# zhoubin-me/supertonic

Hardware: AMD Instinct MI355X
Metric: audio-sec/sec (RTF^-1), 66M model, batch=128 per GPU (higher is better)
Workload: dtype bf16

## Files before the change

### include/stn.h

```cpp
#ifndef STN_H
#define STN_H
#include <stddef.h>
#include <stdint.h>

#include "stn_arch.h"

#ifdef __cplusplus
extern "C" {
#endif

#define STN_OK 0
#define STN_ERR_INVALID (-1)
#define STN_ERR_DEVICE (-2)
#define STN_ERR_STATE (-3)
#define STN_ERR_UNSUPPORTED (-4)
#define STN_ERR_IO (-5)

#define STN_DTYPE_F32 0
#define STN_DTYPE_BF16 1
#define STN_DTYPE_F16 2

typedef struct stn_handle stn_handle;

typedef struct stn_config {
// ... 216 lines not shown
int stn_op_deesser(stn_handle* h, int hz, int rows, int W, const float* x, const stn_deesser* c, float* y);
int stn_op_deesser_ex(stn_handle* h, int hz, int rows, int W, const float* x, const stn_deesser* c, int x_misalign, int in_place, float* y,
                      float* band, float* gr_db, float* st_end, float* st_start, float* s1_end, float* s1_start, float* s2_end,
                      float* s2_start, int* guard_ok, char* form, size_t form_cap);
int stn_deesser_band(const stn_deesser* c, int rate_hz, double c10[10], float c32[10]);
int stn_deesser_coefs(const stn_deesser* c, int rate_hz, double k[2], float k32[2]);
const char* stn_deesser_error(const stn_deesser* c, int rate_hz);

typedef struct stn_expander { float threshold_db, ratio, knee_db, range_db, attack_ms, hold_ms, release_ms; } stn_expander;
int stn_set_expander(stn_handle* h, int on, const stn_expander* c);
int stn_get_expander(const stn_handle* h, int* on, stn_expander* out);
int stn_batch_expander(stn_handle* h, float* min_attenuation_db, int64_t* closed_samples);
int stn_op_expander(stn_handle* h, int hz, int rows, int W, const float* x, const stn_expander* c, float* y);
int stn_op_expander_ex(stn_handle* h, int hz, int rows, int W, const float* x, const stn_expander* c, int x_misalign, int in_place, float* y,
                       float* open_db, float* s1_end, float* s1_start, float* s2_end, float* s2_start, int* guard_ok, char* form,
                       size_t form_cap);
int stn_expander_coefs(const stn_expander* c, int rate_hz, double k[3], float k32[3], int64_t* hold_samples);
int stn_expander_curve(const stn_expander* c, int n, const double* in_db, double* out_db);
const char* stn_expander_error(const stn_expander* c, int rate_hz);

int stn_profile_enable(stn_handle* h, int on);
int stn_profile_reset(stn_handle* h);
int stn_profile_filter(stn_handle* h, const char* family_or_null);
int stn_profile_sample(stn_handle* h, int every);
int stn_launch_log_enable(stn_handle* h, int on);
int64_t stn_launch_log(stn_handle* h, char* out, size_t cap);
int stn_profile_count(stn_handle* h);
int stn_profile_get(stn_handle* h, int idx, char* name, size_t name_cap, double* total_ms, int64_t* launches,
                    double* flops, double* bytes);

int stn_dbg_xattn_hs_enable(stn_handle* h, int on);
int64_t stn_dbg_xattn_hs_stamps(stn_handle* h, unsigned long long* out, size_t cap);
int stn_dbg_fold_run_frames(const int32_t* latent_lengths, int B, int n_cu);

int stn_op_gemm(stn_handle* h, int dtype, int M, int N, int K, const float* A , const float* W ,
                const float* bias_or_null, int act , float* out );
int stn_op_gemm_ex(stn_handle* h, int dtype, int M, int N, int K, const float* A , const float* W , int mode, int act,
                   int out_dtype, int ldo, const float* bias_or_null, const float* gamma_or_null, const int32_t* len_or_null, int L,
                   const int32_t* row_b_or_null, const float* rowvec_or_null, int nseq, int nt, int tr, float* out, int64_t out_elems,
                   char* form, size_t form_cap);
int stn_dbg_gemm_form(int dtype, int M, int N, int K, int mode, int out_dtype, int ldo, int masked, int tr, char* out, size_t cap);
int stn_dbg_ffn_form(int dtype, int stage, int C, int I, int64_t M, int64_t gate_rows, int packed, int k, int max_dil, int mask,
                     int64_t min_rows, int64_t split_min_rows, int nt_hints, char* out, size_t cap);
int stn_op_gemm_bench(stn_handle* h, int dtype, int M, int N, int K, int mode, int iters, double* avg_ms);
int stn_op_gemm_phases(stn_handle* h, int dtype, int M, int N, int K, int mode, double* out6);
int stn_op_dwconv_ln(stn_handle* h, int dtype, int B, int L, int C, int k, int dil, const float* x,
                     const float* w , const float* bias, const float* ln_g, const float* ln_b, float* y);
int stn_op_dwconv_ln_ragged(stn_handle* h, int dtype, int B, int L, int C, int k, int dil, const float* x,
                            const float* w , const float* bias, const float* ln_g, const float* ln_b,
                            const int32_t* seqlen , float* y);
int stn_op_dwconv_ln_ex(stn_handle* h, int dtype, int B, int L, int C, int k, int dil, const float* x, int64_t x_rows,
                        const float* w_or_null , const float* bias_or_null, const float* ln_g, const float* ln_b,
                        const int32_t* seqlen_or_null, int packed, int ln_only, float* y, int64_t y_rows, char* form, size_t form_cap);
int stn_dbg_dwconv_ln_form(int dtype, int B, int L, int C, int k, int packed, char* out, size_t cap);
int stn_op_fold_ln(stn_handle* h, int dtype, int M, int C, int S, const float* part, const float* b2, const float* gamma,
                   const float* rowvec_or_null, const int32_t* row_b_or_null, int nseq, const float* ln_g, const float* ln_b, float* x,
                   float* y);
int stn_op_layout(stn_handle* h, int which, int dtype, const int32_t* p, int n_p, const float* a, int64_t a_n, const float* b, int64_t b_n,
                  const float* c, int64_t c_n, const int64_t* ids, int64_t ids_n, const int32_t* len, int packed, float* out, int64_t out_n,
                  float* out2, int64_t out2_n, int32_t* iout, int64_t iout_n);
int stn_op_attention(stn_handle* h, int dtype, int B, int Lq, int Lk, int H, int dh, const float* q, const float* k,
                     const float* v, const int32_t* qlen_or_null, const int32_t* klen_or_null, int rope_mode, float* o);
int stn_op_attention_ex(stn_handle* h, int dtype, int B, int Lq, int Lk, int H, int dh, const float* q, int64_t q_elems, int ldq,
                        int q_col, float* kv, int64_t kv_elems, int ldk, int k_col, int v_col, float* o, int64_t o_elems, int ldo,
                        const int32_t* qlen_or_null, const int32_t* klen_or_null, const int32_t* q_off_or_null,
                        const int32_t* k_off_or_null, int rope_mode, int k_rotated, int rot_groups, int rot_stride, int rot_col,
                        char* form, size_t form_cap);
int stn_op_xattn_hs(stn_handle* h, int dtype, int M, const float* xn, const float* Wq, const float* bq_or_null, const float* Wo,
                    const float* kv, int64_t kv_elems, int ldk, int k_col, int B, int L, int Lk, const int32_t* qlen,
                    const int32_t* klen_or_null, const int32_t* k_off_or_null, int rope_mode, int pairs_mode, int64_t part_stride,
                    float* part, int64_t part_elems, int32_t* pairs_out_or_null, char* form, size_t form_cap);
int stn_dbg_attn_form(int kind, int dtype, int B, int Lq, int Lk, int H, int dh, int ldq, int ldk, int misaligned, char* out, size_t cap);
int stn_op_ffn(stn_handle* h, int M, int C, int I, const float* xn , const float* W1, const float* b1, const float* W2,
               const float* b2_or_null, const float* gamma_or_null, const float* rowvec_or_null ,
               const int32_t* row_b_or_null , int nseq, float* x, int fused);
int stn_op_ffn_ex(stn_handle* h, int dtype, int M, int C, int I, const float* xn, int ldx, int64_t xn_elems, const float* W1, const float* b1,
                  const float* W2, const float* b2_or_null, const float* gamma_or_null, const int32_t* len_or_null, int L,
                  const int32_t* row_b_or_null, const float* rowvec_or_null, int rv_ld, int nseq, int mode, int split, float* x, int ldo,
                  int64_t x_elems, float* part_or_null, int64_t part_stride, int64_t part_elems, char* form, size_t form_cap);
int stn_op_ffn_bench(stn_handle* h, int M, int C, int I, int fused, int iters, double* out5);
int stn_op_fold_dwconv_ln(stn_handle* h, int B, int C, int k, int dil, int S, const int32_t* seqlen, const float* x, const float* part,
                          const float* b2_or_null, const float* gamma_or_null, const float* rowvec_or_null , const float* w ,
                          const float* bias, const float* ln_g, const float* ln_b, float* x_out, float* y);
int stn_op_fold_dwconv_ln_ex(stn_handle* h, int dtype, int B, int L, int C, int k, int dil, int S, int run_frames, const int32_t* seqlen,
                             const float* x_in, int64_t x_rows, const float* part, int64_t part_stride, int64_t part_elems,
                             const float* b2_or_null, const float* gamma_or_null, const float* rowvec_or_null, int rv_ld,
                             const float* w , const float* bias, const float* ln_g, const float* ln_b, float* x_out, int64_t x_out_rows,
                             float* y, int64_t y_rows, char* form, size_t form_cap);
int stn_dbg_fold_dwconv_ln_form(int dtype, int B, int L, int C, int k, int dil, int S, int has_rowvec, int run_frames, char* out, size_t cap);
int stn_op_block_bench(stn_handle* h, int B, int L, int C, int I, int k, int dil, int mode, int iters, double* out6);
int stn_op_randn(stn_handle* h, uint64_t seed, int B, int D, int L, const int64_t* utt_ids_or_null,
                 const int32_t* len_or_null, float* out);

const char* stn_version(void);
int stn_hip_versions(int* built, int* runtime);
int stn_device_count(void);
int stn_device_sync(int device);
int stn_ffn_fused_forms(int dtype, int C, int I);

#ifdef __cplusplus
}
#endif
#endif
```

### supertonic_amd/binding.py

```python
import ctypes
import os

import numpy as np

from .arch import StnArch

_HERE = os.path.dirname(os.path.abspath(__file__))
LIB_PATH = os.environ.get("STN_LIB") or os.path.join(_HERE, "libstn.so")
_LIB = None

F32, BF16, F16 = 0, 1, 2
_DTYPES = {"f32": F32, "fp32": F32, "float32": F32, "bf16": BF16, "f16": F16, "fp16": F16, "float16": F16, "half": F16,
           F32: F32, BF16: BF16, F16: F16}
ACT_NONE, ACT_GELU, ACT_SILU, ACT_GELU_TANH = 0, 1, 2, 3
EPI_STORE, EPI_RESID, EPI_STORE_T = 0, 1, 2
FFN_VOCODER, FFN_ESTIMATOR, FFN_TEXT = 1, 2, 4
LAYOUT_ROW_MAP, LAYOUT_NCL_TO_ROWS, LAYOUT_EULER_NCL, LAYOUT_UNPACK_ROWS, LAYOUT_EMBED, LAYOUT_MASKED_MEAN, LAYOUT_IM2COL, LAYOUT_VOCODER_IN = range(8)
ENC_F32, ENC_PCM16, ENC_PCM24, ENC_MULAW, ENC_ALAW = 0, 1, 2, 3, 4
ENCODINGS = {"f32": ENC_F32, "pcm16": ENC_PCM16, "pcm24": ENC_PCM24, "mulaw": ENC_MULAW, "alaw": ENC_ALAW}
ENCODING_NAMES = {v: k for k, v in ENCODINGS.items()}
ENCODING_BYTES = {ENC_F32: 4, ENC_PCM16: 2, ENC_PCM24: 3, ENC_MULAW: 1, ENC_ALAW: 1}
ZERO_CODEWORD = {ENC_F32: 0, ENC_PCM16: 0, ENC_PCM24: 0, ENC_MULAW: 0xFF, ENC_ALAW: 0xD5}


# ... 497 lines not shown
    L.stn_batch_vo_rows.restype = ctypes.c_int64
    L.stn_graph_replays.restype = ctypes.c_int64
    L.stn_graph_replays.argtypes = [vp]
    L.stn_graphs_cached.restype = ctypes.c_int64
    L.stn_graphs_cached.argtypes = [vp]
    L.stn_batch_dims.argtypes = [vp, ctypes.POINTER(ci), ctypes.POINTER(ci), ctypes.POINTER(ctypes.c_int64)]
    L.stn_batch_fetch.argtypes = [vp, vp, ctypes.c_size_t, vp]
    L.stn_batch_fetch_latent.argtypes = [vp, _f32p]
    L.stn_batch_fetch_pcm16.argtypes = [vp, vp, ctypes.c_size_t, vp]
    L.stn_batch_fetch_pcm16_begin.argtypes = [vp, ci]
    L.stn_batch_fetch_slot_dims.argtypes = [vp, ci, ctypes.POINTER(ci), ctypes.POINTER(ctypes.c_int64)]
    L.stn_batch_fetch_pcm16_end.argtypes = [vp, ci, ctypes.POINTER(vp), ctypes.POINTER(ctypes.c_size_t), vp]
    L.stn_host_alloc_pinned.restype = vp
    L.stn_host_alloc_pinned.argtypes = [ctypes.c_size_t]
    L.stn_host_free_pinned.argtypes = [vp]
    L.stn_batch_wav_device_ptr.argtypes = [vp, ctypes.POINTER(vp)]
    L.stn_sync.argtypes = [vp]
    L.stn_set_stream.argtypes = [vp, vp]
    L.stn_batch_copy_wav_device.argtypes = [vp, vp, ctypes.c_int64]
    L.stn_batch_copy_pcm16_device.argtypes = [vp, vp, ctypes.c_int64]
    L.stn_profile_filter.argtypes = [vp, ctypes.c_char_p]
    L.stn_profile_sample.argtypes = [vp, ci]
    L.stn_launch_log_enable.argtypes = [vp, ci]
    L.stn_dbg_xattn_hs_enable.argtypes = [vp, ci]
    L.stn_dbg_xattn_hs_stamps.argtypes = [vp, vp, ctypes.c_size_t]
    L.stn_dbg_xattn_hs_stamps.restype = ctypes.c_int64
    L.stn_dbg_fold_run_frames.argtypes = [vp, ctypes.c_int, ctypes.c_int]
    L.stn_dbg_fold_run_frames.restype = ctypes.c_int
    L.stn_dbg_gemm_form.argtypes = [ci, ci, ci, ci, ci, ci, ci, ci, ci, ctypes.c_char_p, ctypes.c_size_t]
    L.stn_dbg_gemm_form.restype = ctypes.c_int
    L.stn_dbg_attn_form.argtypes = [ci, ci, ci, ci, ci, ci, ci, ci, ci, ci, ctypes.c_char_p, ctypes.c_size_t]
    L.stn_dbg_attn_form.restype = ctypes.c_int
    L.stn_dbg_ffn_form.argtypes = [ci, ci, ci, ci, ctypes.c_int64, ctypes.c_int64, ci, ci, ci, ci, ctypes.c_int64, ctypes.c_int64, ci,
                                   ctypes.c_char_p, ctypes.c_size_t]
    L.stn_dbg_ffn_form.restype = ctypes.c_int
    L.stn_launch_log.argtypes = [vp, ctypes.c_char_p, ctypes.c_size_t]
    L.stn_launch_log.restype = ctypes.c_int64
    L.stn_profile_enable.argtypes = [vp, ci]
    L.stn_profile_reset.argtypes = [vp]
    L.stn_profile_count.argtypes = [vp]
    L.stn_profile_get.argtypes = [vp, ci, ctypes.c_char_p, ctypes.c_size_t, ctypes.POINTER(ctypes.c_double),
                                  ctypes.POINTER(ctypes.c_int64), ctypes.POINTER(ctypes.c_double),
                                  ctypes.POINTER(ctypes.c_double)]
    L.stn_op_gemm.argtypes = [vp, ci, ci, ci, ci, _f32p, _f32p, vp, ci, _f32p]
    L.stn_op_gemm_ex.argtypes = [vp, ci, ci, ci, ci, _f32p, _f32p, ci, ci, ci, ci, vp, vp, vp, ci, vp, vp, ci, ci, ci, _f32p,
                                 ctypes.c_int64, ctypes.c_char_p, ctypes.c_size_t]
    L.stn_op_gemm_bench.argtypes = [vp, ci, ci, ci, ci, ci, ci, ctypes.POINTER(ctypes.c_double)]
    L.stn_op_gemm_phases.argtypes = [vp, ci, ci, ci, ci, ci, ctypes.POINTER(ctypes.c_double)]
    L.stn_op_dwconv_ln.argtypes = [vp, ci, ci, ci, ci, ci, ci, _f32p, _f32p, _f32p, _f32p, _f32p, _f32p]
    L.stn_op_dwconv_ln_ragged.argtypes = [vp, ci, ci, ci, ci, ci, ci, _f32p, _f32p, _f32p, _f32p, _f32p, _i32p, _f32p]
    L.stn_op_attention.argtypes = [vp, ci, ci, ci, ci, ci, ci, _f32p, _f32p, _f32p, vp, vp, ci, _f32p]
    L.stn_op_dwconv_ln_ex.argtypes = [vp, ci, ci, ci, ci, ci, ci, _f32p, ctypes.c_int64, vp, vp, _f32p, _f32p, vp, ci, ci, _f32p, ctypes.c_int64,
                                      ctypes.c_char_p, ctypes.c_size_t]
    L.stn_dbg_resample_form.argtypes = [ci, ci, ctypes.c_int64, ctypes.c_char_p, ctypes.c_size_t]
    L.stn_dbg_resample_form.restype = ctypes.c_int
    L.stn_dbg_dwconv_ln_form.argtypes = [ci, ci, ci, ci, ci, ci, ctypes.c_char_p, ctypes.c_size_t]
    L.stn_dbg_dwconv_ln_form.restype = ctypes.c_int
    L.stn_op_fold_ln.argtypes = [vp, ci, ci, ci, ci, _f32p, _f32p, _f32p, vp, vp, ci, _f32p, _f32p, _f32p, _f32p]
    L.stn_op_layout.argtypes = [vp, ci, ci, _i32p, ci, vp, ctypes.c_int64, vp, ctypes.c_int64, vp, ctypes.c_int64, vp, ctypes.c_int64, vp, ci,
                                vp, ctypes.c_int64, vp, ctypes.c_int64, vp, ctypes.c_int64]
    L.stn_op_attention_ex.argtypes = [vp, ci, ci, ci, ci, ci, ci, _f32p, ctypes.c_int64, ci, ci, _f32p, ctypes.c_int64, ci, ci, ci,
                                      _f32p, ctypes.c_int64, ci, vp, vp, vp, vp, ci, ci, ci, ci, ci, ctypes.c_char_p, ctypes.c_size_t]
    L.stn_op_xattn_hs.argtypes = [vp, ci, ci, _f32p, _f32p, vp, _f32p, _f32p, ctypes.c_int64, ci, ci, ci, ci, ci, _i32p, vp, vp, ci, ci,
                                  ctypes.c_int64, _f32p, ctypes.c_int64, vp, ctypes.c_char_p, ctypes.c_size_t]
    L.stn_op_randn.argtypes = [vp, cu64, ci, ci, ci, vp, vp, _f32p]
    L.stn_op_ffn.argtypes = [vp, ci, ci, ci, _f32p, _f32p, _f32p, _f32p, vp, vp, vp, vp, ci, _f32p, ci]
    L.stn_op_ffn_ex.argtypes = [vp, ci, ci, ci, ci, _f32p, ci, ctypes.c_int64, _f32p, _f32p, _f32p, vp, vp, vp, ci, vp, vp, ci, ci, ci, ci, _f32p, ci,
                                ctypes.c_int64, vp, ctypes.c_int64, ctypes.c_int64, ctypes.c_char_p, ctypes.c_size_t]
    L.stn_op_ffn_bench.argtypes = [vp, ci, ci, ci, ci, ci, ctypes.POINTER(ctypes.c_double)]
    L.stn_set_fused_ffn.argtypes = [vp, ci]
    L.stn_set_fused_ffn_min_rows.argtypes = [vp, ctypes.c_int64, ctypes.c_int64]
    L.stn_op_fold_dwconv_ln.argtypes = [vp, ci, ci, ci, ci, ci, _i32p, _f32p, _f32p, vp, vp, vp, _f32p, _f32p, _f32p, _f32p, _f32p, _f32p]
    L.stn_op_fold_dwconv_ln_ex.argtypes = [vp, ci, ci, ci, ci, ci, ci, ci, ci, _i32p, _f32p, ctypes.c_int64, _f32p, ctypes.c_int64, ctypes.c_int64, vp, vp,
                                           vp, ci, _f32p, _f32p, _f32p, _f32p, _f32p, ctypes.c_int64, _f32p, ctypes.c_int64, ctypes.c_char_p,
                                           ctypes.c_size_t]
    L.stn_dbg_fold_dwconv_ln_form.argtypes = [ci, ci, ci, ci, ci, ci, ci, ci, ci, ctypes.c_char_p, ctypes.c_size_t]
    L.stn_dbg_fold_dwconv_ln_form.restype = ctypes.c_int
    L.stn_op_block_bench.argtypes = [vp, ci, ci, ci, ci, ci, ci, ci, ci, ctypes.POINTER(ctypes.c_double)]
    L.stn_group_create.argtypes = [ci, vp, ci, ctypes.POINTER(vp)]
    L.stn_group_destroy.argtypes = [vp]
    L.stn_group_last_error.restype = ctypes.c_char_p
    L.stn_group_last_error.argtypes = [vp]
    L.stn_group_size.argtypes = [vp]
    L.stn_group_uses_rccl.argtypes = [vp]
    L.stn_group_handle.restype = vp
    L.stn_group_handle.argtypes = [vp, ci]
    L.stn_group_load_synthetic.argtypes = [vp, ctypes.POINTER(StnArch), cu64]
    L.stn_group_load_dir.argtypes = [vp, ctypes.c_char_p]
    L.stn_group_deal.argtypes = [ci, _i32p, ci, _i32p, _i32p]
    L.stn_group_synthesize.argtypes = [vp, ci, ci, _i64p, _f32p, _f32p, _f32p, ci, cf, vp, cu64, ctypes.POINTER(ctypes.c_int64)]
    L.stn_group_fetch_pcm16.argtypes = [vp, vp, ctypes.c_size_t, vp]
    L.stn_set_output_rate.argtypes = [vp, ci]
    L.stn_get_output_rate.argtypes = [vp]
    L.stn_resample_filter.argtypes = [ci, ci, vp, ctypes.c_size_t, ctypes.POINTER(ci), ctypes.POINTER(ci)]
    L.stn_resample_error.argtypes = [ci, ci]
    L.stn_resample_error.restype = ctypes.c_char_p
    L.stn_op_resample.argtypes = [vp, ci, ci, ci, ci, _f32p, vp, vp]
    L.stn_group_set_output_rate.argtypes = [vp, ci]
    _f64p = np.ctypeslib.ndpointer(np.float64, flags="C_CONTIGUOUS")
    L.stn_set_loudness.argtypes = [vp, ci, cf, cf]
    L.stn_get_loudness.argtypes = [vp, ctypes.POINTER(ci), ctypes.POINTER(cf), ctypes.POINTER(cf)]
    L.stn_batch_loudness.argtypes = [vp, vp, vp, vp]
    L.stn_op_loudness.argtypes = [vp, ci, ci, ci, _f32p, vp, vp, vp]
    L.stn_kweighting_filter.argtypes = [ci, _f64p, _f64p, _f64p, _f64p]
    L.stn_op_loudness_ex.argtypes = [vp, ci, ci, ci, _f32p, vp, ci, cf, cf, ci, vp, vp, vp, vp, vp, vp, vp, vp, ctypes.c_char_p, ctypes.c_size_t]
    L.stn_loudness_table.argtypes = [ci, vp, vp, ctypes.c_size_t, ctypes.POINTER(ci)]
# ... 1474 lines not shown
        C = x_in.shape[1]
        w = _c(w, np.float32)
        _b2, b2p = _opt(b2, np.float32)
        _g, gp = _opt(gamma, np.float32)
        _v, vp_ = _opt(rowvec, np.float32)
        form = ctypes.create_string_buffer(96)
        self._ck(self._lib.stn_op_fold_dwconv_ln_ex(self._h, self.dtype if dtype is None else _DTYPES[dtype], len(seqlen), int(L), C, w.shape[1], int(dil),
                                                    int(S), int(run_frames), seqlen, x_in.reshape(-1), x_in.shape[0], part, int(part_stride), part.size,
                                                    b2p, gp, vp_, C if _v is None else _v.shape[1], w, _c(bias, np.float32), _c(g, np.float32),
                                                    _c(b, np.float32), xo.reshape(-1), xo.shape[0], yo.reshape(-1), yo.shape[0], form, ctypes.sizeof(form)))
        return xo, yo, form.value.decode()

    def op_block_bench(self, B, L, C, I, k, dil, mode, iters=20):
        out = (ctypes.c_double * 6)()
        self._ck(self._lib.stn_op_block_bench(self._h, B, L, C, I, k, dil, mode, iters, out))
        return dict(ms=out[0], conv_ms=out[1], fold_phase1=out[2], fold_barrier=out[3], fold_phase2=out[4], fold_span=out[5])

    def set_fused_ffn_min_rows(self, k4_rows=-1, split_rows=-1):
        self._ck(self._lib.stn_set_fused_ffn_min_rows(self._h, int(k4_rows), int(split_rows)))

    def op_gemm_phases(self, M, N, K, mode=0, dtype=None):
        out = (ctypes.c_double * 6)()
        self._ck(self._lib.stn_op_gemm_phases(self._h, self.dtype if dtype is None else _DTYPES[dtype], M, N, K, mode, out))
        return dict(first_stage=out[0], k_loop=out[1], epilogue=out[2], grid_span=out[3], entry_spread=out[4], workgroups=int(out[5]))

    def op_dwconv_ln(self, x, w, bias, g, b, dil, dtype=None, seqlen=None):
        B, L, C = x.shape
        k = w.shape[1]
        y = np.empty((B, L, C), np.float32)
        if seqlen is not None:
            self._ck(self._lib.stn_op_dwconv_ln_ragged(self._h, self.dtype if dtype is None else _DTYPES[dtype], B, L, C, k,
                                                       dil, _c(x, np.float32), _c(w, np.float32), _c(bias, np.float32),
                                                       _c(g, np.float32), _c(b, np.float32), _c(seqlen, np.int32), y))
            return y
        self._ck(self._lib.stn_op_dwconv_ln(self._h, self.dtype if dtype is None else _DTYPES[dtype], B, L, C, k, dil,
                                            _c(x, np.float32), _c(w, np.float32), _c(bias, np.float32),
                                            _c(g, np.float32), _c(b, np.float32), y))
        return y

    def op_dwconv_ln_ex(self, x, w, bias, g, b, dil, out, B, L, seqlen=None, packed=False, ln_only=False, dtype=None):
        x = _c(x, np.float32)
        o_r = np.array(out, dtype=np.float32, order="C", copy=True)
        C = x.shape[1]
        _w, wp = _opt(w, np.float32)
        _b, bp = _opt(bias, np.float32)
        _l, lp = _opt(seqlen, np.int32)
        form = ctypes.create_string_buffer(32)
        self._ck(self._lib.stn_op_dwconv_ln_ex(self._h, self.dtype if dtype is None else _DTYPES[dtype], int(B), int(L), C,
                                               1 if _w is None else _w.shape[1], int(dil), x.reshape(-1), x.shape[0], wp, bp, _c(g, np.float32),
                                               _c(b, np.float32), lp, int(bool(packed)), int(bool(ln_only)), o_r.reshape(-1), o_r.shape[0], form,
                                               ctypes.sizeof(form)))
        return o_r, form.value.decode()

    def op_fold_ln(self, x, part, b2, gamma, g, b, rowvec=None, row_b=None, dtype=None):
        x_r = np.array(x, dtype=np.float32, order="C", copy=True)
        M, C = x_r.shape
        part = _c(part, np.float32)
        y = np.empty((M, C), np.float32)
        _v, vp_ = _opt(rowvec, np.float32)
        _r, rp = _opt(row_b, np.int32)
        self._ck(self._lib.stn_op_fold_ln(self._h, self.dtype if dtype is None else _DTYPES[dtype], M, C, part.shape[0], part.reshape(-1),
                                          _c(b2, np.float32), _c(gamma, np.float32), vp_, rp, 0 if _v is None else _v.shape[0],
                                          _c(g, np.float32), _c(b, np.float32), x_r, y))
        return x_r, y

    def op_layout(self, which, p, a=None, b=None, c=None, ids=None, length=None, packed=False, out=None, out2=None, iout=None, dtype="f32"):
        def f32(v):
            return (None, None, 0) if v is None else (lambda arr: (arr, arr.ctypes.data, arr.size))(_c(v, np.float32))
        pa = _c(p, np.int32)
        _a, ap, an = f32(a)
        _b, bp, bn = f32(b)
        _cc, cp, cn = f32(c)
        _i, ip = _opt(ids, np.int64)
        _l, lp = _opt(length, np.int32)
        o1 = None if out is None else np.array(out, dtype=np.float32, order="C", copy=True)
        o2 = None if out2 is None else np.array(out2, dtype=np.float32, order="C", copy=True)
        io = None if iout is None else np.array(iout, dtype=np.int32, order="C", copy=True)
        ptr = lambda v: (None, 0) if v is None else (v.ctypes.data, v.size)
        self._ck(self._lib.stn_op_layout(self._h, int(which), _DTYPES[dtype], pa, len(pa), ap, an, bp, bn, cp, cn, ip, 0 if _i is None else _i.size,
                                         lp, int(bool(packed)), *ptr(o1), *ptr(o2), *ptr(io)))
        return o1, o2, io

    def op_attention(self, q, k, v, H, qlen=None, klen=None, rope_mode=-1, dtype=None):
        B, Lq, C = q.shape
        Lk = k.shape[1]
        o = np.empty((B, Lq, C), np.float32)
        _q, qp = _opt(qlen, np.int32)
        _k, kp = _opt(klen, np.int32)
        self._ck(self._lib.stn_op_attention(self._h, self.dtype if dtype is None else _DTYPES[dtype], B, Lq, Lk, H,
                                            C // H, _c(q, np.float32), _c(k, np.float32), _c(v, np.float32), qp, kp,
                                            rope_mode, o))
        return o

    def op_attention_ex(self, q, kv, out, B, Lq, Lk, H, dh, q_col=0, k_col=0, v_col=None, qlen=None, klen=None, q_off=None, k_off=None,
                        rope_mode=-1, k_rotated=False, rot_groups=1, rot_stride=0, rot_col=None, dtype=None):
        q = _c(q, np.float32)
        kv_r = np.array(kv, dtype=np.float32, order="C", copy=True)
        o_r = np.array(out, dtype=np.float32, order="C", copy=True)
        _a, qlp = _opt(qlen, np.int32)
        _b, klp = _opt(klen, np.int32)
        _d, qop = _opt(q_off, np.int32)
        _e, kop = _opt(k_off, np.int32)
        form = ctypes.create_string_buffer(64)
        self._ck(self._lib.stn_op_attention_ex(self._h, self.dtype if dtype is None else _DTYPES[dtype], int(B), int(Lq), int(Lk), int(H), int(dh),
                                               q.reshape(-1), q.size, q.shape[1], int(q_col), kv_r.reshape(-1), kv_r.size, kv_r.shape[1],
                                               int(k_col), int(k_col + H * dh if v_col is None else v_col), o_r.reshape(-1), o_r.size,
# ... 42 lines not shown
```

### supertonic_amd/csrc/api.cpp

```cpp
#include "../../include/stn.h"

#include <algorithm>
#include <complex>
#include <cstdio>
#include <cstring>
#include <fstream>
#include <string>

#include "engine.hpp"
#include "host/json_min.hpp"
#include "host/graph_bind.hpp"
#include "host/onnx_reader.hpp"

#include <map>
#include <sstream>

struct stn_handle {
    stn::Engine* eng = nullptr;
    std::string err;
    std::vector<std::pair<std::string, stn::KernelStat>> prof;
};

static thread_local std::string g_create_err;

// ... 883 lines not shown
        (dtype != STN_DTYPE_F32 && dtype != STN_DTYPE_BF16 && dtype != STN_DTYPE_F16))
        return STN_ERR_INVALID;
    const std::string f = stn::ffn_form(dtype, stage, C, I, M, gate_rows, packed != 0, k, max_dil, mask, min_rows, split_min_rows, nt_hints != 0).str();
    if (out && cap > f.size()) std::memcpy(out, f.c_str(), f.size() + 1);
    return (int)f.size();
}
int stn_op_gemm_bench(stn_handle* h, int dtype, int M, int N, int K, int mode, int iters, double* avg_ms) {
    STN_TRY(h, { need(M > 0 && N > 0 && K > 0 && iters > 0 && avg_ms, "stn_op_gemm_bench: bad argument");
                 need(K % (dtype != STN_DTYPE_F32 ? 8 : 4) == 0, "K must be a multiple of 8 (bf16) / 4 (f32)");
                 *avg_ms = h->eng->op_gemm_bench(dtype, M, N, K, mode, iters); })
}
int stn_op_gemm_phases(stn_handle* h, int dtype, int M, int N, int K, int mode, double* out6) {
    STN_TRY(h, { need(M > 0 && N > 0 && K > 0 && out6, "stn_op_gemm_phases: bad argument");
                 need(K % (dtype != STN_DTYPE_F32 ? 8 : 4) == 0, "K must be a multiple of 8 (bf16) / 4 (f32)");
                 h->eng->op_gemm_phases(dtype, M, N, K, mode, out6); })
}
int stn_op_dwconv_ln(stn_handle* h, int dtype, int B, int L, int C, int k, int dil, const float* x, const float* w,
                     const float* bias, const float* g, const float* b, float* y) {
    STN_TRY(h, { need(B > 0 && L > 0 && C > 0 && C % 4 == 0 && C <= 1024 && k > 0 && (k & 1) && dil > 0 && x && w && bias && g && b && y,
                      "stn_op_dwconv_ln: bad argument");
                 h->eng->op_dwconv_ln(dtype, B, L, C, k, dil, x, w, bias, g, b, y); })
}
int stn_op_dwconv_ln_ragged(stn_handle* h, int dtype, int B, int L, int C, int k, int dil, const float* x, const float* w,
                            const float* bias, const float* g, const float* b, const int32_t* seqlen, float* y) {
    STN_TRY(h, { need(B > 0 && L > 0 && C > 0 && C % 4 == 0 && C <= 1024 && k > 0 && (k & 1) && dil > 0 && x && w && bias && g && b && y && seqlen,
                      "stn_op_dwconv_ln_ragged: bad argument");
                 for (int i = 0; i < B; ++i) need(seqlen[i] >= 0 && seqlen[i] <= L, "stn_op_dwconv_ln_ragged: seqlen out of [0, L]");
                 h->eng->op_dwconv_ln(dtype, B, L, C, k, dil, x, w, bias, g, b, y, seqlen); })
}
static void dwconv_ln_ex_checked(stn_handle* h, int dtype, int B, int L, int C, int k, int dil, const float* x, int64_t x_rows, const float* w,
                                 const float* bias, const float* g, const float* b, const int32_t* seqlen, int packed, int ln_only, float* y,
                                 int64_t y_rows, char* form, size_t form_cap) {
    need(B > 0 && L > 0 && C > 0 && C % 4 == 0 && C <= 1024 && k > 0 && (k & 1) && dil > 0 && x && g && b && y && x_rows > 0 && y_rows > 0,
         "stn_op_dwconv_ln_ex: bad argument");
    need(dtype == STN_DTYPE_F32 || dtype == STN_DTYPE_BF16 || dtype == STN_DTYPE_F16, "stn_op_dwconv_ln_ex: unknown dtype");
    need(ln_only || (w && bias), "stn_op_dwconv_ln_ex: the conv needs w and bias");
    need(!(packed && ln_only), "stn_op_dwconv_ln_ex: ln_only takes no packed layout");
    need(!packed || (seqlen && B <= 1024), "stn_op_dwconv_ln_ex: packed rows need seqlen and B <= 1024");
    int64_t rows = (int64_t)B * L;
    if (seqlen && !ln_only) {
        int64_t tot = 0;
        for (int i = 0; i < B; ++i) { need(seqlen[i] >= 0 && seqlen[i] <= L, "stn_op_dwconv_ln_ex: seqlen out of [0, L]"); tot += seqlen[i]; }
        if (packed) rows = tot;
    }
    need(x_rows >= rows && y_rows >= rows, "stn_op_dwconv_ln_ex: x / y hold fewer rows than the launch addresses");
    const std::string f = h->eng->op_dwconv_ln_ex(dtype, B, L, C, k, dil, x, x_rows, w, bias, g, b, ln_only ? nullptr : seqlen, packed, ln_only, y, y_rows);
    if (form && form_cap) std::snprintf(form, form_cap, "%s", f.c_str());
}
int stn_op_dwconv_ln_ex(stn_handle* h, int dtype, int B, int L, int C, int k, int dil, const float* x, int64_t x_rows, const float* w,
                        const float* bias, const float* g, const float* b, const int32_t* seqlen, int packed, int ln_only, float* y,
                        int64_t y_rows, char* form, size_t form_cap) {
    STN_TRY(h, dwconv_ln_ex_checked(h, dtype, B, L, C, k, dil, x, x_rows, w, bias, g, b, seqlen, packed, ln_only, y, y_rows, form, form_cap))
}
int stn_dbg_dwconv_ln_form(int dtype, int B, int L, int C, int k, int packed, char* out, size_t cap) {
    if (B < 1 || L < 1 || C < 1 || k < 1 || !(k & 1) || (dtype != STN_DTYPE_F32 && dtype != STN_DTYPE_BF16 && dtype != STN_DTYPE_F16)) return STN_ERR_INVALID;
    std::string f;
    try { f = stn::dwconv_ln_form(dtype, B, L, C, k, packed != 0).str(); } catch (const std::exception&) { return STN_ERR_INVALID; }
    if (out && cap > f.size()) std::memcpy(out, f.c_str(), f.size() + 1);
    return (int)f.size();
}
int stn_op_fold_ln(stn_handle* h, int dtype, int M, int C, int S, const float* part, const float* b2, const float* gamma, const float* rowvec,
                   const int32_t* row_b, int nseq, const float* g, const float* b, float* x, float* y) {
    STN_TRY(h, { need(M > 0 && C > 0 && C % 4 == 0 && C <= 1024 && (S == 4 || S == 8 || S == 12 || S == 24) && part && b2 && gamma && g && b && x && y,
                      "stn_op_fold_ln: bad argument");
                 need(dtype == STN_DTYPE_BF16 || dtype == STN_DTYPE_F16, "stn_op_fold_ln: a 16-bit format needed");
                 need(!rowvec || nseq > 0, "stn_op_fold_ln: rowvec needs nseq > 0");
                 if (rowvec && row_b) for (int m = 0; m < M; ++m) need(row_b[m] >= 0 && row_b[m] < nseq, "stn_op_fold_ln: row_b out of range");
                 h->eng->op_fold_ln(dtype, M, C, S, part, b2, gamma, rowvec, row_b, nseq, g, b, x, y); })
}
int stn_op_layout(stn_handle* h, int which, int dtype, const int32_t* p, int n_p, const float* a, int64_t a_n, const float* b, int64_t b_n,
                  const float* c, int64_t c_n, const int64_t* ids, int64_t ids_n, const int32_t* len, int packed, float* out, int64_t out_n,
                  float* out2, int64_t out2_n, int32_t* iout, int64_t iout_n) {
    static const int n_params[8] = {3, 4, 5, 3, 4, 3, 6, 6};
    STN_TRY(h, { need(which >= 0 && which < 8 && p && n_p == n_params[which], "stn_op_layout: unknown kernel or parameter count");
                 need(dtype == STN_DTYPE_F32 || dtype == STN_DTYPE_BF16 || dtype == STN_DTYPE_F16, "stn_op_layout: unknown dtype");
                 need(a_n >= 0 && b_n >= 0 && c_n >= 0 && ids_n >= 0 && out_n >= 0 && out2_n >= 0 && iout_n >= 0 && (a || !a_n) && (b || !b_n) && (c || !c_n) &&
                          (ids || !ids_n) && (out || !out_n) && (out2 || !out2_n) && (iout || !iout_n),
                      "stn_op_layout: a buffer without a pointer");
                 h->eng->op_layout(which, dtype, p, a, a_n, b, b_n, c, c_n, ids, ids_n, len, packed, out, out_n, out2, out2_n, iout, iout_n); })
}
int stn_op_attention(stn_handle* h, int dtype, int B, int Lq, int Lk, int H, int dh, const float* q, const float* k,
                     const float* v, const int32_t* qlen, const int32_t* klen, int rope_mode, float* o) {
    STN_TRY(h, { need(B > 0 && Lq > 0 && Lk > 0 && H > 0 && dh >= 8 && dh % 8 == 0 && dh <= 96 && q && k && v && o,
                      "stn_op_attention: bad argument");
                 h->eng->op_attention(dtype, B, Lq, Lk, H, dh, q, k, v, qlen, klen, rope_mode, o); })
}
static void attention_ex_checked(stn_handle* h, int dtype, int B, int Lq, int Lk, int H, int dh, const float* q, int64_t q_elems, int ldq,
                                 int q_col, float* kv, int64_t kv_elems, int ldk, int k_col, int v_col, float* o, int64_t o_elems, int ldo,
                                 const int32_t* qlen, const int32_t* klen, const int32_t* q_off, const int32_t* k_off, int rope_mode,
                                 int k_rotated, int rot_groups, int rot_stride, int rot_col, char* form, size_t form_cap) {
    need(B > 0 && Lq > 0 && Lk > 0 && H > 0 && dh >= 8 && dh % 8 == 0 && dh <= 96 && q && kv && o, "stn_op_attention_ex: bad argument");
    need(dtype == STN_DTYPE_F32 || dtype == STN_DTYPE_BF16 || dtype == STN_DTYPE_F16, "stn_op_attention_ex: unknown dtype");
    need(rope_mode >= -1 && rope_mode <= 1, "stn_op_attention_ex: rope_mode must be -1, 0 or 1");
    const int64_t C = (int64_t)H * dh;
    need(ldq > 0 && ldk > 0 && ldo >= C && q_col >= 0 && k_col >= 0 && v_col >= 0 && q_col + C <= ldq && k_col + C <= ldk && v_col + C <= ldk,
         "stn_op_attention_ex: the heads must lie inside the rows (col + H*dh <= ld, ldo >= H*dh)");
    need((q_off == nullptr || qlen) && (k_off == nullptr || klen), "stn_op_attention_ex: packed rows need their lengths");
    const int64_t qrows = q_elems / ldq, krows = kv_elems / ldk, orows = o_elems / ldo;
    for (int b = 0; b < B; ++b) {
        need(!qlen || qlen[b] >= 0, "stn_op_attention_ex: qlen < 0");
        need(!klen || klen[b] >= 0, "stn_op_attention_ex: klen < 0");
        if (q_off)
            need(qlen[b] <= Lq && q_off[b] >= 0 && (int64_t)q_off[b] + qlen[b] <= std::min(qrows, orows),
                 "stn_op_attention_ex: packed query rows outside q / o (or qlen > Lq)");
        if (k_off) need(k_off[b] >= 0 && (int64_t)k_off[b] + std::min(klen[b], Lk) <= krows, "stn_op_attention_ex: packed key rows outside kv");
    }
// ... 169 lines not shown
```

### supertonic_amd/csrc/engine.cpp

```cpp
#include "engine.hpp"
#include "dev_env.hpp"
#include "engine_internal.hpp"

#include <algorithm>
#include <cmath>
#include <cstdio>
#include <cstring>

namespace stn {
using detail::up;

Arena::~Arena() {
    for (auto& c : chunks_) (void)hipFree(c.p);
}
size_t Arena::capacity() const {
    size_t t = 0;
    for (auto& c : chunks_) t += c.cap;
    return t;
}
void* Arena::alloc(size_t bytes) {
    bytes = (bytes + 255) & ~size_t(255);
    if (bytes == 0) bytes = 256;
    for (;;) {
        if (cur_ < chunks_.size()) {
// ... 80 lines not shown
    STN_HIP(hipEventCreateWithFlags(&ev_te_, hipEventDisableTiming));
    STN_HIP(hipEventCreateWithFlags(&ev_copied_, hipEventDisableTiming));
    STN_HIP(hipEventCreateWithFlags(&ev_dp_, hipEventDisableTiming));
    STN_HIP(hipStreamCreateWithPriority(&te_s_, hipStreamNonBlocking, prio_side));
    if (const char* p = stn::dev_env("STN_DP_STREAM")) if (atoi(p) == 0) {
        (void)hipStreamDestroy(dp_s_); dp_s_ = nullptr;
        (void)hipStreamDestroy(te_s_); te_s_ = nullptr;
    }
    if (const char* p = stn::dev_env("STN_NT")) nt_hints_ = atoi(p) != 0;
    if (const char* p = stn::dev_env("STN_FFN")) fused_ffn_ = atoi(p);
    if (const char* p = stn::dev_env("STN_FFN_MIN_ROWS")) ffn_min_rows_ = atoll(p);
    if (const char* p = stn::dev_env("STN_XATTN")) set_fused_xattn(atoi(p));
    if (const char* p = stn::dev_env("STN_FFN_SPLIT_MIN_ROWS")) ffn_split_min_rows_ = atoll(p);
    if (const char* p = stn::dev_env("STN_PACKED")) packed_ve_ = atoi(p) != 0;
}

void Engine::set_stream(hipStream_t s) {
    sync();
    s_ = s ? s : own_s_;
}

void Engine::drop_graphs() {
    for (auto& g : graphs_) {
        if (g.exec) (void)hipGraphExecDestroy(g.exec);
        if (g.graph) (void)hipGraphDestroy(g.graph);
        if (g.exec2) (void)hipGraphExecDestroy(g.exec2);
        if (g.graph2) (void)hipGraphDestroy(g.graph2);
    }
    graphs_.clear();
    warm_keys_.clear();
}

void Engine::free_weights() {
    if (s_) (void)hipStreamSynchronize(s_);
    drop_graphs();
    ++wgen_;
    for (void* p : owned_) (void)hipFree(p);
    owned_.clear();
    w_.clear();
    frag_w_.clear();
    ffn_w_.clear();
    loaded_ = false;
    params_ = 0;
}

Engine::~Engine() {
    (void)hipSetDevice(device_);
    if (s_) (void)hipStreamSynchronize(s_);
    if (dp_s_) (void)hipStreamSynchronize(dp_s_);
    if (te_s_) (void)hipStreamSynchronize(te_s_);
    free_weights();
    for (void* p : batch_owned_) (void)hipFree(p);
    for (void* p : batch_retired_) (void)hipFree(p);
    if (vo_quiet_) (void)hipFree(vo_quiet_);
    if (vo_edge_) (void)hipFree(vo_edge_);
    if (tcond_.buf) (void)hipFree(tcond_.buf);
    for (auto& sp : spans_) { (void)hipEventDestroy(sp.a); (void)hipEventDestroy(sp.b); }
    for (auto ev : ev_pool_) (void)hipEventDestroy(ev);
    drop_graphs();
    if (pin_llen_) (void)hipHostFree(pin_llen_);
    if (pin_seed_) (void)hipHostFree(pin_seed_);
    if (seed_dev_) (void)hipFree(seed_dev_);
    rs_release();
    fl_release();
    xp_release();
    ds_release();
    cp_release();
    lo_release();
    for (auto& f : fetch_) {
        if (f.busy && f.done) (void)hipEventSynchronize(f.done);
        if (f.dev) (void)hipFree(f.dev);
        if (f.pin) (void)hipHostFree(f.pin);
        if (f.ready) (void)hipEventDestroy(f.ready);
        if (f.done) (void)hipEventDestroy(f.done);
    }
    if (copy_s_) (void)hipStreamDestroy(copy_s_);
    if (own_s_) (void)hipStreamDestroy(own_s_);
    if (dp_s_) (void)hipStreamDestroy(dp_s_);
    if (te_s_) (void)hipStreamDestroy(te_s_);
    if (ev_te_) (void)hipEventDestroy(ev_te_);
    if (ev_copied_) (void)hipEventDestroy(ev_copied_);
    if (ev_dp_) (void)hipEventDestroy(ev_dp_);
}

DevTensor& Engine::tensor(const std::string& name) {
    auto it = w_.find(name);
    if (it == w_.end()) throw std::runtime_error("unknown weight tensor: " + name);
    return it->second;
}
Linear Engine::linear(const std::string& p) {
    Linear l;
    l.w = tensor(p + ".w");
    l.b = tensor(p + ".b").f32;
    l.N = l.w.rows;
    l.K = l.w.cols;
    return l;
}
LNorm Engine::lnorm(const std::string& p) { return LNorm{tensor(p + ".g").f32, tensor(p + ".b").f32}; }
ConvNeXt Engine::convnext_w(const std::string& p) {
    ConvNeXt c;
    c.dw_t = tensor(p + ".dw.wt").f32;
    c.dw_b = tensor(p + ".dw.b").f32;
    c.ln = lnorm(p + ".ln");
    c.pw1 = linear(p + ".pw1");
    c.pw2 = linear(p + ".pw2");
    c.gamma = tensor(p + ".gamma").f32;
    return c;
}
// ... 257 lines not shown
        while (b < k.size() && (k[b] == '(' || k[b] == ' ' || k[b] == '&')) ++b;
        size_t en = b;
        while (en < k.size() && (isalnum((unsigned char)k[en]) || k[en] == '_' || k[en] == ':')) ++en;
        out += e.first + "\t" + k.substr(b, en - b) + "\n";
    }
    return out;
}
std::vector<std::pair<std::string, KernelStat>> Engine::profile_collect() {
    sync();
    std::unordered_map<std::string, KernelStat> acc;
    std::vector<std::string> order;
    for (auto& sp : spans_) {
        float ms = 0.f;
        if (hipEventElapsedTime(&ms, sp.a, sp.b) != hipSuccess) { (void)hipGetLastError(); continue; }
        auto it = acc.find(sp.tag);
        if (it == acc.end()) { order.push_back(sp.tag); it = acc.emplace(sp.tag, KernelStat{}).first; }
        it->second.ms += ms;
        it->second.launches += 1;
        it->second.flops += sp.flops;
        it->second.bytes += sp.bytes;
    }
    std::vector<std::pair<std::string, KernelStat>> out;
    for (auto& t : order) out.emplace_back(t, acc[t]);
    return out;
}

void Engine::gemm(const char* tag, int dt, const void* A, int lda, const Linear& w, int M, Epilogue e) {
    if (!e.bias) e.bias = w.b;
    const double esz = is_half(dt) ? 2.0 : 4.0;
    if (prof_on_) {
        double out_b = (double)M * w.N * (e.mode == EPI_STORE ? (is_half(e.out_dtype) ? 2.0 : 4.0) : (e.mode == EPI_RESID ? 8.0 : 4.0));
        prof_begin(tag, 2.0 * M * (double)w.N * w.K, ((double)M * w.K + (double)w.N * w.K) * esz + out_b);
    }
    const GemmForm f = gemm_form(dt, M, w.N, w.K, lda, w.K, e, A, w.w.as(dt));
    if (f.split > 1) {
        const Arena::Mark mk = ar_.mark();
        float* ws = f32_alloc((int64_t)f.split * M * w.N);
        launch_gemm_form(s_, f, A, lda, w.w.as(dt), w.K, M, w.N, w.K, e, ws);
        ar_.release(mk);
    } else {
        launch_gemm_form(s_, f, A, lda, w.w.as(dt), w.K, M, w.N, w.K, e, nullptr);
    }
    if (prof_on_) prof_end();
}

void* Engine::to_act(const float* src, int64_t n) {
    if (dt_ == F32) return const_cast<float*>(src);
    void* d = act_alloc(n);
    launch_cast(s_, dt_, src, n, d);
    return d;
}

void Engine::convnext(const ConvNeXt& p, const FfnForm& f, float* x, int B, int L, int C, int hid, int k, int dil, const int* len,
                      const int* conv_len, const float* rowvec, int rv_ld, const Ragged* rg, FoldState* fs) {
    const int64_t M = rg ? (int64_t)rg->rows : (int64_t)B * L;
    if (f.kind == FFN_K4_SPLIT && !(fs && rg)) throw std::logic_error("convnext: K4-split needs the stage's fold state and packed rows");
    const Arena::Mark mk = ar_.mark();
    void* xn = act_alloc(M * C);
    if (fs) x = fs->x;
    if (fs && fs->pending) {
        if (prof_on_) prof_begin("fold_dwconv_ln", (double)M * C * (2.0 * k + 8 + 2.0 * fs->fold.S), (double)M * C * (8.0 + 2.0 + 2.0 * fs->fold.S));
        fs->fold.run_frames = rg->fold_run;
        launch_fold_dwconv_ln(s_, dt_, fs->x, fs->x_alt, B, L, C, fs->fold, p.dw_t, p.dw_b, k, dil, p.ln.g, p.ln.b, a_.ln_eps, xn, len, rg->off);
        if (prof_on_) prof_end();
        std::swap(fs->x, fs->x_alt);
        fs->pending = false;
        x = fs->x;
    } else {
        if (prof_on_) prof_begin("dwconv_ln", (double)M * C * (2.0 * k + 8), (double)M * C * (4.0 + (is_half(dt_) ? 2.0 : 4.0)));
        launch_dwconv_ln(s_, dt_, x, B, L, C, p.dw_t, p.dw_b, k, dil, p.ln.g, p.ln.b, a_.ln_eps, xn, rg ? len : conv_len, rg ? rg->off : nullptr);
        if (prof_on_) prof_end();
    }
    FfnArgs fa;
    fa.xn = xn; fa.ldx = C; fa.b1 = p.pw1.b; fa.b2 = p.pw2.b; fa.gamma = p.gamma; fa.x = x; fa.ldo = C; fa.M = (int)M; fa.I = hid;
    fa.rowvec = rowvec; fa.rv_ld = rv_ld; fa.row_b = (rg && rowvec) ? rg->row_b : nullptr;
    fa.len = rg ? nullptr : len; fa.L = L;
    if (f.kind != FFN_GEMMS) {
        const auto fw = ffn_w_.find(p.pw1.w.as(dt_));
        const int* s = std::find(std::begin(FFN_SPLITS), std::end(FFN_SPLITS), f.split);
        fa.wseq = fw == ffn_w_.end() ? nullptr : f.kind == FFN_K4 ? fw->second.wseq : s != std::end(FFN_SPLITS) ? fw->second.wsplit[s - FFN_SPLITS] : nullptr;
        if (!fa.wseq) throw std::logic_error("convnext: no packed weight stream for " + f.str());
    }
    if (f.kind == FFN_K4_SPLIT) { fa.part = fs->part; fa.part_stride = fs->part_stride; }
    const FoldArgs pending = ffn_launch(f, C, fa, p.pw1, p.pw2);
    if (f.kind == FFN_K4_SPLIT) { fs->fold = pending; fs->pending = true; }
    ar_.release(mk);
}

FoldArgs Engine::ffn_launch(const FfnForm& f, int C, const FfnArgs& a, const Linear& w1, const Linear& w2) {
    const int64_t M = a.M;
    const int hid = a.I;
    FoldArgs pending;
    if (f.kind == FFN_K4_SPLIT) {
        FfnArgs sa;
        sa.xn = a.xn; sa.ldx = a.ldx; sa.wseq = a.wseq; sa.b1 = a.b1; sa.M = a.M; sa.I = hid; sa.ts = a.ts;
        sa.split = f.split; sa.part = a.part; sa.part_stride = a.part_stride;
        if (prof_on_) prof_begin("ffn_split", 4.0 * M * (double)C * hid, (double)M * C * (2.0 + 2.0 * sa.split) + 4.0 * C * hid);
        launch_ffn_fused(s_, dt_, C, sa);
        if (prof_on_) prof_end();
        pending = ffn_pending(f, a);
    } else if (f.kind == FFN_K4) {
        if (prof_on_) prof_begin("ffn_fused", 4.0 * M * (double)C * hid, (double)M * C * (2.0 + 8.0) + 4.0 * C * hid);
        launch_ffn_fused(s_, dt_, C, a);
        if (prof_on_) prof_end();
    } else {
        const Arena::Mark mk = ar_.mark();
        void* u = act_alloc(M * hid);
        Epilogue e1;
        e1.mode = EPI_STORE; e1.act = gelu_act_; e1.out_dtype = dt_; e1.out = u; e1.ldo = hid; e1.bias = a.b1; e1.nt = f.nt ? 1 : 0;
        gemm("gemm_pw1_gelu", dt_, a.xn, a.ldx, w1, (int)M, e1);
        Epilogue e2;
        e2.mode = EPI_RESID; e2.resid = a.x; e2.ldo = a.ldo; e2.bias = a.b2; e2.gamma = a.gamma; e2.len = a.len; e2.L = a.L;
        e2.rowvec = a.rowvec; e2.rv_ld = a.rv_ld; e2.row_b = a.row_b;
        gemm("gemm_pw2_resid", dt_, u, hid, w2, (int)M, e2);
        ar_.release(mk);
    }
    return pending;
}

void Engine::fold_layernorm(FoldState& fs, int64_t M, int C, const LNorm& ln, void* xn, const char* tag) {
    const size_t esz = is_half(dt_) ? 2 : 4;
    if (fs.pending) {
        if (prof_on_) prof_begin("fold_ln", (double)M * C * (8 + 2.0 * fs.fold.S), (double)M * C * (8.0 + esz + 2.0 * fs.fold.S));
// ... 334 lines not shown
                owned_.push_back(dst);
                launch_repack_frag_acc(s_, src, w.o.N, w.o.K, dst);
                frag_acc_w_[src] = dst;
            }
        }
    sync();
}

void Engine::prepare_ffn_weights() {
    ffn_w_.clear();
    const stn_arch& a = a_;
    void* tmp = nullptr;
    size_t tmp_bytes = 0;
    auto add = [&](const std::string& p, int C, int hid) {
        if (!ffn_fused_supported(dt_, C, hid)) return;
        const ConvNeXt c = convnext_w(p);
        void* wseq = nullptr;
        STN_HIP(hipMalloc(&wseq, (size_t)2 * hid * C * 2));
        owned_.push_back(wseq);
        if ((size_t)2 * hid * C * 2 > tmp_bytes) {
            if (tmp) (void)hipFree(tmp);
            tmp_bytes = (size_t)2 * hid * C * 2;
            STN_HIP(hipMalloc(&tmp, tmp_bytes));
        }
        launch_ffn_pack(s_, c.pw1.w.as(dt_), c.pw2.w.as(dt_), C, hid, tmp, wseq);
        sync();
        FfnW fw; fw.wseq = wseq;
        if (p.compare(0, 3, "ve.") == 0)
            for (size_t i = 0; i < std::size(FFN_SPLITS); ++i) {
                if (!ffn_split_valid(dt_, C, hid, FFN_SPLITS[i])) continue;
                void* ws = nullptr;
                STN_HIP(hipMalloc(&ws, (size_t)2 * hid * C * 2));
                owned_.push_back(ws);
                launch_ffn_pack(s_, c.pw1.w.as(dt_), c.pw2.w.as(dt_), C, hid, tmp, ws, FFN_SPLITS[i]);
                sync();
                fw.wsplit[i] = ws;
            }
        ffn_w_[c.pw1.w.as(dt_)] = fw;
    };
    auto S = [](const char* fmt, int i, int j = 0) { char b[64]; snprintf(b, sizeof b, fmt, i, j); return std::string(b); };
    for (int i = 0; i < a.dp_conv_blocks; ++i) add(S("dp.conv%d", i), a.dp_dim, a.dp_hidden);
    for (int i = 0; i < a.te_conv_blocks; ++i) add(S("te.conv%d", i), a.te_dim, a.te_hidden);
    for (int b = 0; b < a.ve_main_blocks; ++b) {
        for (int j = 0; j < a.ve_dilated; ++j) add(S("ve.m%d.dil%d", b, j), a.ve_dim, a.ve_hidden);
        add(S("ve.m%d.cn_a", b), a.ve_dim, a.ve_hidden);
        add(S("ve.m%d.cn_b", b), a.ve_dim, a.ve_hidden);
    }
    for (int j = 0; j < a.ve_tail_blocks; ++j) add(S("ve.tail%d", j), a.ve_dim, a.ve_hidden);
    for (int i = 0; i < a.vo_blocks; ++i) add(S("vo.blk%d", i), a.vo_dim, a.vo_hidden);
    sync();
    if (tmp) (void)hipFree(tmp);
}

void Engine::prepare_vocoder_constants() {
    if (vo_quiet_) { (void)hipFree(vo_quiet_); vo_quiet_ = nullptr; }
    if (vo_edge_) { (void)hipFree(vo_edge_); vo_edge_ = nullptr; }
    vo_rf_ = 0;
    const stn_arch& a = a_;
    if (!is_half(dt_) || !dwconv_ln_supports_packed(a.vo_dim, a.vo_kernel) || a.base_chunk_size % 4) return;
    const int rf = vocoder_receptive_field(), ccf = a.chunk_compress_factor, W = a.base_chunk_size;
    const int Lz = (4 * rf + ccf) / ccf + 1, Tz = Lz * ccf, D = a.latent_dim * ccf;
    ar_.reset();
    float* lat = f32_alloc((int64_t)D * Lz);
    float* wz = f32_alloc((int64_t)Tz * W);
    STN_HIP(hipMemsetAsync(lat, 0, sizeof(float) * (size_t)D * Lz, s_));
    vocoder_dev(1, Lz, lat, wz);
    STN_HIP(hipMalloc(reinterpret_cast<void**>(&vo_quiet_), sizeof(float) * (size_t)W));
    STN_HIP(hipMalloc(reinterpret_cast<void**>(&vo_edge_), sizeof(float) * (size_t)rf * W));
    STN_HIP(hipMemcpyAsync(vo_quiet_, wz + (size_t)2 * rf * W, sizeof(float) * (size_t)W, hipMemcpyDeviceToDevice, s_));
    STN_HIP(hipMemcpyAsync(vo_edge_, wz + (size_t)(Tz - rf) * W, sizeof(float) * (size_t)rf * W, hipMemcpyDeviceToDevice, s_));
    sync();
    vo_rf_ = rf;
}

int Engine::trimmed_rows(int B, int L, std::vector<int>* n_host) const {
    if (!packed_ve_ || vo_ragged_ || !vo_quiet_ || vo_rf_ <= 0 || B > 1024) return 0;
    const int ccf = a_.chunk_compress_factor, T = L * ccf, rf = vo_rf_;
    long tot = 0;
    bool any = false;
    for (int i = 0; i < B; ++i) {
        const int l6 = bt_.h_llen[i] * ccf;
        const bool trim = l6 + 2 * rf <= T;
        any = any || trim;
        const int n = trim ? l6 + 2 * rf : T;
        if (n_host) n_host->push_back(n);
        tot += n;
    }
    return (any && tot * 10 <= (long)B * T * 9) ? (int)tot : 0;
}

void Engine::vocoder_dev(int B, int L, const float* latent, float* wav, const int* vlen, int vrows, const int* valid) {
    stage_ = "vo";
    const stn_arch& a = a_;
    const int C = a.vo_dim, T = L * a.chunk_compress_factor;
    const bool packed = vlen && vrows > 0 && is_half(dt_) && B <= 1024 && dwconv_ln_supports_packed(C, a.vo_kernel);
    if (valid && !packed) throw std::runtime_error("trimmed vocoder needs the packed bf16 path");
    const int64_t M = packed ? (int64_t)vrows : (int64_t)B * T;
    const Arena::Mark mk = ar_.mark();
    Ragged rg;
    if (packed) {
        int* off = static_cast<int*>(ar_.alloc(sizeof(int) * (size_t)(B + 1)));
        launch_row_map(s_, vlen, B, off, nullptr);
        rg.off = off; rg.rows = vrows;
    }
    const Ragged* rgp = packed ? &rg : nullptr;
    float* x = f32_alloc(M * C);
    if (is_half(dt_)) {
        const int kp = (a.latent_dim * a.vo_in_kernel + 63) / 64 * 64;
        void* cols = act_alloc(M * kp);
        launch_vocoder_im2col(s_, dt_, latent, B, L, a.latent_dim, a.chunk_compress_factor, a.vo_in_kernel, kp, cols, vlen,
                              packed ? rg.off : nullptr);
        Linear lin;
        lin.w = tensor("vo.in_gemm.w"); lin.b = vecf("vo.in.b"); lin.N = C; lin.K = kp;
        Epilogue ei; ei.mode = EPI_STORE; ei.out_dtype = F32; ei.out = x; ei.ldo = C;
        gemm("gemm_in", dt_, cols, kp, lin, (int)M, ei);
    } else {
        if (prof_on_) prof_begin("vocoder_in", 2.0 * M * C * a.latent_dim * a.vo_in_kernel, (double)M * (a.latent_dim + C) * 4.0);
        launch_vocoder_in(s_, latent, B, L, a.latent_dim, a.chunk_compress_factor, vecf("vo.in.wt"), vecf("vo.in.b"), C,
                          a.vo_in_kernel, x, vlen);
        if (prof_on_) prof_end();
    }
    const FfnForm ff = ffn_plan(FFN_VOCODER, C, a.vo_hidden, M, valid ? (int64_t)B * T : 0, packed, a.vo_kernel,
                                a.vo_blocks ? *std::max_element(a.vo_dilations, a.vo_dilations + a.vo_blocks) : 1);
    for (int i = 0; i < a.vo_blocks; ++i)
        convnext(convnext_w("vo.blk" + std::to_string(i)), ff, x, B, T, C, a.vo_hidden, a.vo_kernel, a.vo_dilations[i],
                 packed ? vlen : nullptr, packed ? nullptr : vlen, nullptr, 0, rgp);
    void* xn = act_alloc(M * C);
    const LNorm ln = lnorm("vo.out_ln");
    launch_layernorm(s_, dt_, x, M, C, ln.g, ln.b, a.ln_eps, xn);
    if (packed) {
        float* wp = f32_alloc(M * a.base_chunk_size);
        Epilogue e; e.mode = EPI_STORE; e.out_dtype = F32; e.out = wp; e.ldo = a.base_chunk_size;
        gemm("gemm_head", dt_, xn, C, linear("vo.head"), (int)M, e);
        if (valid) launch_unpack_rows_quiet(s_, wp, valid, rg.off, B, T, a.base_chunk_size, vo_rf_, vo_quiet_, vo_edge_, wav);
        else launch_unpack_rows(s_, wp, vlen, rg.off, B, T, a.base_chunk_size, wav);
    } else {
        Epilogue e; e.mode = EPI_STORE; e.out_dtype = F32; e.out = wav; e.ldo = a.base_chunk_size; e.len = vlen; e.L = T;
        gemm("gemm_head", dt_, xn, C, linear("vo.head"), (int)M, e);
    }
    ar_.release(mk);
}


void Engine::duration(int B, int Lt, const int64_t* ids, const float* style_dp, const float* text_mask, float* dur) {
    STN_HIP(hipSetDevice(device_));
    ar_.reset();
    int64_t* d_ids = up(ar_, s_, ids, (size_t)B * Lt);
    float* d_mask = up(ar_, s_, text_mask, (size_t)B * Lt);
    float* d_st = up(ar_, s_, style_dp, (size_t)B * a_.n_style_dp * a_.d_style_dp);
    int* tlen = static_cast<int*>(ar_.alloc(sizeof(int) * B));
    float* d_dur = f32_alloc(B);
    launch_mask_to_len(s_, d_mask, B, Lt, tlen);
    duration_dev(B, Lt, d_ids, d_st, tlen, d_dur);
    STN_HIP(hipMemcpyAsync(dur, d_dur, sizeof(float) * B, hipMemcpyDeviceToHost, s_));
    sync();
}

void Engine::text_enc(int B, int Lt, const int64_t* ids, const float* style_ttl, const float* text_mask, float* text_emb) {
    STN_HIP(hipSetDevice(device_));
    ar_.reset();
    int64_t* d_ids = up(ar_, s_, ids, (size_t)B * Lt);
    float* d_mask = up(ar_, s_, text_mask, (size_t)B * Lt);
    float* d_st = up(ar_, s_, style_ttl, (size_t)B * a_.n_style_ttl * a_.d_style_ttl);
    int* tlen = static_cast<int*>(ar_.alloc(sizeof(int) * B));
    const size_t n = (size_t)B * a_.te_out_dim * Lt;
    float* d_out = f32_alloc(n);
    launch_mask_to_len(s_, d_mask, B, Lt, tlen);
    text_enc_dev(B, Lt, d_ids, d_st, tlen, d_out, nullptr);
    STN_HIP(hipMemcpyAsync(text_emb, d_out, n * 4, hipMemcpyDeviceToHost, s_));
    sync();
}

void Engine::vector_est(int B, int L, int Lt, const float* noisy, const float* text_emb, const float* style_ttl,
                        const float* text_mask, const float* latent_mask, const float* total_step,
                        const float* current_step, float* denoised) {
    STN_HIP(hipSetDevice(device_));
    ar_.reset();
    const int D = a_.latent_dim * a_.chunk_compress_factor, Ce = a_.te_out_dim;
    float* d_x = up(ar_, s_, noisy, (size_t)B * D * L);
    float* d_emb = up(ar_, s_, text_emb, (size_t)B * Ce * Lt);
    float* d_st = up(ar_, s_, style_ttl, (size_t)B * a_.n_style_ttl * a_.d_style_ttl);
    float* d_tm = up(ar_, s_, text_mask, (size_t)B * Lt);
    float* d_lm = up(ar_, s_, latent_mask, (size_t)B * L);
    float* d_tot = up(ar_, s_, total_step, (size_t)B);
    float* d_cur = up(ar_, s_, current_step, (size_t)B);
    int* tlen = static_cast<int*>(ar_.alloc(sizeof(int) * B));
    int* llen = static_cast<int*>(ar_.alloc(sizeof(int) * B));
    float* d_out = f32_alloc((size_t)B * D * L);
// ... 24 lines not shown
```

### supertonic_amd/csrc/engine.hpp

```cpp
#pragma once
#include <cmath>
#include <hip/hip_runtime.h>

#include <cstdint>
#include <functional>
#include <iterator>
#include <stdexcept>
#include <string>
#include <unordered_map>
#include <vector>

#include "../../include/stn_arch.h"
#include "host/join_plan.hpp"
#include "host/pause_plan.hpp"
#include "host/pitch.hpp"
#include "kernels.hpp"

namespace stn {

#define STN_HIP(expr)                                                                                          \
    do {                                                                                                       \
        hipError_t e_ = (expr);                                                                                \
        if (e_ != hipSuccess)                                                                                  \
            throw std::runtime_error(std::string("HIP error: ") + hipGetErrorString(e_) + " at " #expr);       \
// ... 77 lines not shown
};

struct Carve {
    char* base = nullptr;
    size_t off = 0;
    template <typename T> T* take(size_t count) {
        const size_t o = off;
        off += (count * sizeof(T) + 255) / 256 * 256;
        return base ? reinterpret_cast<T*>(base + o) : nullptr;
    }
};

struct KernelStat { double ms = 0; long launches = 0; double flops = 0; double bytes = 0; };

class Engine {
   public:
    Engine(int device, int dtype);
    ~Engine();
    Engine(const Engine&) = delete;

    void load_synthetic(const stn_arch& a, uint64_t seed);
    using TensorSource = std::function<std::vector<float>(const std::string& name, int rows, int cols)>;
    void load_tensors(const stn_arch& a, const TensorSource& src);
    std::vector<std::string> tensor_names(const stn_arch& a);
    bool loaded() const { return loaded_; }
    const stn_arch& arch() const { return a_; }
    int64_t param_count() const { return params_; }
    int dtype() const { return dt_; }
    hipStream_t stream() const { return s_; }
    void sync() { STN_HIP(hipStreamSynchronize(s_)); if (dp_s_) STN_HIP(hipStreamSynchronize(dp_s_)); if (te_s_) STN_HIP(hipStreamSynchronize(te_s_)); }
    void set_stream(hipStream_t s);

    struct Ragged;
    void duration_dev(int B, int Lt, const int64_t* ids, const float* style_dp, const int* tlen, float* dur, const Ragged* trg = nullptr);
    void text_enc_dev(int B, int Lt, const int64_t* ids, const float* style_ttl, const int* tlen, float* ncl, void* rows,
                      const Ragged* trg = nullptr);
    struct VeCtx { void* text_kv = nullptr; void* style_kv = nullptr; int Lt = 0; const int* text_off = nullptr; };
    VeCtx ve_prepare_dev(int B, int Lt, const void* text_rows, const float* style_ttl, const int* tlen, const Ragged* trg = nullptr, bool defer_text = false);
    void ve_text_kv_dev(const VeCtx& c, int B, int Lt, const void* text_rows, const int* tlen, const Ragged* trg);
    float* ve_time_cond_dev(int rows, const float* total_step, const float* current_step, float* tb_out = nullptr );
    struct TimeCond { int steps = 0, B = 0; uint64_t wgen = ~0ull; float* buf = nullptr; size_t cap = 0; float *tot = nullptr, *cur = nullptr, *dt = nullptr, *tb = nullptr; };
    TimeCond tcond_;
    void ensure_time_cond(int total_step, int B);
    struct Ragged { const int* off = nullptr; const int* row_b = nullptr; int rows = 0;
                    const int* hs_pairs = nullptr;
                    int fold_run = 0; };
    void ve_step_dev(int B, int L, const VeCtx& c, const float* noisy, const int* tlen, const int* llen,
                     const float* total_step, const float* current_step, float* denoised, const float* tb = nullptr,
                     const Ragged* rg = nullptr, const float* dt = nullptr ,
                     void* z_rows = nullptr ,
                     bool z_ready = false ,
                     bool z_next = false );
    void vocoder_dev(int B, int L, const float* latent, float* wav, const int* vlen = nullptr, int vrows = 0,
                     const int* valid = nullptr);
    int vocoder_receptive_field() const;
    void prepare_xattn_weights();
    std::unordered_map<const void*, const void*> frag_w_;
    void hs_stamps_enable(bool on);
    int64_t hs_stamps_fetch(unsigned long long* out, size_t cap);
    unsigned long long* hs_ts_ = nullptr;
    int hs_ts_wgs_ = 0;
    static constexpr int HS_TS_WG = 8192;
    const float* unit_vec_ = nullptr;
    std::unordered_map<const void*, const void*> frag_acc_w_;
    void prepare_vocoder_constants();
    void prepare_ffn_weights();
    struct FfnW { const void *wseq = nullptr, *wsplit[std::size(FFN_SPLITS)] = {}; };
    std::unordered_map<const void*, FfnW> ffn_w_;

    void duration(int B, int Lt, const int64_t* ids, const float* style_dp, const float* text_mask, float* dur);
    void text_enc(int B, int Lt, const int64_t* ids, const float* style_ttl, const float* text_mask, float* text_emb);
    void vector_est(int B, int L, int Lt, const float* noisy, const float* text_emb, const float* style_ttl,
                    const float* text_mask, const float* latent_mask, const float* total_step,
                    const float* current_step, float* denoised);
    void vocoder(int B, int L, const float* latent, float* wav);

    struct Batch {
        int B = 0, Lt = 0, L = 0, noise_L = 0, total_step = 0;
        float speed = 1.f;
        bool have_override = false, have_noise = false;
        uint64_t noise_seed = 0;
        int64_t* ids = nullptr; size_t ids_cap = 0;
        int* tlen = nullptr; size_t tlen_cap = 0;
        float* style_ttl = nullptr; size_t ttl_cap = 0;
        float* style_dp = nullptr; size_t dp_cap = 0;
        float* dur = nullptr; size_t dur_cap = 0;
        int* llen = nullptr; size_t llen_cap = 0;
        int64_t* utt_ids = nullptr; size_t utt_cap = 0;
        float* noise = nullptr; size_t noise_cap = 0;
        float* xt[2] = {nullptr, nullptr}; size_t xt_cap[2] = {0, 0};
        float* wav = nullptr; size_t wav_cap = 0;
        unsigned char* text_side = nullptr; size_t text_side_cap = 0;
        unsigned char* text_rows = nullptr; size_t text_cap = 0;
        int* toff = nullptr; size_t toff_cap = 0;
        int trows = 0;
        uint64_t gen = 0;
        std::vector<float> h_dur; std::vector<int> h_llen;
    };
    void batch_upload(int B, int Lt, const int64_t* ids, const float* text_mask, const float* style_ttl,
                      const float* style_dp, const float* duration_override, const int64_t* utt_ids);
    void batch_set_noise(const float* noise, int L);
    void batch_run(int total_step, float speed, uint64_t noise_seed);
    void set_graph_mode(bool on) { graph_on_ = on; }
    void set_vocoder_mode(bool length_aware) { vo_ragged_ = length_aware; }
    void set_packed_rows(bool on) { packed_ve_ = on; }
    void set_gelu_form(int tanh_form) { if ((tanh_form != 0) != (gelu_act_ == ACT_GELU_TANH)) { sync(); drop_graphs(); } gelu_act_ = tanh_form ? ACT_GELU_TANH : ACT_GELU; }
    int gelu_form() const { return gelu_act_ == ACT_GELU_TANH ? 1 : 0; }
// ... 142 lines not shown
        const char* form = "";
    };
    void op_compressor(int hz, int rows, int W, const float* x, const stn_compressor& c, float* y, CpProbe* probe);

    void set_deesser(bool on, const stn_deesser* c);
    bool deesser_on() const { return ds_on_; }
    const stn_deesser& deesser() const { return ds_set_; }
    void batch_deesser(float* max_reduction_db);
    struct DsProbe {
        int x_misalign = 0, in_place = 0;
        float *band = nullptr, *gr = nullptr, *st_end = nullptr, *st_start = nullptr;
        float *s1_end = nullptr, *s1_start = nullptr, *s2_end = nullptr, *s2_start = nullptr;
        bool guard_ok = false;
        const char* form = "";
    };
    void op_deesser(int hz, int rows, int W, const float* x, const stn_deesser& c, float* y, DsProbe* probe);

    void set_expander(bool on, const stn_expander* c);
    bool expander_on() const { return xp_on_; }
    const stn_expander& expander() const { return xp_set_; }
    void batch_expander(float* min_attenuation_db, int64_t* closed_samples);
    struct XpProbe {
        int x_misalign = 0, in_place = 0;
        float *open = nullptr, *s1_end = nullptr, *s1_start = nullptr, *s2_end = nullptr, *s2_start = nullptr;
        bool guard_ok = false;
        const char* form = "";
    };
    void op_expander(int hz, int rows, int W, const float* x, const stn_expander& c, float* y, XpProbe* probe);

    void profile_enable(bool on) { if (on != prof_on_) profile_reset(); prof_on_ = on; }
    void launch_log_enable(bool on);
    std::string launch_log() const;
    void profile_sample(int every) { prof_every_ = every < 1 ? 1 : every; prof_seen_ = 0; }
    void profile_filter(const std::string& family) { if (family != prof_filter_) profile_reset(); prof_filter_ = family; }
    void profile_reset();
    std::vector<std::pair<std::string, KernelStat>> profile_collect();

    void op_gemm(int dtype, int M, int N, int K, const float* A, const float* W, const float* bias, int act, float* out);
    std::string op_gemm_ex(int dtype, int M, int N, int K, const float* A, const float* W, int mode, int act, int out_dtype, int ldo,
                           const float* bias, const float* gamma, const int* len, int L, const int* row_b, const float* rowvec, int nseq,
                           int nt, int tr, float* out, int64_t out_elems);
    std::string op_attention_ex(int dtype, int B, int Lq, int Lk, int H, int dh, const float* q, int64_t q_elems, int ldq, int q_col,
                                float* kv, int64_t kv_elems, int ldk, int k_col, int v_col, float* o, int64_t o_elems, int ldo,
                                const int* qlen, const int* klen, const int* q_off, const int* k_off, int rope_mode, int k_rotated,
                                int rot_groups, int rot_stride, int rot_col);
    std::string op_xattn_hs(int dtype, int M, const float* xn, const float* Wq, const float* bq, const float* Wo, const float* kv,
                            int64_t kv_elems, int ldk, int k_col, int B, int L, int Lk, const int* qlen, const int* klen, const int* k_off,
                            int rope_mode, int pairs_mode, int64_t part_stride, float* part, int64_t part_elems, int* pairs_out);
    void op_attention(int dtype, int B, int Lq, int Lk, int H, int dh, const float* q, const float* k, const float* v,
                      const int* qlen, const int* klen, int rope_mode, float* o);
    void op_dwconv_ln(int dtype, int B, int L, int C, int k, int dil, const float* x, const float* w, const float* bias,
                      const float* g, const float* b, float* y, const int* seqlen = nullptr );
    std::string op_dwconv_ln_ex(int dtype, int B, int L, int C, int k, int dil, const float* x, int64_t x_rows, const float* w, const float* bias,
                                const float* g, const float* b, const int* seqlen, int packed, int ln_only, float* y, int64_t y_rows);
    void op_fold_ln(int dtype, int M, int C, int S, const float* part, const float* b2, const float* gamma, const float* rowvec, const int* row_b,
                    int nseq, const float* g, const float* b, float* x, float* y);
    void op_layout(int which, int dtype, const int* p, const float* a, int64_t a_n, const float* b, int64_t b_n, const float* c, int64_t c_n,
                   const int64_t* ids, int64_t ids_n, const int* len, int packed, float* out, int64_t out_n, float* out2, int64_t out2_n, int* iout,
                   int64_t iout_n);
    double op_gemm_bench(int dtype, int M, int N, int K, int mode, int iters);
    void op_gemm_phases(int dtype, int M, int N, int K, int mode, double* out6);
    void op_randn(uint64_t seed, int B, int D, int L, const int64_t* utt_ids, const int* len, float* out);
    void op_ffn(int M, int C, int I, const float* xn, const float* W1, const float* b1, const float* W2, const float* b2, const float* gamma,
                const float* rowvec , const int* row_b , int nseq, float* x, int mode);
    std::string op_ffn_ex(int M, int C, int I, const float* xn, int ldx, int64_t xn_elems, const float* W1, const float* b1, const float* W2,
                          const float* b2, const float* gamma, const int* len, int L, const int* row_b, const float* rowvec, int rv_ld, int nseq,
                          int mode, int split, float* x, int ldo, int64_t x_elems, float* part, int64_t part_stride, int64_t part_elems);
    void op_fold_dwconv_ln(int B, int C, int k, int dil, int S, const int* seqlen, const float* x, const float* part, const float* b2,
                           const float* gamma, const float* rowvec , const float* w , const float* bias,
                           const float* g, const float* b, float* x_out, float* y);
    std::string op_fold_dwconv_ln_ex(int dtype, int B, int L, int C, int k, int dil, int S, int run_frames, const int* seqlen, const float* x_in,
                                     int64_t x_rows, const float* part, int64_t part_stride, int64_t part_elems, const float* b2, const float* gamma,
                                     const float* rowvec, int rv_ld, const float* w, const float* bias, const float* g, const float* b, float* x_out,
                                     int64_t x_out_rows, float* y, int64_t y_rows);
    void op_ffn_bench(int M, int C, int I, int mode, int iters, double* out5);
    void op_block_bench(int B, int L, int C, int I, int k, int dil, int mode, int iters, double* out6);

    Arena& arena() { return ar_; }

   private:
    DevTensor& tensor(const std::string& name);
    const float* vecf(const std::string& name) { return tensor(name).f32; }
    Linear linear(const std::string& prefix);
    LNorm lnorm(const std::string& prefix);
    ConvNeXt convnext_w(const std::string& prefix);
    Attn attn_w(const std::string& prefix, bool self);
    void free_weights();
    using RawSource = std::function<std::vector<float>(const std::string& name, int kind, int rows, int cols, float gain)>;
    void load_weights(const stn_arch& a, const RawSource& src, std::vector<std::string>* names_only);

    size_t act_bytes(int64_t n) const { return (size_t)n * (is_half(dt_) ? 2 : 4); }
    void* act_alloc(int64_t n) { return ar_.alloc(act_bytes(n)); }
    float* f32_alloc(int64_t n) { return static_cast<float*>(ar_.alloc((size_t)n * 4)); }
    void gemm(const char* tag, int dt, const void* A, int lda, const Linear& w, int M, Epilogue e);
    struct FoldState {
        float* x = nullptr;
        float* x_alt = nullptr;
        void* part = nullptr;
        int64_t part_stride = 0;
        bool pending = false;
        FoldArgs fold;
    };
    FfnForm ffn_plan(int stage, int C, int I, int64_t M, int64_t gate_rows, bool packed, int k, int max_dil) const {
        return ffn_form(dt_, stage, C, I, M, gate_rows, packed, k, max_dil, fused_ffn_, ffn_min_rows_, ffn_split_min_rows_, nt_hints_);
    }
    FoldArgs ffn_launch(const FfnForm& f, int C, const FfnArgs& a, const Linear& w1, const Linear& w2);
    static FoldArgs ffn_pending(const FfnForm& f, const FfnArgs& a) {
        return FoldArgs{a.part, f.split, a.part_stride, a.b2, a.gamma, a.rowvec, a.rv_ld, a.row_b};
    }
    struct FfnOp { FfnForm f; Linear w1, w2; FfnArgs a; };
    FfnOp op_ffn_setup(const char* op, int mode, int M, int C, int I, const float* W1, const float* W2, int split = 0);
    void convnext(const ConvNeXt& p, const FfnForm& f, float* x, int B, int L, int C, int hid, int k, int dil, const int* len,
                  const int* conv_len = nullptr, const float* rowvec = nullptr, int rv_ld = 0, const Ragged* rg = nullptr, FoldState* fs = nullptr);
    void fold_layernorm(FoldState& fs, int64_t M, int C, const LNorm& ln, void* xn, const char* tag);
    void attn_block(const Attn& p, float* x, int B, int Lq, int C, int H, const void* ctx, int Lk, const int* qlen,
                    const int* klen, int rope_mode, bool self, const Ragged* qrg = nullptr);
    void* to_act(const float* src, int64_t n);

    struct ProfSpan { std::string tag; hipEvent_t a, b; double flops, bytes; };
    void prof_begin(const char* tag, double flops, double bytes);
    void prof_end();
    class StageSpan {
       public:
        StageSpan(Engine& e, const char* stage, const char* tag, double flops, double bytes) : e_(e), prev_(e.stage_) {
            e_.stage_ = stage;
            begin(tag, flops, bytes);
        }
        ~StageSpan() { end(); e_.stage_ = prev_; }
        StageSpan(const StageSpan&) = delete;
        StageSpan& operator=(const StageSpan&) = delete;
        void next(const char* tag, double flops, double bytes) { end(); begin(tag, flops, bytes); }

       private:
        void begin(const char* tag, double flops, double bytes) { if ((begun_ = e_.prof_on_)) e_.prof_begin(tag, flops, bytes); }
        void end() { if (begun_) e_.prof_end(); begun_ = false; }
        Engine& e_;
        const char* prev_;
        bool begun_ = false;
    };

    int device_, dt_;
    int n_cu_ = 256;
    hipStream_t s_ = nullptr, own_s_ = nullptr;
    const char* stage_ = "";
    std::string prof_filter_;
    std::string log_family_;
    int prof_every_ = 1;
    uint64_t prof_seen_ = 0;
    bool prof_active_ = false;
    stn_arch a_{};
    bool loaded_ = false;
    int64_t params_ = 0;
    std::unordered_map<std::string, DevTensor> w_;
    std::vector<void*> owned_;
    Arena ar_;
    Batch bt_;
    std::vector<void*> batch_owned_;
    std::vector<void*> batch_retired_;
    template <typename T> void ensure(T*& p, size_t& cap, size_t need);
    std::vector<float> reported_dur_;
    std::vector<int64_t> out_spans(int64_t Wo, int hz) const;
    void enqueue_after_duration(int total_step, const std::function<void()>& take_text_rows);
    struct GraphKey {
        int B = 0, Lt = 0, L = 0, steps = 0; bool noise = false, ragged = false; int xattn = 0; int ffn = 0; int rows = 0, vrows = 0, trows = 0;
        uint64_t gen = 0, wgen = 0; const void* p0 = nullptr; const void* p1 = nullptr; const void* pin = nullptr; hipStream_t s = nullptr;
        bool operator==(const GraphKey& o) const {
            return B == o.B && Lt == o.Lt && L == o.L && steps == o.steps && noise == o.noise && ragged == o.ragged && xattn == o.xattn && ffn == o.ffn &&
                   rows == o.rows && vrows == o.vrows && trows == o.trows && gen == o.gen && wgen == o.wgen && p0 == o.p0 && p1 == o.p1 && pin == o.pin && s == o.s;
        }
    };
    struct GraphEntry { GraphKey key; hipGraph_t graph = nullptr, graph2 = nullptr; hipGraphExec_t exec = nullptr, exec2 = nullptr; uint64_t last_use = 0; };
    static constexpr size_t kGraphCache = 8, kWarmKeys = 16;
    std::vector<GraphEntry> graphs_;
    std::vector<GraphKey> warm_keys_;
    uint64_t graph_clock_ = 0, wgen_ = 0;
    void drop_graphs();
    bool graph_on_ = true;
    bool vo_ragged_ = false;
    bool packed_ve_ = true;
    bool nt_hints_ = true;
    hipStream_t dp_s_ = nullptr, te_s_ = nullptr;
    Arena dp_ar_, te_ar_;
    hipEvent_t ev_te_ = nullptr, ev_copied_ = nullptr, ev_dp_ = nullptr;
    std::function<void()> text_gate_;
    bool copied_valid_ = false;
    int64_t ffn_min_rows_ = 18432;
    int64_t ffn_split_min_rows_ = 1;
    int fused_ffn_ = 9;
    bool shape_buckets_ = false;
    bool dur_read_always_ = false;
    int gelu_act_ = ACT_GELU;
    int fused_xattn_ = 1;
    int64_t last_ve_rows_ = 0, last_vo_rows_ = 0;
    float* vo_quiet_ = nullptr;
    float* vo_edge_ = nullptr;
    int vo_rf_ = 0;
    int trimmed_rows(int B, int L, std::vector<int>* n_host) const;
    long graph_replays_ = 0;
    int* pin_llen_ = nullptr; size_t pin_llen_cap_ = 0;
    unsigned long long* pin_seed_ = nullptr;
    bool pin_valid_ = false;
    unsigned long long* seed_dev_ = nullptr;
    int final_xt_ = 0;
    struct FetchSlot { unsigned char* dev = nullptr; unsigned char* pin = nullptr; size_t cap = 0, n = 0; int enc = ENC_PCM16; hipEvent_t ready = nullptr, done = nullptr; bool busy = false; std::vector<float> dur; };
    FetchSlot fetch_[2];
    int out_hz_ = 0;
    ResampleTable rs_, op_rs_;
    void rs_prepare(ResampleTable& t, int in_hz, int out_hz);
    const ResampleTable& rs_table();
    void rs_release();
    void resample_enqueue(const ResampleTable& t, const float* x, int64_t rows, int64_t W, int enc, void* y, int64_t dst_stride);
    float ps_semi_ = 0.0f;
    int ps_a_ = 1, ps_b_ = 1;
    uint64_t ps_gen_ = 0;
    ResampleTable ps_rs_, op_ps_rs_;
    void ps_table(ResampleTable& t, int a, int b);
    DevBuf ps_buf_;
    struct PsScratch { int64_t* n; float* win; int* delta; float* score; float* ys; float* y; size_t bytes; };
    static PsScratch ps_layout(char* base, int64_t rows, int64_t W, const PitchPlan& p);
    std::vector<int64_t> ps_n_; std::vector<float> ps_win_;
    struct PsKey {
        uint64_t seq = 0, gen = 0; int64_t W = 0; int B = 0; const void* buf = nullptr;
        bool operator==(const PsKey& o) const { return seq == o.seq && gen == o.gen && W == o.W && B == o.B && buf == o.buf; }
    };
    PsKey ps_key_; bool ps_valid_ = false;
    void ps_enqueue(const float* x, int64_t rows, int64_t W, const int64_t* n, int a, int b, const PitchPlan& p, const float* win, int* delta, float* score,
                    float* ys);
    void ps_resample(const ResampleTable& t, const float* ys, int64_t rows, int64_t Ws, int64_t W, float* y);
    void ps_op(int hz, int rows, int W, const float* x, const int64_t* n, int a, int b, float* ys_out, int* delta_out, float* score_out, float* y_out);
    const float* ps_batch();
    const float* wav_rows() { return pitch_on() ? ps_batch() : bt_.wav; }
    bool lo_on_ = false;
    float lo_target_ = -23.0f, lo_ceiling_ = -1.0f;
    LoudTable lo_, op_lo_;
    DevBuf lo_buf_;
    std::vector<int64_t> lo_n_;
    int64_t* lo_n_ptr_ = nullptr;
    struct LoRes { const float *lufs = nullptr, *peak = nullptr, *gain = nullptr; const int64_t* n = nullptr; };
    struct LoScratch { float *st, *pk, *pa, *pb, *res; int64_t* n; LoRes out; size_t bytes; };
    static LoScratch lo_layout(char* base, int64_t rows, int64_t W);
    LoScratch lo_scratch(int64_t rows, int64_t W);
    void lo_prepare(LoudTable& t, int hz);
    void lo_release();
    void lo_measure(const LoudTable& t, const float* x, int64_t rows, int64_t W, const LoScratch& sc, int64_t max_seg, bool on, float target, float ceiling,
                    float* st_end = nullptr, bool true_peak = false);
    void lo_op(int hz, int rows, int W, const float* x, const int64_t* n, bool on, float target, float ceiling, LoProbe* probe, float* lufs,
               float* peak, float* gain);
    LoRes lo_rows(const LoudTable& t, const float* x, int64_t rows, int64_t W, std::vector<int64_t> n, bool on, float target, float ceiling,
                  bool true_peak = false);
    bool lo_true_peak() const { return true_peak_on() && !limiter_active(); }
// ... 161 lines not shown
```

### supertonic_amd/csrc/engine_batch.cpp

```cpp
#include "engine.hpp"
#include "engine_internal.hpp"

#include <algorithm>
#include <cmath>
#include <cstdio>
#include <cstring>

namespace stn {
using detail::up;


template <typename T>
void Engine::ensure(T*& p, size_t& cap, size_t need) {
    if (p && need <= cap) return;
    const size_t n = std::max<size_t>(need + need / 4, 64);
    T* q = nullptr;
    STN_HIP(hipMalloc(reinterpret_cast<void**>(&q), n * sizeof(T)));
    if (p) {
        batch_owned_.erase(std::find(batch_owned_.begin(), batch_owned_.end(), static_cast<void*>(p)));
        batch_retired_.push_back(p);
    }
    batch_owned_.push_back(q);
    p = q;
    cap = n;
// ... 114 lines not shown
                STN_HIP(hipEventRecord(ev_dp_, s_));
            }
        }
        if (!b.have_override || dur_read_always_) STN_HIP(hipEventSynchronize(ev_dp_));
        if (b.have_override) dur = b.h_dur;
    }
    auto take_text_rows = [this, &b, text_bytes]() {
        if (te_s_) STN_HIP(hipStreamWaitEvent(s_, ev_te_, 0));
        STN_HIP(hipMemcpyAsync(b.text_rows, b.text_side, text_bytes, hipMemcpyDeviceToDevice, s_));
        STN_HIP(hipEventRecord(ev_copied_, s_));
        copied_valid_ = true;
    };
    for (float& d : dur) d /= speed;
    int L = 0;
    latent_geometry(a, dur, L, b.h_llen);
    if (L < 1) throw std::runtime_error("predicted duration too short: zero latent frames");
    if (shape_buckets_ && !b.have_noise) L = (int)bucket_up(L, 16);
    if (b.have_noise && b.noise_L != L)
        throw std::runtime_error("injected noise has L=" + std::to_string(b.noise_L) + " but the durations imply L=" + std::to_string(L));
    b.L = L;
    reported_dur_ = dur;
    ++ed_seq_;
    const size_t nx = (size_t)B * D * L, nw = (size_t)B * L * a.base_chunk_size * a.chunk_compress_factor;
    ensure(b.xt[0], b.xt_cap[0], nx);
    ensure(b.xt[1], b.xt_cap[1], nx);
    ensure(b.wav, b.wav_cap, nw);
    if ((size_t)B > pin_llen_cap_) {
        if (pin_llen_) { sync(); drop_graphs(); (void)hipHostFree(pin_llen_); pin_llen_ = nullptr; }
        const size_t cap = std::max<size_t>((size_t)B, 1024);
        STN_HIP(hipHostMalloc(reinterpret_cast<void**>(&pin_llen_), sizeof(int) * cap, hipHostMallocDefault));
        pin_llen_cap_ = cap;
        pin_valid_ = false;
    }
    if (!pin_seed_) {
        STN_HIP(hipHostMalloc(reinterpret_cast<void**>(&pin_seed_), sizeof(unsigned long long), hipHostMallocDefault));
        STN_HIP(hipMalloc(reinterpret_cast<void**>(&seed_dev_), sizeof(unsigned long long)));
        pin_valid_ = false;
    }
    if (!pin_valid_ || !std::equal(b.h_llen.begin(), b.h_llen.end(), pin_llen_) || *pin_seed_ != (unsigned long long)noise_seed) {
        sync();
        std::copy(b.h_llen.begin(), b.h_llen.end(), pin_llen_);
        *pin_seed_ = (unsigned long long)noise_seed;
        pin_valid_ = true;
    }

    ensure_time_cond(total_step, B);
    GraphKey key;
    key.B = B; key.Lt = Lt; key.L = L; key.steps = total_step; key.noise = b.have_noise; key.ragged = vo_ragged_; key.xattn = fused_xattn_;
    key.ffn = fused_ffn_; key.gen = b.gen; key.wgen = wgen_; key.pin = pin_llen_;
    key.rows = 0;
    if (packed_rows_ok(B)) for (int v : b.h_llen) key.rows += v;
    if (shape_buckets_) key.rows = (int)bucket_up(key.rows, 64);
    last_ve_rows_ = key.rows ? key.rows : (int64_t)B * L;
    key.vrows = trimmed_rows(B, L, nullptr);
    if (shape_buckets_) key.vrows = (int)bucket_up(key.vrows, 64 * a.chunk_compress_factor);
    key.trows = tpk ? b.trows : 0;
    last_vo_rows_ = (int64_t)B * L * a.chunk_compress_factor;
    if (vo_ragged_ && packed_ve_ && is_half(dt_)) {
        last_vo_rows_ = 0;
        for (int v : b.h_llen) last_vo_rows_ += (int64_t)v * a.chunk_compress_factor;
        if (shape_buckets_) last_vo_rows_ = bucket_up(last_vo_rows_, 64 * a.chunk_compress_factor);
        key.vrows = (int)last_vo_rows_;
    }
    else if (key.vrows) last_vo_rows_ = key.vrows;
    key.p0 = b.xt[0]; key.p1 = b.wav; key.s = s_;
    const bool graphable = graph_on_ && !prof_on_;
    if (graphable) {
        for (auto& g : graphs_)
            if (g.key == key) {
                g.last_use = ++graph_clock_;
                STN_HIP(hipGraphLaunch(g.exec, s_));
                take_text_rows();
                STN_HIP(hipGraphLaunch(g.exec2, s_));
                ++graph_replays_;
                return;
            }
    }
    const auto warm = std::find(warm_keys_.begin(), warm_keys_.end(), key);
    if (graphable && warm != warm_keys_.end()) {
        const Arena::Mark cap0 = ar_.mark();
        const size_t cap_before = ar_.capacity();
        STN_HIP(hipStreamBeginCapture(s_, hipStreamCaptureModeThreadLocal));
        bool ok = true;
        std::string why;
        hipGraph_t g = nullptr, g2 = nullptr;
        hipError_t ec1 = hipErrorUnknown;
        bool split = false;
        auto split_capture = [&]() {
            ec1 = hipStreamEndCapture(s_, &g);
            split = true;
            STN_HIP(hipStreamBeginCapture(s_, hipStreamCaptureModeThreadLocal));
        };
        try { enqueue_after_duration(total_step, split_capture); } catch (const std::exception& e) { ok = false; why = e.what(); }
        const hipError_t ec = hipStreamEndCapture(s_, &g2);
        text_gate_ = nullptr;
        ar_.release(cap0);
        hipGraphExec_t ex = nullptr, ex2 = nullptr;
        if (ok && split && ec1 == hipSuccess && ec == hipSuccess && g && g2 && ar_.capacity() == cap_before &&
            hipGraphInstantiate(&ex, g, nullptr, nullptr, 0) == hipSuccess && hipGraphInstantiate(&ex2, g2, nullptr, nullptr, 0) == hipSuccess) {
            if (graphs_.size() >= kGraphCache) {
                auto lru = std::min_element(graphs_.begin(), graphs_.end(), [](const GraphEntry& x, const GraphEntry& y) { return x.last_use < y.last_use; });
                sync();
                (void)hipGraphExecDestroy(lru->exec);
                (void)hipGraphDestroy(lru->graph);
                if (lru->exec2) (void)hipGraphExecDestroy(lru->exec2);
                if (lru->graph2) (void)hipGraphDestroy(lru->graph2);
                graphs_.erase(lru);
// ... 62 lines not shown
        launch_mask_ncl(s_, b.xt[0], B, D, L, b.llen);
    } else {
        launch_randn_masked(s_, 0, b.utt_ids, B, D, L, b.llen, b.xt[0], seed_dev_);
    }
    VeCtx c = ve_prepare_dev(B, Lt, text_rows, b.style_ttl, b.tlen, trgp, true);
    text_gate_ = [this, &c, &b, &take_text_rows, B, Lt, text_rows, trgp]() {
        take_text_rows();
        ve_text_kv_dev(c, B, Lt, text_rows, b.tlen, trgp);
    };
    struct Disarm { std::function<void()>& g; ~Disarm() { g = nullptr; } } disarm{text_gate_};
    if (a.ve_main_blocks == 0) { auto fire = std::move(text_gate_); text_gate_ = nullptr; fire(); }
    if (tcond_.steps != total_step || tcond_.B != B || tcond_.wgen != wgen_) throw std::runtime_error("time conditioning not prepared for this run");
    const float* tot_all = tcond_.tot;
    const float* cur_all = tcond_.cur;
    const float* dt_all = tcond_.dt;
    const float* tb_all = tcond_.tb;
    const size_t tb_stride = (size_t)B * a.ve_main_blocks * a.ve_dim;
    Ragged rg;
    const Ragged* rgp = nullptr;
    if (packed_rows_ok(B)) {
        rg.rows = 0;
        for (int v : b.h_llen) rg.rows += v;
        if (shape_buckets_) rg.rows = (int)bucket_up(rg.rows, 64);
        int* off = static_cast<int*>(ar_.alloc(sizeof(int) * (size_t)(B + 1)));
        int* row_b = static_cast<int*>(ar_.alloc(sizeof(int) * (size_t)std::max(rg.rows, 1)));
        launch_row_map(s_, b.llen, B, off, row_b, rg.rows);
        rg.off = off; rg.row_b = row_b;
        rg.fold_run = fold_run_frames(b.h_llen.data(), B, n_cu_);
        if (fused_xattn_ && is_half(dt_) && B >= 2) {
            int* pairs = static_cast<int*>(ar_.alloc(sizeof(int) * (size_t)(B + 2)));
            launch_xattn_hs_pairs(s_, b.llen, B, pairs);
            rg.hs_pairs = pairs;
        }
        rgp = &rg;
    }
    int cur = 0;
    const int Dz = (a.latent_dim * a.chunk_compress_factor + 63) / 64 * 64;
    const int64_t Mz = rgp ? (int64_t)rg.rows : (int64_t)B * L;
    void* z_rows = act_alloc(Mz * Dz);
    for (int st = 0; st < total_step; ++st) {
        ve_step_dev(B, L, c, b.xt[cur], b.tlen, b.llen, tot_all + (size_t)st * B, cur_all + (size_t)st * B, b.xt[cur ^ 1],
                    tb_all + (size_t)st * tb_stride, rgp, dt_all, z_rows, st > 0, st + 1 < total_step);
        cur ^= 1;
    }
    final_xt_ = cur;
    const int* vlen = nullptr;
    if (vo_ragged_) {
        int* v = static_cast<int*>(ar_.alloc(sizeof(int) * B));
        launch_scale_len(s_, b.llen, B, a.chunk_compress_factor, v);
        vlen = v;
    }
    int vrows = 0;
    const int* valid = nullptr;
    if (vo_ragged_ && packed_ve_) {
        for (int v : b.h_llen) vrows += v * a.chunk_compress_factor;
        if (shape_buckets_) vrows = (int)bucket_up(vrows, 64 * a.chunk_compress_factor);
    } else if (int tr = trimmed_rows(B, L, nullptr)) {
        if (shape_buckets_) tr = (int)bucket_up(tr, 64 * a.chunk_compress_factor);
        int* n_dev = static_cast<int*>(ar_.alloc(sizeof(int) * B));
        int* v_dev = static_cast<int*>(ar_.alloc(sizeof(int) * B));
        launch_trim_len(s_, b.llen, B, a.chunk_compress_factor, L * a.chunk_compress_factor, vo_rf_, n_dev, v_dev);
        vlen = n_dev; valid = v_dev; vrows = tr;
    }
    vocoder_dev(B, L, b.xt[cur], b.wav, vlen, vrows, valid);
    STN_HIP(hipGetLastError());
}


char* DevBuf::reserve(Engine& e, size_t bytes, bool* moved) {
    const bool grow = !p_ || bytes > cap_;
    if (moved) *moved = grow;
    if (!grow) return p_;
    e.sync();
    if (p_) (void)hipFree(p_);
    p_ = nullptr; cap_ = 0;
    STN_HIP(hipMalloc(reinterpret_cast<void**>(&p_), bytes + bytes / 4));
    cap_ = bytes + bytes / 4;
    return p_;
}

int64_t Engine::out_row_len() {
    STN_HIP(hipSetDevice(device_));
    const Batch& b = bt_;
    if (!b.wav || b.L == 0) throw std::runtime_error("no finished batch");
    return out_len(native_row_len());
}

bool Engine::out_native() const { return !pitch_on() && !loudness_on() && !out_in_scratch(); }

const float* Engine::out_source(int64_t Wo) {
    const Batch& b = bt_;
    const float* wav = wav_rows();
    if (!out_in_scratch()) return wav;
    float* d = out_f32_buf((size_t)b.B * Wo);
    if (resample_on()) resample_enqueue(rs_table(), wav, b.B, native_row_len(), ENC_F32, d, Wo);
    if (filter_on()) fl_batch(resample_on() ? d : wav, Wo, d);
    if (expander_on()) xp_batch(resample_on() || filter_on() ? d : wav, Wo, d);
    if (deesser_on()) ds_batch(resample_on() || filter_on() || expander_on() ? d : wav, Wo, d);
    if (compressor_on()) cp_batch(resample_on() || filter_on() || expander_on() || deesser_on() ? d : wav, Wo, d);
    return d;
}

Engine::GainedRows Engine::gain_step(const float* src, int64_t rows, int64_t W, int64_t stride, const LoRes& m) {
    if (!limiter_active()) return {src, m.gain, stride};
    const LmScratch lm = lm_rows(src, rows, W, m.n, m.gain);
    return {lm.y, lm.trim, W};
}

static int64_t join_stride(const JoinPlan& p);
static size_t join_f32_offset(size_t n_rows);
static int need_enc(int enc) {
    const int eb = enc_bytes(enc);
    if (eb == 0) throw std::invalid_argument("unknown sample encoding " + std::to_string(enc));
    return eb;
}

void Engine::enqueue_output(const OutRows& o) {
// ... 422 lines not shown
```

### supertonic_amd/csrc/engine_ops.cpp

```cpp
#include "engine.hpp"
#include "engine_internal.hpp"

#include <algorithm>
#include <cmath>
#include <cstdio>
#include <cstring>

namespace stn {
using detail::up;

void Engine::op_gemm(int dtype, int M, int N, int K, const float* A, const float* W, const float* bias, int act, float* out) {
    STN_HIP(hipSetDevice(device_));
    ar_.reset();
    float* dA = up(ar_, s_, A, (size_t)M * K);
    float* dW = up(ar_, s_, W, (size_t)N * K);
    float* dB = bias ? up(ar_, s_, bias, (size_t)N) : nullptr;
    float* dO = f32_alloc((size_t)M * N);
    const void* pa = dA;
    const void* pw = dW;
    if (is_half(dtype)) {
        void* a16 = ar_.alloc((size_t)M * K * 2);
        void* w16 = ar_.alloc((size_t)N * K * 2);
        launch_cast(s_, dtype, dA, (int64_t)M * K, a16);
        launch_cast(s_, dtype, dW, (int64_t)N * K, w16);
// ... 451 lines not shown
            ++live;
            p1 += (double)(h[4 * w + 1] - h[4 * w]); p2 += (double)(h[4 * w + 2] - h[4 * w + 1]); p3 += (double)(h[4 * w + 3] - h[4 * w + 2]);
            tmin = std::min(tmin, h[4 * w]); tmax = std::max(tmax, h[4 * w + 3]);
        }
        if (live) { out2[2] = p1 / live; out2[3] = p2 / live; out2[4] = p3 / live; out2[5] = (double)(tmax - tmin); }
    }
    STN_HIP(hipGetLastError());
    sync();
}

static void down_as(Arena& ar, hipStream_t s, int dtype, const void* d, float* h, size_t n) {
    const float* src = static_cast<const float*>(d);
    if (is_half(dtype)) {
        float* w = static_cast<float*>(ar.alloc(n * 4));
        launch_half_to_f32(s, dtype, d, (int64_t)n, w);
        src = w;
    }
    STN_HIP(hipMemcpyAsync(h, src, n * 4, hipMemcpyDeviceToHost, s));
}

std::string Engine::op_ffn_ex(int M, int C, int I, const float* xn, int ldx, int64_t xn_elems, const float* W1, const float* b1, const float* W2,
                              const float* b2, const float* gamma, const int* len, int L, const int* row_b, const float* rowvec, int rv_ld, int nseq,
                              int mode, int split, float* x, int ldo, int64_t x_elems, float* part, int64_t part_stride, int64_t part_elems) {
    STN_HIP(hipSetDevice(device_));
    ar_.reset();
    float* d_w1 = up(ar_, s_, W1, (size_t)I * C);
    float* d_w2 = up(ar_, s_, W2, (size_t)C * I);
    FfnOp op = op_ffn_setup("op_ffn_ex", mode, M, C, I, d_w1, d_w2, split);
    FfnArgs& fa = op.a;
    fa.xn = up_as(ar_, s_, dt_, xn, (size_t)xn_elems); fa.ldx = ldx;
    float* d_x = up(ar_, s_, x, (size_t)x_elems);
    fa.x = d_x; fa.ldo = ldo;
    fa.b1 = up(ar_, s_, b1, (size_t)I);
    fa.b2 = b2 ? up(ar_, s_, b2, (size_t)C) : nullptr;
    fa.gamma = gamma ? up(ar_, s_, gamma, (size_t)C) : nullptr;
    fa.rowvec = rowvec ? up(ar_, s_, rowvec, (size_t)nseq * rv_ld) : nullptr; fa.rv_ld = rv_ld;
    fa.row_b = row_b ? up(ar_, s_, row_b, (size_t)M) : nullptr;
    fa.len = len ? up(ar_, s_, len, (size_t)nseq) : nullptr; fa.L = L;
    void* d_part = nullptr;
    if (op.f.kind == FFN_K4_SPLIT) {
        d_part = up_as(ar_, s_, dt_, part, (size_t)part_elems);
        fa.part = d_part; fa.part_stride = part_stride;
    }
    ffn_launch(op.f, C, fa, op.w1, op.w2);
    STN_HIP(hipGetLastError());
    STN_HIP(hipMemcpyAsync(x, d_x, sizeof(float) * (size_t)x_elems, hipMemcpyDeviceToHost, s_));
    if (d_part) down_as(ar_, s_, dt_, d_part, part, (size_t)part_elems);
    sync();
    return op.f.str();
}

std::string Engine::op_dwconv_ln_ex(int dtype, int B, int L, int C, int k, int dil, const float* x, int64_t x_rows, const float* w,
                                    const float* bias, const float* g, const float* b, const int* seqlen, int packed, int ln_only, float* y,
                                    int64_t y_rows) {
    STN_HIP(hipSetDevice(device_));
    ar_.reset();
    const int* dlen = seqlen ? up(ar_, s_, seqlen, (size_t)B) : nullptr;
    float* dx = up(ar_, s_, x, (size_t)x_rows * C);
    float* dg = up(ar_, s_, g, (size_t)C);
    float* dbt = up(ar_, s_, b, (size_t)C);
    void* dy = up_as(ar_, s_, dtype, y, (size_t)y_rows * C);
    std::string form = "layernorm";
    if (ln_only) {
        launch_layernorm(s_, dtype, dx, (int64_t)B * L, C, dg, dbt, 1e-6f, dy);
    } else {
        std::vector<float> wt((size_t)C * k);
        for (int c = 0; c < C; ++c) for (int j = 0; j < k; ++j) wt[(size_t)j * C + c] = w[(size_t)c * k + j];
        float* dw = up(ar_, s_, wt.data(), wt.size());
        float* db = up(ar_, s_, bias, (size_t)C);
        int* off = nullptr;
        if (packed) {
            off = static_cast<int*>(ar_.alloc(sizeof(int) * (size_t)(B + 1)));
            launch_row_map(s_, dlen, B, off, nullptr);
        }
        form = dwconv_ln_form(dtype, B, L, C, k, packed != 0).str();
        launch_dwconv_ln(s_, dtype, dx, B, L, C, dw, db, k, dil, dg, dbt, 1e-6f, dy, dlen, off);
    }
    STN_HIP(hipGetLastError());
    down_as(ar_, s_, dtype, dy, y, (size_t)y_rows * C);
    sync();
    return form;
}

void Engine::op_fold_ln(int dtype, int M, int C, int S, const float* part, const float* b2, const float* gamma, const float* rowvec,
                        const int* row_b, int nseq, const float* g, const float* b, float* x, float* y) {
    STN_HIP(hipSetDevice(device_));
    ar_.reset();
    const size_t n = (size_t)M * C;
    FoldArgs fo;
    fo.part = up_as(ar_, s_, dtype, part, n * S); fo.S = S; fo.part_stride = (int64_t)n;
    fo.b2 = up(ar_, s_, b2, (size_t)C); fo.gamma = up(ar_, s_, gamma, (size_t)C);
    fo.rowvec = rowvec ? up(ar_, s_, rowvec, (size_t)nseq * C) : nullptr; fo.rv_ld = C;
    fo.row_b = (rowvec && row_b) ? up(ar_, s_, row_b, (size_t)M) : nullptr;
    float* dx = up(ar_, s_, x, n);
    float* dg = up(ar_, s_, g, (size_t)C);
    float* dbt = up(ar_, s_, b, (size_t)C);
    void* dy = ar_.alloc(n * 2);
    launch_fold_ln(s_, dtype, dx, M, C, fo, dg, dbt, 1e-6f, dy);
    STN_HIP(hipGetLastError());
    STN_HIP(hipMemcpyAsync(x, dx, n * 4, hipMemcpyDeviceToHost, s_));
    down_as(ar_, s_, dtype, dy, y, n);
    sync();
}

std::string Engine::op_fold_dwconv_ln_ex(int dtype, int B, int L, int C, int k, int dil, int S, int run_frames, const int* seqlen, const float* x_in,
                                         int64_t x_rows, const float* part, int64_t part_stride, int64_t part_elems, const float* b2, const float* gamma,
                                         const float* rowvec, int rv_ld, const float* w, const float* bias, const float* g, const float* b, float* x_out,
                                         int64_t x_out_rows, float* y, int64_t y_rows) {
    STN_HIP(hipSetDevice(device_));
    ar_.reset();
    std::vector<float> wt((size_t)C * k);
    for (int c = 0; c < C; ++c) for (int j = 0; j < k; ++j) wt[(size_t)j * C + c] = w[(size_t)c * k + j];
    const int* dlen = up(ar_, s_, seqlen, (size_t)B);
    int* doff = static_cast<int*>(ar_.alloc(sizeof(int) * (size_t)(B + 1)));
    launch_row_map(s_, dlen, B, doff, nullptr);
    float* dx = up(ar_, s_, x_in, (size_t)x_rows * C);
    float* dxo = up(ar_, s_, x_out, (size_t)x_out_rows * C);
    void* dy = up_as(ar_, s_, dtype, y, (size_t)y_rows * C);
    float* dw = up(ar_, s_, wt.data(), wt.size());
    float* db = up(ar_, s_, bias, (size_t)C);
    float* dg = up(ar_, s_, g, (size_t)C);
    float* dbt = up(ar_, s_, b, (size_t)C);
    FoldArgs fo;
    fo.part = up_as(ar_, s_, dtype, part, (size_t)part_elems); fo.S = S; fo.part_stride = part_stride;
    if (b2) fo.b2 = up(ar_, s_, b2, (size_t)C);
    else { float* z = f32_alloc(C); launch_fill(s_, z, C, 0.f); fo.b2 = z; }
    if (gamma) fo.gamma = up(ar_, s_, gamma, (size_t)C);
    else { float* o = f32_alloc(C); launch_fill(s_, o, C, 1.f); fo.gamma = o; }
    fo.rowvec = rowvec ? up(ar_, s_, rowvec, (size_t)B * rv_ld) : nullptr; fo.rv_ld = rowvec ? rv_ld : C;
// ... 160 lines not shown
```

### supertonic_amd/csrc/kernels.hpp

```cpp
#pragma once
#include <hip/hip_runtime.h>
#include <hip/hip_ext.h>
#include <stdint.h>
#include <stdio.h>
#include <stdlib.h>

#include <stdexcept>
#include <type_traits>
#include <utility>
#include <vector>
#include <string>

#include "dither.hpp"

namespace stn {

struct LaunchEvents { hipEvent_t start = nullptr, stop = nullptr; };
inline thread_local LaunchEvents g_launch_ev;
struct LaunchLog {
    bool on = false;
    const char* family = "-";
    std::vector<std::pair<std::string, const char*>> entries;
    void add(const char* kexpr) { if (entries.size() < 200000) entries.emplace_back(family, kexpr); }
};
// ... 95 lines not shown
    int M = 0, I = 0;
    const int* row_b = nullptr;
    const float* rowvec = nullptr; int rv_ld = 0;
    const int* len = nullptr; int L = 1;
    unsigned long long* ts = nullptr;
    int split = 1;
    void* part = nullptr;
    int64_t part_stride = 0;
};
bool ffn_fused_supported(int dtype, int C, int I);
int ffn_split_factor(int dtype, int C, int I);
constexpr int FFN_SPLITS[] = {4, 8, 12};
bool ffn_split_valid(int dtype, int C, int I, int S);
int ffn_split_choose(int dtype, int C, int I, int64_t M);
inline int64_t ffn_split_rows(int64_t M) { return (M + 127) / 128 * 128; }
enum FfnKind : int { FFN_GEMMS = 0, FFN_K4 = 1, FFN_K4_SPLIT = 2 };
enum FfnStage : int { FFN_VOCODER = 1, FFN_ESTIMATOR = 2, FFN_TEXT = 4 };
struct FfnForm {
    int kind = FFN_GEMMS, split = 1;
    bool nt = false;
    std::string str() const;
};
FfnForm ffn_form(int dtype, int stage, int C, int I, int64_t M, int64_t gate_rows, bool packed, int k, int max_dil, int mask, int64_t min_rows,
                 int64_t split_min_rows, bool nt_hints);
__host__ __device__ constexpr inline int ffn_lds_side_offset(int C, int I) { return (4 * C * 64 + (I + 2 * C) * 4 + 1023) & ~1023; }
__host__ __device__ constexpr inline bool ffn_lds_has_side(int C) { return C == 384; }
void launch_ffn_fused(hipStream_t s, int dtype, int C, const FfnArgs& a);
struct FoldArgs {
    const void* part = nullptr; int S = 0; int64_t part_stride = 0;
    const float* b2 = nullptr;
    const float* gamma = nullptr;
    const float* rowvec = nullptr; int rv_ld = 0;
    const int* row_b = nullptr;
    unsigned long long* ts = nullptr;
    int run_frames = 0;
};
int fold_run_frames(const int* lengths, int B, int n_cu);
void launch_fold_ln(hipStream_t s, int act_dtype, float* x, int64_t M, int C, const FoldArgs& f, const float* g, const float* b, float eps, void* y);
bool fold_dwconv_ln_supported(int C, int k, int dil);
struct FoldDwconvLnForm {
    int act_dtype = BF16, K = 5, nslot = 3, S = 4, U = 1, run = 32, cps = 1;
    bool rv = false;
    unsigned grid = 0;
    size_t lds = 0;
    std::string str() const;
};
FoldDwconvLnForm fold_dwconv_ln_form(int act_dtype, int B, int L, int C, int k, int dil, int S, bool has_rowvec, int run_frames);
void launch_fold_dwconv_ln(hipStream_t s, int act_dtype, const float* x_in, float* x_out, int B, int L, int C, const FoldArgs& f, const float* w_t,
                           const float* bias, int k, int dil, const float* ln_g, const float* ln_b, float eps, void* y, const int* seqlen,
                           const int* row_off);
void launch_repack_frag_acc(hipStream_t s, const void* W, int N, int K, void* Wf);
void launch_ffn_pack(hipStream_t s, const void* W1, const void* W2, int C, int I, void* tmp, void* wseq, int S = 1);

void launch_dwconv_ln(hipStream_t s, int out_dtype, const float* x, int B, int L, int C, const float* w_t,
                      const float* bias, int k, int dil, const float* ln_g, const float* ln_b, float eps, void* y,
                      const int* seqlen = nullptr, const int* row_off = nullptr);
enum DwconvLnKernel : int { DW_V3 = 0, DW_V2 = 1, DW_GENERIC = 2 };
struct DwconvLnForm {
    int out_dtype = F32;
    int kernel = DW_GENERIC;
    int K = 0, R = 1;
    bool occ4 = false;
    std::string str() const;
};
DwconvLnForm dwconv_ln_form(int out_dtype, int B, int L, int C, int k, bool packed);
bool dwconv_ln_supports_packed(int C, int k);
void launch_row_map(hipStream_t s, const int* len, int B, int* row_off , int* row_b ,
                    int rows_padded = 0 );
constexpr int LN_NI = 4;
void check_ln_shape(int C);
void launch_layernorm(hipStream_t s, int out_dtype, const float* x, int64_t M, int C, const float* g, const float* b,
                      float eps, void* y);

enum AttnVec : int { ATTN_VEC_Q = 1, ATTN_VEC_K = 2, ATTN_VEC_V = 4 };
struct AttnForm {
    int dtype = F32;
    bool mfma = false;
    int dh = 0;
    int kc = 0, nch = 0;
    int tpr = 8, vec = 0;
    size_t lds = 0;
    std::string str() const;
};
AttnForm attn_form(int dtype, int B, int Lq, int Lk, int H, int dh, int ldq, int ldk, const void* q, const void* k, const void* v);
void launch_attention(hipStream_t s, int dtype, const void* q, int ldq, const void* k, const void* v, int ldk, void* o,
                      int ldo, int B, int Lq, int Lk, int H, int dh, const int* qlen, const int* klen, int rope_mode,
                      float rope_base, float rope_gamma, bool k_rotated = false,
                      const int* q_off = nullptr ,
                      const int* k_off = nullptr );
void launch_repack_frag(hipStream_t s, const void* W, int N, int K, void* Wf);
bool xattn_hs_supported(int dtype, int C, int H, int L, int Lk, int ldk);
void launch_xattn_hs(hipStream_t s, int dtype, const void* xn, int64_t M, const void* WqF, const float* bq, const void* kp, const void* vp, int ldk,
                     const void* WoA, void* part, int64_t part_stride, int B, int L, int Lk, const int* qlen, const int* klen,
                     const int* q_off, const int* k_off, int rope_mode, float rope_base, float rope_gamma, unsigned long long* ts = nullptr,
                     const int* pairs = nullptr );
struct XattnHsForm {
    bool f16 = false;
    int U = 1, kc = 32;
    size_t lds = 0;
    std::string str() const;
};
XattnHsForm xattn_hs_form(int dtype, int C, int H, int B, int L, int Lk, int ldk);
void launch_xattn_hs_pairs(hipStream_t s, const int* qlen, int B, int* pairs);
void launch_rope_rows(hipStream_t s, int dtype, void* x, int ld, int B, int L, const int* len, int groups, int group_stride,
                      int H, int dh, int rope_mode, float rope_base, float rope_gamma, const int* row_off = nullptr );

void launch_embed(hipStream_t s, const int64_t* ids, const float* emb, int vocab, int B, int L, int C, const int* len,
                  float* x, const int* row_off = nullptr );
void launch_mask_to_len(hipStream_t s, const float* mask, int B, int L, int* len);
void launch_ncl_to_rows(hipStream_t s, int out_dtype, const float* in, int B, int C, int L, void* out, int ld_out = 0,
                        const int* len = nullptr, const int* row_off = nullptr );
void launch_euler_ncl(hipStream_t s, const float* prev, const float* v, const float* dt, const int* len, int B, int D, int L, float* out,
                      const int* row_off = nullptr , void* z_rows = nullptr, int z_dtype = 0, int ldz = 0);
void launch_cast(hipStream_t s, int out_dtype, const float* in, int64_t n, void* out);
void launch_add_rowvec(hipStream_t s, float* x, const float* v, int ldv, int B, int L, int C, const int* len);
void launch_time_embed(hipStream_t s, const float* cur, const float* tot, int B, int dim, float scale, float* te);
void launch_scale_len(hipStream_t s, const int* len, int B, int factor, int* out);
void launch_vocoder_in(hipStream_t s, const float* latent, int B, int L, int ld, int ccf, const float* w ,
                       const float* bias, int C, int k, float* x, const int* seqlen = nullptr);
void launch_vocoder_im2col(hipStream_t s, int out_dtype, const float* latent, int B, int L, int ld, int ccf, int k, int kp, void* cols,
                           const int* seqlen = nullptr ,
                           const int* row_off = nullptr );
void launch_unpack_rows(hipStream_t s, const float* src, const int* len, const int* row_off, int B, int T, int W, float* dst);
void launch_trim_len(hipStream_t s, const int* len, int B, int ccf, int T, int rf, int* n_out, int* valid_out);
void launch_unpack_rows_quiet(hipStream_t s, const float* src, const int* valid, const int* row_off, int B, int T, int W, int rf,
                              const float* quiet, const float* edge, float* dst);
void launch_masked_mean(hipStream_t s, int in_dtype, const void* x, int B, int L, int C, const int* len, float* pooled,
                        const int* row_off = nullptr );
void launch_softplus(hipStream_t s, float* x, int n);
void launch_scale(hipStream_t s, float* x, int n, float mul);
void launch_randn_masked(hipStream_t s, uint64_t seed, const int64_t* utt_ids, int B, int D, int L, const int* len,
                         float* xt, const unsigned long long* seed_dev = nullptr );
void launch_mask_ncl(hipStream_t s, float* x, int B, int D, int L, const int* len);
void launch_reciprocal(hipStream_t s, const float* in, int n, float* out);
void launch_bf16_to_f32(hipStream_t s, const uint16_t* in, int64_t n, float* out);
void launch_half_to_f32(hipStream_t s, int in_dtype, const void* in, int64_t n, float* out);
void launch_fill(hipStream_t s, float* x, int n, float v);
void launch_step_counters(hipStream_t s, float* tot , float* cur , float* dt , int B, int steps);
enum OutEnc : int { ENC_F32 = 0, ENC_PCM16 = 1, ENC_PCM24 = 2, ENC_MULAW = 3, ENC_ALAW = 4 };
constexpr int enc_bytes(int enc) {
    return enc == ENC_F32 ? 4 : enc == ENC_PCM16 ? 2 : enc == ENC_PCM24 ? 3 : (enc == ENC_MULAW || enc == ENC_ALAW) ? 1 : 0;
}
template <typename Fn>
inline void with_enc(int enc, const char* who, Fn&& fn) {
    switch (enc) {
        case ENC_F32: fn(std::integral_constant<int, ENC_F32>{}); break;
        case ENC_PCM16: fn(std::integral_constant<int, ENC_PCM16>{}); break;
        case ENC_PCM24: fn(std::integral_constant<int, ENC_PCM24>{}); break;
        case ENC_MULAW: fn(std::integral_constant<int, ENC_MULAW>{}); break;
        case ENC_ALAW: fn(std::integral_constant<int, ENC_ALAW>{}); break;
        default: throw std::invalid_argument(std::string(who) + ": unknown encoding " + std::to_string(enc));
    }
}
struct Dither {
    int mode = DITHER_OFF; uint64_t seed = 0; unsigned kind = DITHER_ROW; const int64_t* ids = nullptr;
    const int64_t* lim = nullptr; int64_t lim_stride = 1;
};
void launch_store_rows(hipStream_t s, const float* x, int64_t rows, int64_t W, const float* g, int enc, void* y, int64_t dst_stride, const Dither& d = {});
struct JoinSeg { int64_t dst, len, row; };
struct JoinProg { int64_t len; int32_t first, count; };
void launch_join_rows(hipStream_t s, const float* x, int64_t src_stride, const JoinSeg* seg, const JoinProg* prog, int G, int64_t Wj, const float* g,
                      int enc, void* y, int64_t dst_stride, const Dither& d = {});
struct JoinSegT { int64_t dst, len, row, src; int32_t fin, fout; };
void launch_join_trim_rows(hipStream_t s, const float* x, int64_t src_stride, const JoinSegT* seg, const JoinProg* prog, int G, int64_t Wj,
                           const float* g, const float* fade, int enc, void* y, int64_t dst_stride, const Dither& d = {});

constexpr int ED_CHUNK = 32;
constexpr int ED_WG = 256;
__host__ __device__ inline int64_t ed_chunks(int64_t W) { return (W + ED_CHUNK - 1) / ED_CHUNK; }
inline int edges_frame(int hz) { return (hz + 50) / 100; }
inline int64_t edges_frames(int64_t W, int hz) { const int F = edges_frame(hz); return (W + F - 1) / F; }
void launch_edges_frames(hipStream_t s, const float* x, int64_t rows, int64_t W, const int64_t* n, int hz, float* pa, float* pb);
void launch_edges_rows(hipStream_t s, int64_t rows, int64_t W, const int64_t* n, int hz, double top_db, int64_t keep, int64_t fd, const float* pa,
                       const float* pb, double* lev, int64_t* edges, JoinSegT* seg, JoinProg* prog);
const char* edges_staging_form(const float* x, int64_t W);
constexpr int PZ_MAX_CUTS = 255;
void launch_pause_rows(hipStream_t s, int64_t rows, int64_t W, const int64_t* n, int hz, double top_db, int64_t fd, int64_t Mp, int S, const double* lev,
// ... 122 lines not shown
```

### supertonic_amd/csrc/kernels_dwconv_ln.hip

```cpp
#include "kernels.hpp"
#include "kernels_dev.hpp"
#include "dev_env.hpp"

#include <type_traits>
#include <stdio.h>
#include <stdlib.h>

namespace stn {

template <typename OutT, bool CONV>
__global__ __launch_bounds__(256) void dwconv_ln_kernel(const float* __restrict__ x, int64_t M, int L, int C,
                                                        const float* __restrict__ w_t, const float* __restrict__ bias,
                                                        int k, int dil, const float* __restrict__ g,
                                                        const float* __restrict__ bt, float eps, OutT* __restrict__ y,
                                                        const int* __restrict__ seqlen) {
    const int lane = threadIdx.x & 63;
    const int64_t row = (int64_t)blockIdx.x * 4 + (threadIdx.x >> 6);
    if (row >= M) return;
    const int Lv = (CONV && seqlen) ? seqlen[row / L] : L;
    const bool live = !(CONV && (int)(row % L) >= Lv);
    const int C4 = C >> 2;
    const float4* x4 = reinterpret_cast<const float4*>(x);
    float4 h[LN_NI];
    if (CONV) {
// ... 90 lines not shown
#pragma unroll
        for (int j = 0; j < K; ++j) wv[j] = w4[(int64_t)j * C4 + cc];
#pragma unroll
        for (int r = 0; r < R; ++r)
#pragma unroll
            for (int j = 0; j < K; ++j) {
                const int tt = tpos[r] + (j - HALF) * dil;
                const int tc = tt < 0 ? 0 : (tt >= L ? L - 1 : tt);
                xv[r][j] = x4[(base[r] + tc) * C4 + cc];
            }
        const float4 bv = b4[cc];
#pragma unroll
        for (int r = 0; r < R; ++r) {
            float4 a = bv;
#pragma unroll
            for (int j = 0; j < K; ++j) {
                const int tt = tpos[r] + (j - HALF) * dil;
                const bool keep = tt >= 0 && tt < lv[r];
                const float4 v = keep ? xv[r][j] : make_float4(0.f, 0.f, 0.f, 0.f);
                a.x = fmaf(wv[j].x, v.x, a.x); a.y = fmaf(wv[j].y, v.y, a.y);
                a.z = fmaf(wv[j].z, v.z, a.z); a.w = fmaf(wv[j].w, v.w, a.w);
            }
            h[r][i] = act ? a : make_float4(0.f, 0.f, 0.f, 0.f);
        }
    }
    const float4* g4 = reinterpret_cast<const float4*>(g);
    const float4* bt4 = reinterpret_cast<const float4*>(bt);
#pragma unroll
    for (int r = 0; r < R; ++r) {
        float s = (h[r][0].x + h[r][0].y) + (h[r][0].z + h[r][0].w) + (h[r][1].x + h[r][1].y) + (h[r][1].z + h[r][1].w);
        const float mean = wave_sum(s) / (float)C;
        float v = 0.f;
#pragma unroll
        for (int i = 0; i < 2; ++i)
            if (lane + 64 * i < C4) {
                const float dx = h[r][i].x - mean, dy = h[r][i].y - mean, dz = h[r][i].z - mean, dw = h[r][i].w - mean;
                v += (dx * dx + dy * dy) + (dz * dz + dw * dw);
            }
        const float rstd = rsqrtf(wave_sum(v) / (float)C + eps);
        if (!rowok[r]) continue;
        const bool live = tpos[r] < lv[r];
#pragma unroll
        for (int i = 0; i < 2; ++i) {
            const int c4 = lane + 64 * i;
            if (c4 < C4) {
                const float4 gg = g4[c4], bb = bt4[c4];
                store4(y + (r0 + r) * C + c4 * 4, live ? (h[r][i].x - mean) * rstd * gg.x + bb.x : 0.f, live ? (h[r][i].y - mean) * rstd * gg.y + bb.y : 0.f,
                       live ? (h[r][i].z - mean) * rstd * gg.z + bb.z : 0.f, live ? (h[r][i].w - mean) * rstd * gg.w + bb.w : 0.f);
            }
        }
    }
}

template <typename OutT, int K, int R>
__device__ __forceinline__ void dwconv_ln_v3_body(const float* __restrict__ x, int nseq, int L, int C,
                                                           const float* __restrict__ w_t, const float* __restrict__ bias,
                                                           int dil, int wps , const float* __restrict__ g,
                                                           const float* __restrict__ bt, float eps, OutT* __restrict__ y,
                                                           const int* __restrict__ seqlen, const int* __restrict__ row_off, int xcd_runs) {
    const int lane = threadIdx.x & 63;
    int bid = blockIdx.x;
    if (xcd_runs) {
        const int nb = gridDim.x, q = nb >> 3, rr = nb & 7, xcd = bid & 7, idx = bid >> 3;
        bid = xcd * q + (xcd < rr ? xcd : rr) + idx;
    }
    const int64_t wid = (int64_t)bid * 4 + (threadIdx.x >> 6);
    if (wid >= (int64_t)nseq * wps) return;
    const int b = (int)(wid / wps), rem = (int)(wid % wps);
    const int t0 = (rem / dil) * (R * dil) + (rem % dil);
    const int Lv = seqlen ? seqlen[b] : L;
    constexpr int HALF = (K - 1) / 2, NWIN = R + K - 1;
    const int C4 = C >> 2;
    const int64_t row0 = row_off ? (int64_t)row_off[b] : (int64_t)b * L;
    if (t0 >= Lv) {
        if (row_off) return;
#pragma unroll
        for (int r = 0; r < R; ++r) {
            const int t = t0 + r * dil;
            if (t >= L) break;
#pragma unroll
            for (int i = 0; i < 2; ++i)
                if (lane + 64 * i < C4) store4(y + (row0 + t) * C + (lane + 64 * i) * 4, 0.f, 0.f, 0.f, 0.f);
        }
        return;
    }
    const float4* x4 = reinterpret_cast<const float4*>(x) + row0 * C4;
    const float4* w4 = reinterpret_cast<const float4*>(w_t);
    const float4* b4 = reinterpret_cast<const float4*>(bias);
    float4 h[R][2];
#pragma unroll
    for (int i = 0; i < 2; ++i) {
        const int c4 = lane + 64 * i;
        const bool act = c4 < C4;
        const int cc = act ? c4 : 0;
        float4 win[NWIN], wv[K];
#pragma unroll
        for (int j = 0; j < K; ++j) wv[j] = w4[(int64_t)j * C4 + cc];
#pragma unroll
        for (int q = 0; q < NWIN; ++q) {
            const int tt = t0 + (q - HALF) * dil;
            const int hi_ = row_off ? Lv : L;
            const int tc = tt < 0 ? 0 : (tt >= hi_ ? hi_ - 1 : tt);
            const float4 v = x4[(int64_t)tc * C4 + cc];
            win[q] = (tt >= 0 && tt < Lv) ? v : make_float4(0.f, 0.f, 0.f, 0.f);
        }
        const float4 bv = b4[cc];
#pragma unroll
        for (int r = 0; r < R; ++r) {
            float4 a = bv;
#pragma unroll
            for (int j = 0; j < K; ++j) {
                a.x = fmaf(wv[j].x, win[r + j].x, a.x); a.y = fmaf(wv[j].y, win[r + j].y, a.y);
                a.z = fmaf(wv[j].z, win[r + j].z, a.z); a.w = fmaf(wv[j].w, win[r + j].w, a.w);
            }
            h[r][i] = act ? a : make_float4(0.f, 0.f, 0.f, 0.f);
        }
    }
    const float4* g4 = reinterpret_cast<const float4*>(g);
    const float4* bt4 = reinterpret_cast<const float4*>(bt);
    float4 gg[2], bb[2];
#pragma unroll
    for (int i = 0; i < 2; ++i) {
        const int c4 = lane + 64 * i;
        gg[i] = g4[c4 < C4 ? c4 : 0];
        bb[i] = bt4[c4 < C4 ? c4 : 0];
    }
#pragma unroll
    for (int r = 0; r < R; ++r) {
        const int t = t0 + r * dil;
        const float s = (h[r][0].x + h[r][0].y) + (h[r][0].z + h[r][0].w) + (h[r][1].x + h[r][1].y) + (h[r][1].z + h[r][1].w);
        const float mean = wave_sum(s) / (float)C;
        float v = 0.f;
#pragma unroll
        for (int i = 0; i < 2; ++i)
            if (lane + 64 * i < C4) {
                const float dx = h[r][i].x - mean, dy = h[r][i].y - mean, dz = h[r][i].z - mean, dw = h[r][i].w - mean;
                v += (dx * dx + dy * dy) + (dz * dz + dw * dw);
            }
        const float rstd = rsqrtf(wave_sum(v) / (float)C + eps);
        if (t >= L) continue;
        if (t >= Lv) {
            if (row_off) continue;
#pragma unroll
            for (int i = 0; i < 2; ++i)
                if (lane + 64 * i < C4) store4(y + (row0 + t) * C + (lane + 64 * i) * 4, 0.f, 0.f, 0.f, 0.f);
            continue;
        }
#pragma unroll
        for (int i = 0; i < 2; ++i) {
            const int c4 = lane + 64 * i;
            if (c4 < C4)
                store4(y + (row0 + t) * C + c4 * 4, (h[r][i].x - mean) * rstd * gg[i].x + bb[i].x,
                       (h[r][i].y - mean) * rstd * gg[i].y + bb[i].y, (h[r][i].z - mean) * rstd * gg[i].z + bb[i].z,
                       (h[r][i].w - mean) * rstd * gg[i].w + bb[i].w);
        }
    }
}

template <typename OutT, int K, int R>
__global__ __launch_bounds__(256) void dwconv_ln_v3_kernel(const float* __restrict__ x, int nseq, int L, int C, const float* __restrict__ w_t,
                                                           const float* __restrict__ bias, int dil, int wps, const float* __restrict__ g, const float* __restrict__ bt,
                                                           float eps, OutT* __restrict__ y, const int* __restrict__ seqlen, const int* __restrict__ row_off, int xcd_runs) {
    dwconv_ln_v3_body<OutT, K, R>(x, nseq, L, C, w_t, bias, dil, wps, g, bt, eps, y, seqlen, row_off, xcd_runs);
}
template <typename OutT, int K, int R>
__global__ __launch_bounds__(256) __attribute__((amdgpu_waves_per_eu(4, 4))) void dwconv_ln_v3_occ4_kernel(
    const float* __restrict__ x, int nseq, int L, int C, const float* __restrict__ w_t, const float* __restrict__ bias, int dil, int wps,
    const float* __restrict__ g, const float* __restrict__ bt, float eps, OutT* __restrict__ y, const int* __restrict__ seqlen,
    const int* __restrict__ row_off, int xcd_runs) {
    dwconv_ln_v3_body<OutT, K, R>(x, nseq, L, C, w_t, bias, dil, wps, g, bt, eps, y, seqlen, row_off, xcd_runs);
}

template <typename OutT, int K, int R>
static void launch_dwconv_ln_v3_kr(hipStream_t s, bool occ4, const float* x, int nseq, int L, int C, const float* w_t, const float* bias,
                                   int dil, const float* g, const float* b, float eps, OutT* y, const int* seqlen, const int* row_off) {
    const int wps = ((L + R * dil - 1) / (R * dil)) * dil;
    const int64_t nw = (int64_t)nseq * wps;
    static const int xcd_runs = [] { const char* e = stn::dev_env("STN_DWCONV_XCD"); return e ? atoi(e) : 1; }();
    if constexpr (K == 7 && R == 4 && !std::is_same<OutT, f16_t>::value) {
        if (occ4) {
            STN_KLAUNCH((dwconv_ln_v3_occ4_kernel<OutT, K, R>), dim3((unsigned)((nw + 3) / 4)), dim3(256), 0, s, x, nseq, L, C, w_t, bias,
                               dil, wps, g, b, eps, y, seqlen, row_off, xcd_runs);
            return;
        }
    }
    if (occ4) throw std::logic_error("dwconv_ln: no occ4 kernel for this form");
    STN_KLAUNCH((dwconv_ln_v3_kernel<OutT, K, R>), dim3((unsigned)((nw + 3) / 4)), dim3(256), 0, s, x, nseq, L, C, w_t, bias,
                       dil, wps, g, b, eps, y, seqlen, row_off, xcd_runs);
}

void check_ln_shape(int C) {
    if (C % 4 || C > 4 * 64 * LN_NI) { char m_[256]; snprintf(m_, sizeof m_, "LayerNorm width %d unsupported (C %% 4 == 0, C <= 1024)", C); throw std::invalid_argument(m_); }
}

bool dwconv_ln_supports_packed(int C, int k) { return C <= 512 && C % 4 == 0 && (k == 5 || k == 7); }

std::string DwconvLnForm::str() const {
    if (kernel == DW_GENERIC) return "generic";
    char m_[32];
    if (kernel == DW_V2) snprintf(m_, sizeof m_, "v2<%d>", K);
    else snprintf(m_, sizeof m_, "%s<%d,%d>", occ4 ? "v3occ4" : "v3", K, R);
    return m_;
}

DwconvLnForm dwconv_ln_form(int out_dtype, int B, int L, int C, int k, bool packed) {
    check_ln_shape(C);
    if (packed && !dwconv_ln_supports_packed(C, k)) throw std::invalid_argument("packed dwconv_ln needs lengths, C <= 512, k in {5,7}");
    DwconvLnForm f;
    f.out_dtype = out_dtype == BF16 || out_dtype == F16 ? out_dtype : F32;
    f.K = k;
    if (C > 512 || (k != 5 && k != 7)) return f;
    const int64_t M = (int64_t)B * L;
    f.kernel = DW_V3;
    if (M >= 32768) {
        f.R = k == 5 ? 8 : 4;
    } else if (M >= 4096) {
        f.R = k == 5 ? (M < 16384 ? 2 : 4) : 4;
    } else if (packed) {
        f.R = k == 5 ? (M < 1024 ? 2 : 4) : 4;
    } else {
        f.kernel = DW_V2;
        f.R = 2;
    }
    f.occ4 = f.kernel == DW_V3 && f.K == 7 && f.R == 4 && f.out_dtype != F16;
    return f;
}

template <typename OutT>
static void launch_dwconv_ln_t(hipStream_t s, const DwconvLnForm& f, const float* x, int B, int L, int C, const float* w_t, const float* bias,
                               int k, int dil, const float* g, const float* b, float eps, OutT* y, const int* seqlen, const int* row_off) {
    const int64_t M = (int64_t)B * L;
    if (f.kernel == DW_V3) {
        if (f.K == 5 && f.R == 2) launch_dwconv_ln_v3_kr<OutT, 5, 2>(s, f.occ4, x, B, L, C, w_t, bias, dil, g, b, eps, y, seqlen, row_off);
        else if (f.K == 5 && f.R == 4) launch_dwconv_ln_v3_kr<OutT, 5, 4>(s, f.occ4, x, B, L, C, w_t, bias, dil, g, b, eps, y, seqlen, row_off);
        else if (f.K == 5 && f.R == 8) launch_dwconv_ln_v3_kr<OutT, 5, 8>(s, f.occ4, x, B, L, C, w_t, bias, dil, g, b, eps, y, seqlen, row_off);
        else if (f.K == 7 && f.R == 4) launch_dwconv_ln_v3_kr<OutT, 7, 4>(s, f.occ4, x, B, L, C, w_t, bias, dil, g, b, eps, y, seqlen, row_off);
        else throw std::logic_error("dwconv_ln: no v3 kernel for form " + f.str());
    } else if (f.kernel == DW_V2) {
        constexpr int R = 2;
        const dim3 grid((unsigned)((M + 4 * R - 1) / (4 * R)));
        if (f.K == 5) STN_KLAUNCH((dwconv_ln_v2_kernel<OutT, 5, R>), grid, dim3(256), 0, s, x, M, L, C, w_t, bias, dil, g, b, eps, y, seqlen);
        else if (f.K == 7) STN_KLAUNCH((dwconv_ln_v2_kernel<OutT, 7, R>), grid, dim3(256), 0, s, x, M, L, C, w_t, bias, dil, g, b, eps, y, seqlen);
        else throw std::logic_error("dwconv_ln: no v2 kernel for form " + f.str());
    } else {
        const dim3 grid((unsigned)((M + 3) / 4));
        STN_KLAUNCH((dwconv_ln_kernel<OutT, true>), grid, dim3(256), 0, s, x, M, L, C, w_t, bias, k, dil, g, b, eps, y, seqlen);
    }
}

void launch_dwconv_ln(hipStream_t s, int out_dtype, const float* x, int B, int L, int C, const float* w_t,
                      const float* bias, int k, int dil, const float* ln_g, const float* ln_b, float eps, void* y,
                      const int* seqlen, const int* row_off) {
    check_ln_shape(C);
    if ((int64_t)B * L == 0) return;
    if (row_off && !seqlen) { throw std::invalid_argument("packed dwconv_ln needs lengths, C <= 512, k in {5,7}"); }
    const DwconvLnForm f = dwconv_ln_form(out_dtype, B, L, C, k, row_off != nullptr);
    with_out_type(f.out_dtype, [&](auto* tag) {
        using T = std::remove_pointer_t<decltype(tag)>;
        launch_dwconv_ln_t(s, f, x, B, L, C, w_t, bias, k, dil, ln_g, ln_b, eps, static_cast<T*>(y), seqlen, row_off);
    });
}

void launch_layernorm(hipStream_t s, int out_dtype, const float* x, int64_t M, int C, const float* g, const float* b,
                      float eps, void* y) {
    check_ln_shape(C);
    if (M == 0) return;
    const dim3 grid((unsigned)((M + 3) / 4));
    with_out_type(out_dtype, [&](auto* tag) {
        using T = std::remove_pointer_t<decltype(tag)>;
        STN_KLAUNCH((dwconv_ln_kernel<T, false>), grid, dim3(256), 0, s, x, M, 1, C, nullptr, nullptr, 1, 1, g, b, eps, static_cast<T*>(y),
                    static_cast<const int*>(nullptr));
    });
}

}
```

### supertonic_amd/csrc/kernels_layout.hip

```cpp
#include "kernels.hpp"
#include "kernels_dev.hpp"

#include <type_traits>

namespace stn {

__global__ void embed_kernel(const int64_t* __restrict__ ids, const float* __restrict__ emb, int vocab, int L, int C,
                             const int* __restrict__ len, float* __restrict__ x, const int* __restrict__ row_off) {
    const int row = blockIdx.x, b = row / L, t = row - b * L;
    if (row_off && t >= len[b]) return;
    const int64_t id = ids[row];
    const bool ok = t < len[b] && id >= 0 && id < vocab;
    const int C4 = C >> 2;
    float4* o = reinterpret_cast<float4*>(x) + (row_off ? (int64_t)row_off[b] + t : (int64_t)row) * C4;
    const float4* e = reinterpret_cast<const float4*>(emb) + (ok ? id : 0) * C4;
    for (int c = threadIdx.x; c < C4; c += blockDim.x) {
        float4 v = make_float4(0.f, 0.f, 0.f, 0.f);
        if (ok) v = e[c];
        o[c] = v;
    }
}
void launch_embed(hipStream_t s, const int64_t* ids, const float* emb, int vocab, int B, int L, int C, const int* len,
                  float* x, const int* row_off) {
    if (B * L == 0) return;
// ... 364 lines not shown
}
void launch_step_counters(hipStream_t s, float* tot, float* cur, float* dt, int B, int steps) {
    const int n = B * steps;
    if (n) STN_KLAUNCH(step_counters_kernel, dim3((n + 255) / 256), dim3(256), 0, s, tot, cur, dt, B, steps);
}

__global__ void randn_masked_kernel(unsigned long long seed, const unsigned long long* __restrict__ seed_dev,
                                    const int64_t* __restrict__ utt_ids, int D, int L, const int* __restrict__ len, int64_t n4,
                                    float* __restrict__ xt) {
    if (seed_dev) seed = *seed_dev;
    const int64_t i = (int64_t)blockIdx.x * blockDim.x + threadIdx.x;
    if (i >= n4) return;
    const int L4 = (L + 3) >> 2;
    const int t4 = (int)(i % L4);
    const int64_t r = i / L4;
    const int d = (int)(r % D);
    const int b = (int)(r / D);
    const unsigned long long u = utt_ids ? (unsigned long long)utt_ids[b] : (unsigned long long)b;
    unsigned c[4] = {(unsigned)t4, (unsigned)d, (unsigned)u, (unsigned)(u >> 32)};
    philox4x32_10(c, (unsigned)seed, (unsigned)(seed >> 32));
    float nrm[4];
#pragma unroll
    for (int h = 0; h < 2; ++h) {
        const float u1 = ((float)(c[2 * h] >> 8) + 0.5f) * (1.0f / 16777216.0f);
        const float u2 = ((float)(c[2 * h + 1] >> 8) + 0.5f) * (1.0f / 16777216.0f);
        const float rr = sqrtf(-2.0f * logf(u1)), th = 6.28318530717958647692f * u2;
        nrm[2 * h] = rr * cosf(th);
        nrm[2 * h + 1] = rr * sinf(th);
    }
    const int nb = len ? len[b] : L;
#pragma unroll
    for (int q = 0; q < 4; ++q) {
        const int t = t4 * 4 + q;
        if (t < L) xt[((int64_t)b * D + d) * L + t] = t < nb ? nrm[q] : 0.f;
    }
}
void launch_randn_masked(hipStream_t s, uint64_t seed, const int64_t* utt_ids, int B, int D, int L, const int* len,
                         float* xt, const unsigned long long* seed_dev) {
    const int64_t n4 = (int64_t)B * D * ((L + 3) / 4);
    if (n4 == 0) return;
    STN_KLAUNCH(randn_masked_kernel, dim3((unsigned)((n4 + 255) / 256)), dim3(256), 0, s, (unsigned long long)seed,
                       seed_dev, utt_ids, D, L, len, n4, xt);
}

__global__ void scale_len_kernel(const int* __restrict__ len, int B, int factor, int* __restrict__ out) {
    const int i = blockIdx.x * blockDim.x + threadIdx.x;
    if (i < B) out[i] = len[i] * factor;
}
void launch_scale_len(hipStream_t s, const int* len, int B, int factor, int* out) {
    if (B == 0) return;
    STN_KLAUNCH(scale_len_kernel, dim3((B + 255) / 256), dim3(256), 0, s, len, B, factor, out);
}

__global__ void trim_len_kernel(const int* __restrict__ len, int B, int ccf, int T, int rf, int* __restrict__ n_out,
                                int* __restrict__ valid_out) {
    const int i = blockIdx.x * blockDim.x + threadIdx.x;
    if (i >= B) return;
    const int l6 = len[i] * ccf;
    const bool trim = l6 + 2 * rf <= T;
    n_out[i] = trim ? l6 + 2 * rf : T;
    valid_out[i] = trim ? l6 + rf : T;
}
void launch_trim_len(hipStream_t s, const int* len, int B, int ccf, int T, int rf, int* n_out, int* valid_out) {
    if (B == 0) return;
    STN_KLAUNCH(trim_len_kernel, dim3((B + 255) / 256), dim3(256), 0, s, len, B, ccf, T, rf, n_out, valid_out);
}

__global__ void unpack_rows_quiet_kernel(const float* __restrict__ src, const int* __restrict__ valid, const int* __restrict__ row_off,
                                         int T, int W4, int rf, const float* __restrict__ quiet, const float* __restrict__ edge,
                                         int64_t n4, float* __restrict__ dst) {
    const int64_t i = (int64_t)blockIdx.x * blockDim.x + threadIdx.x;
    if (i >= n4) return;
    const int c = (int)(i % W4);
    const int64_t r = i / W4;
    const int t = (int)(r % T);
    const int b = (int)(r / T);
    float4 v;
    if (t < valid[b]) v = reinterpret_cast<const float4*>(src)[((int64_t)row_off[b] + t) * W4 + c];
    else if (t >= T - rf) v = reinterpret_cast<const float4*>(edge)[(int64_t)(t - (T - rf)) * W4 + c];
    else v = reinterpret_cast<const float4*>(quiet)[c];
    reinterpret_cast<float4*>(dst)[i] = v;
}
void launch_unpack_rows_quiet(hipStream_t s, const float* src, const int* valid, const int* row_off, int B, int T, int W, int rf,
                              const float* quiet, const float* edge, float* dst) {
    const int64_t n4 = (int64_t)B * T * (W / 4);
    if (n4 == 0) return;
    if (W % 4) { throw std::invalid_argument("unpack_rows needs W % 4 == 0"); }
    STN_KLAUNCH(unpack_rows_quiet_kernel, dim3((unsigned)((n4 + 255) / 256)), dim3(256), 0, s, src, valid, row_off, T, W / 4, rf, quiet, edge,
                n4, dst);
}

__global__ void mask_ncl_kernel(float* __restrict__ x, int D, int L, int64_t n, const int* __restrict__ len) {
    const int64_t i = (int64_t)blockIdx.x * blockDim.x + threadIdx.x;
    if (i >= n) return;
    const int t = (int)(i % L);
    const int b = (int)(i / ((int64_t)D * L));
    if (t >= len[b]) x[i] = 0.f;
}
void launch_mask_ncl(hipStream_t s, float* x, int B, int D, int L, const int* len) {
    const int64_t n = (int64_t)B * D * L;
    if (n == 0) return;
    STN_KLAUNCH(mask_ncl_kernel, dim3((unsigned)((n + 255) / 256)), dim3(256), 0, s, x, D, L, n, len);
}

}
```

Baseline: 47200.

## Add tail-table trimmed vocoder form using precomputed zero-latent boundary rows

Adds a new trimmed vocoder form that computes only valid rows plus one receptive field per sequence, instead of two. Rows past each sequence's end that the dwconv stencil needs come from per-block tail tables captured once from a zero-latent run. The tables are kept separately for the GEMM and fused-K4 FFN forms. The unpack kernel is also restructured so each wave copies whole rows and resolves its source pointers once. The tail substitution assumes boundary activations match the zero-latent run, which adds complexity and some numerical risk.

```diff
diff --git a/include/stn.h b/include/stn.h
--- a/include/stn.h
+++ b/include/stn.h
@@ -292,6 +292,9 @@
 int stn_op_dwconv_ln_ex(stn_handle* h, int dtype, int B, int L, int C, int k, int dil, const float* x, int64_t x_rows,
                         const float* w_or_null , const float* bias_or_null, const float* ln_g, const float* ln_b,
                         const int32_t* seqlen_or_null, int packed, int ln_only, float* y, int64_t y_rows, char* form, size_t form_cap);
+int stn_op_dwconv_ln_tail(stn_handle* h, int dtype, int B, int L, int C, int k, int dil, const float* x, int64_t x_rows,
+                          const float* w , const float* bias, const float* ln_g, const float* ln_b, const int32_t* seqlen,
+                          const float* tail , int T, int rf, float* y, int64_t y_rows, char* form, size_t form_cap);
 int stn_dbg_dwconv_ln_form(int dtype, int B, int L, int C, int k, int packed, char* out, size_t cap);
 int stn_op_fold_ln(stn_handle* h, int dtype, int M, int C, int S, const float* part, const float* b2, const float* gamma,
                    const float* rowvec_or_null, const int32_t* row_b_or_null, int nseq, const float* ln_g, const float* ln_b, float* x,
diff --git a/supertonic_amd/binding.py b/supertonic_amd/binding.py
--- a/supertonic_amd/binding.py
+++ b/supertonic_amd/binding.py
@@ -573,6 +573,8 @@
     L.stn_op_attention.argtypes = [vp, ci, ci, ci, ci, ci, ci, _f32p, _f32p, _f32p, vp, vp, ci, _f32p]
     L.stn_op_dwconv_ln_ex.argtypes = [vp, ci, ci, ci, ci, ci, ci, _f32p, ctypes.c_int64, vp, vp, _f32p, _f32p, vp, ci, ci, _f32p, ctypes.c_int64,
                                       ctypes.c_char_p, ctypes.c_size_t]
+    L.stn_op_dwconv_ln_tail.argtypes = [vp, ci, ci, ci, ci, ci, ci, _f32p, ctypes.c_int64, _f32p, _f32p, _f32p, _f32p, _i32p, _f32p, ci, ci, _f32p,
+                                        ctypes.c_int64, ctypes.c_char_p, ctypes.c_size_t]
     L.stn_dbg_resample_form.argtypes = [ci, ci, ctypes.c_int64, ctypes.c_char_p, ctypes.c_size_t]
     L.stn_dbg_resample_form.restype = ctypes.c_int
     L.stn_dbg_dwconv_ln_form.argtypes = [ci, ci, ci, ci, ci, ci, ctypes.c_char_p, ctypes.c_size_t]
@@ -2153,6 +2155,21 @@
                                                ctypes.sizeof(form)))
         return o_r, form.value.decode()
 
+    def op_dwconv_ln_tail(self, x, w, bias, g, b, dil, out, L, seqlen, tail, T, dtype=None):
+        x = _c(x, np.float32)
+        tail = _c(tail, np.float32)
+        o_r = np.array(out, dtype=np.float32, order="C", copy=True)
+        C = x.shape[1]
+        w = _c(w, np.float32)
+        seqlen = _c(seqlen, np.int32)
+        assert tail.ndim == 2 and tail.shape[1] == C and tail.shape[0] >= 1
+        form = ctypes.create_string_buffer(32)
+        self._ck(self._lib.stn_op_dwconv_ln_tail(self._h, self.dtype if dtype is None else _DTYPES[dtype], len(seqlen), int(L), C, w.shape[1],
+                                                 int(dil), x.reshape(-1), x.shape[0], w, _c(bias, np.float32), _c(g, np.float32),
+                                                 _c(b, np.float32), seqlen, tail.reshape(-1), int(T), tail.shape[0] - 1, o_r.reshape(-1),
+                                                 o_r.shape[0], form, ctypes.sizeof(form)))
+        return o_r, form.value.decode()
+
     def op_fold_ln(self, x, part, b2, gamma, g, b, rowvec=None, row_b=None, dtype=None):
         x_r = np.array(x, dtype=np.float32, order="C", copy=True)
         M, C = x_r.shape
diff --git a/supertonic_amd/csrc/api.cpp b/supertonic_amd/csrc/api.cpp
--- a/supertonic_amd/csrc/api.cpp
+++ b/supertonic_amd/csrc/api.cpp
@@ -959,6 +959,25 @@
                         int64_t y_rows, char* form, size_t form_cap) {
     STN_TRY(h, dwconv_ln_ex_checked(h, dtype, B, L, C, k, dil, x, x_rows, w, bias, g, b, seqlen, packed, ln_only, y, y_rows, form, form_cap))
 }
+static void dwconv_ln_tail_checked(stn_handle* h, int dtype, int B, int L, int C, int k, int dil, const float* x, int64_t x_rows, const float* w,
+                                   const float* bias, const float* g, const float* b, const int32_t* seqlen, const float* tail, int T, int rf,
+                                   float* y, int64_t y_rows, char* form, size_t form_cap) {
+    need(B > 0 && B <= 1024 && L > 0 && C > 0 && C % 4 == 0 && C <= 512 && (k == 5 || k == 7) && dil > 0 && x && w && bias && g && b && y && seqlen &&
+             x_rows > 0 && y_rows > 0,
+         "stn_op_dwconv_ln_tail: bad argument");
+    need(dtype == STN_DTYPE_F32 || dtype == STN_DTYPE_BF16 || dtype == STN_DTYPE_F16, "stn_op_dwconv_ln_tail: unknown dtype");
+    need(tail && rf >= 0 && T >= L, "stn_op_dwconv_ln_tail: needs a tail table of rf + 1 >= 1 rows and T >= L");
+    int64_t rows = 0;
+    for (int i = 0; i < B; ++i) { need(seqlen[i] >= 0 && seqlen[i] <= L, "stn_op_dwconv_ln_tail: seqlen out of [0, L]"); rows += seqlen[i]; }
+    need(x_rows >= rows && y_rows >= rows, "stn_op_dwconv_ln_tail: x / y hold fewer rows than the launch addresses");
+    const std::string f = h->eng->op_dwconv_ln_ex(dtype, B, L, C, k, dil, x, x_rows, w, bias, g, b, seqlen, 1, 0, y, y_rows, tail, T, rf);
+    if (form && form_cap) std::snprintf(form, form_cap, "%s", f.c_str());
+}
+int stn_op_dwconv_ln_tail(stn_handle* h, int dtype, int B, int L, int C, int k, int dil, const float* x, int64_t x_rows, const float* w,
+                          const float* bias, const float* g, const float* b, const int32_t* seqlen, const float* tail, int T, int rf, float* y,
+                          int64_t y_rows, char* form, size_t form_cap) {
+    STN_TRY(h, dwconv_ln_tail_checked(h, dtype, B, L, C, k, dil, x, x_rows, w, bias, g, b, seqlen, tail, T, rf, y, y_rows, form, form_cap))
+}
 int stn_dbg_dwconv_ln_form(int dtype, int B, int L, int C, int k, int packed, char* out, size_t cap) {
     if (B < 1 || L < 1 || C < 1 || k < 1 || !(k & 1) || (dtype != STN_DTYPE_F32 && dtype != STN_DTYPE_BF16 && dtype != STN_DTYPE_F16)) return STN_ERR_INVALID;
     std::string f;
diff --git a/supertonic_amd/csrc/engine.cpp b/supertonic_amd/csrc/engine.cpp
--- a/supertonic_amd/csrc/engine.cpp
+++ b/supertonic_amd/csrc/engine.cpp
@@ -156,8 +156,7 @@
     free_weights();
     for (void* p : batch_owned_) (void)hipFree(p);
     for (void* p : batch_retired_) (void)hipFree(p);
-    if (vo_quiet_) (void)hipFree(vo_quiet_);
-    if (vo_edge_) (void)hipFree(vo_edge_);
+    free_vocoder_constants();
     if (tcond_.buf) (void)hipFree(tcond_.buf);
     for (auto& sp : spans_) { (void)hipEventDestroy(sp.a); (void)hipEventDestroy(sp.b); }
     for (auto ev : ev_pool_) (void)hipEventDestroy(ev);
@@ -521,12 +520,13 @@
 }
 
 void Engine::convnext(const ConvNeXt& p, const FfnForm& f, float* x, int B, int L, int C, int hid, int k, int dil, const int* len,
-                      const int* conv_len, const float* rowvec, int rv_ld, const Ragged* rg, FoldState* fs) {
+                      const int* conv_len, const float* rowvec, int rv_ld, const Ragged* rg, FoldState* fs, const DwconvTail& tl) {
     const int64_t M = rg ? (int64_t)rg->rows : (int64_t)B * L;
     if (f.kind == FFN_K4_SPLIT && !(fs && rg)) throw std::logic_error("convnext: K4-split needs the stage's fold state and packed rows");
     const Arena::Mark mk = ar_.mark();
     void* xn = act_alloc(M * C);
     if (fs) x = fs->x;
+    if (tl.tail && (fs || !rg)) throw std::logic_error("convnext: a tail table needs packed rows and no fold state");
     if (fs && fs->pending) {
         if (prof_on_) prof_begin("fold_dwconv_ln", (double)M * C * (2.0 * k + 8 + 2.0 * fs->fold.S), (double)M * C * (8.0 + 2.0 + 2.0 * fs->fold.S));
         fs->fold.run_frames = rg->fold_run;
@@ -537,7 +537,7 @@
         x = fs->x;
     } else {
         if (prof_on_) prof_begin("dwconv_ln", (double)M * C * (2.0 * k + 8), (double)M * C * (4.0 + (is_half(dt_) ? 2.0 : 4.0)));
-        launch_dwconv_ln(s_, dt_, x, B, L, C, p.dw_t, p.dw_b, k, dil, p.ln.g, p.ln.b, a_.ln_eps, xn, rg ? len : conv_len, rg ? rg->off : nullptr);
+        launch_dwconv_ln(s_, dt_, x, B, L, C, p.dw_t, p.dw_b, k, dil, p.ln.g, p.ln.b, a_.ln_eps, xn, rg ? len : conv_len, rg ? rg->off : nullptr, tl);
         if (prof_on_) prof_end();
     }
     FfnArgs fa;
@@ -978,29 +978,46 @@
     if (tmp) (void)hipFree(tmp);
 }
 
+void Engine::free_vocoder_constants() {
+    for (VoConsts& c : vo_c_) {
+        if (c.quiet) (void)hipFree(c.quiet);
+        if (c.edge) (void)hipFree(c.edge);
+        if (c.tail) (void)hipFree(c.tail);
+        c = VoConsts();
+    }
+    vo_rf_ = 0;
+}
+
 void Engine::prepare_vocoder_constants() {
-    if (vo_quiet_) { (void)hipFree(vo_quiet_); vo_quiet_ = nullptr; }
-    if (vo_edge_) { (void)hipFree(vo_edge_); vo_edge_ = nullptr; }
-    vo_rf_ = 0;
+    free_vocoder_constants();
     const stn_arch& a = a_;
     if (!is_half(dt_) || !dwconv_ln_supports_packed(a.vo_dim, a.vo_kernel) || a.base_chunk_size % 4) return;
-    const int rf = vocoder_receptive_field(), ccf = a.chunk_compress_factor, W = a.base_chunk_size;
+    const int rf = vocoder_receptive_field(), ccf = a.chunk_compress_factor, W = a.base_chunk_size, C = a.vo_dim;
     const int Lz = (4 * rf + ccf) / ccf + 1, Tz = Lz * ccf, D = a.latent_dim * ccf;
-    ar_.reset();
-    float* lat = f32_alloc((int64_t)D * Lz);
-    float* wz = f32_alloc((int64_t)Tz * W);
-    STN_HIP(hipMemsetAsync(lat, 0, sizeof(float) * (size_t)D * Lz, s_));
-    vocoder_dev(1, Lz, lat, wz);
-    STN_HIP(hipMalloc(reinterpret_cast<void**>(&vo_quiet_), sizeof(float) * (size_t)W));
-    STN_HIP(hipMalloc(reinterpret_cast<void**>(&vo_edge_), sizeof(float) * (size_t)rf * W));
-    STN_HIP(hipMemcpyAsync(vo_quiet_, wz + (size_t)2 * rf * W, sizeof(float) * (size_t)W, hipMemcpyDeviceToDevice, s_));
-    STN_HIP(hipMemcpyAsync(vo_edge_, wz + (size_t)(Tz - rf) * W, sizeof(float) * (size_t)rf * W, hipMemcpyDeviceToDevice, s_));
-    sync();
+    const bool k4 = a.vo_blocks > 0 && ffn_fused_supported(dt_, C, a.vo_hidden) && ffn_w_.count(convnext_w("vo.blk0").pw1.w.as(dt_));
+    for (int kind : {(int)FFN_GEMMS, (int)FFN_K4}) {
+        if (kind == FFN_K4 && !k4) continue;
+        VoConsts& c = vo_c_[kind == FFN_K4];
+        const size_t tail_n = (size_t)std::max(a.vo_blocks, 1) * (rf + 1) * C;
+        STN_HIP(hipMalloc(reinterpret_cast<void**>(&c.quiet), sizeof(float) * (size_t)W));
+        STN_HIP(hipMalloc(reinterpret_cast<void**>(&c.edge), sizeof(float) * (size_t)std::max(rf, 1) * W));
+        STN_HIP(hipMalloc(reinterpret_cast<void**>(&c.tail), sizeof(float) * tail_n));
+        ar_.reset();
+        float* lat = f32_alloc((int64_t)D * Lz);
+        float* wz = f32_alloc((int64_t)Tz * W);
+        STN_HIP(hipMemsetAsync(lat, 0, sizeof(float) * (size_t)D * Lz, s_));
+        vo_force_ffn_ = kind; vo_capture_ = c.tail;
+        try { vocoder_dev(1, Lz, lat, wz); } catch (...) { vo_force_ffn_ = -1; vo_capture_ = nullptr; throw; }
+        vo_force_ffn_ = -1; vo_capture_ = nullptr;
+        STN_HIP(hipMemcpyAsync(c.quiet, wz + (size_t)2 * rf * W, sizeof(float) * (size_t)W, hipMemcpyDeviceToDevice, s_));
+        STN_HIP(hipMemcpyAsync(c.edge, wz + (size_t)(Tz - rf) * W, sizeof(float) * (size_t)rf * W, hipMemcpyDeviceToDevice, s_));
+        sync();
+    }
     vo_rf_ = rf;
 }
 
 int Engine::trimmed_rows(int B, int L, std::vector<int>* n_host) const {
-    if (!packed_ve_ || vo_ragged_ || !vo_quiet_ || vo_rf_ <= 0 || B > 1024) return 0;
+    if (!packed_ve_ || vo_ragged_ || !vo_c_[0].quiet || vo_rf_ <= 0 || B > 1024) return 0;
     const int ccf = a_.chunk_compress_factor, T = L * ccf, rf = vo_rf_;
     long tot = 0;
     bool any = false;
@@ -1015,12 +1032,28 @@
     return (any && tot * 10 <= (long)B * T * 9) ? (int)tot : 0;
 }
 
-void Engine::vocoder_dev(int B, int L, const float* latent, float* wav, const int* vlen, int vrows, const int* valid) {
+int Engine::tail_rows(int B, int L) const {
+    if (!packed_ve_ || vo_ragged_ || !vo_c_[0].tail || vo_rf_ <= 0 || B > 1024) return 0;
+    const int ccf = a_.chunk_compress_factor, T = L * ccf, rf = vo_rf_;
+    long tot = 0;
+    for (int i = 0; i < B; ++i) tot += std::min(bt_.h_llen[i] * ccf + rf, T);
+    return tot * 10 <= (long)B * T * 9 ? (int)tot : 0;
+}
+
+int Engine::vocoder_rows(int B, int L, int* form) const {
+    int rows = trimmed_rows(B, L, nullptr);
+    *form = rows ? VO_TRIM_2RF : VO_DENSE;
+    if (!rows && (rows = tail_rows(B, L))) *form = VO_TRIM_TAIL;
+    return rows;
+}
+
+void Engine::vocoder_dev(int B, int L, const float* latent, float* wav, const int* vlen, int vrows, const int* valid, bool tails) {
     stage_ = "vo";
     const stn_arch& a = a_;
     const int C = a.vo_dim, T = L * a.chunk_compress_factor;
     const bool packed = vlen && vrows > 0 && is_half(dt_) && B <= 1024 && dwconv_ln_supports_packed(C, a.vo_kernel);
     if (valid && !packed) throw std::runtime_error("trimmed vocoder needs the packed bf16 path");
+    if (tails && !valid) throw std::logic_error("vocoder_dev: the tail form is a trimmed form");
     const int64_t M = packed ? (int64_t)vrows : (int64_t)B * T;
     const Arena::Mark mk = ar_.mark();
     Ragged rg;
@@ -1046,11 +1079,23 @@
                           a.vo_in_kernel, x, vlen);
         if (prof_on_) prof_end();
     }
-    const FfnForm ff = ffn_plan(FFN_VOCODER, C, a.vo_hidden, M, valid ? (int64_t)B * T : 0, packed, a.vo_kernel,
-                                a.vo_blocks ? *std::max_element(a.vo_dilations, a.vo_dilations + a.vo_blocks) : 1);
-    for (int i = 0; i < a.vo_blocks; ++i)
+    FfnForm ff = ffn_plan(FFN_VOCODER, C, a.vo_hidden, M, valid ? (int64_t)B * T : 0, packed, a.vo_kernel,
+                          a.vo_blocks ? *std::max_element(a.vo_dilations, a.vo_dilations + a.vo_blocks) : 1);
+    if (vo_force_ffn_ >= 0) ff = FfnForm{vo_force_ffn_, 1, false};
+    const VoConsts& vc = vo_c_[ff.kind == FFN_K4];
+    if (valid && !(vc.quiet && vc.edge && vc.tail)) throw std::logic_error("vocoder_dev: no zero-latent constants for form " + ff.str());
+    DwconvTail tl;
+    for (int i = 0; i < a.vo_blocks; ++i) {
+        if (vo_capture_) {
+            const int rf = vocoder_receptive_field();
+            for (int j = 0; j <= rf; ++j)
+                STN_HIP(hipMemcpyAsync(vo_capture_ + ((size_t)i * (rf + 1) + j) * C, x + (size_t)(M - 1 - j) * C, sizeof(float) * (size_t)C,
+                                       hipMemcpyDeviceToDevice, s_));
+        }
+        if (tails) { tl.tail = vc.tail + (size_t)i * (vo_rf_ + 1) * C; tl.T = T; tl.rf = vo_rf_; }
         convnext(convnext_w("vo.blk" + std::to_string(i)), ff, x, B, T, C, a.vo_hidden, a.vo_kernel, a.vo_dilations[i],
-                 packed ? vlen : nullptr, packed ? nullptr : vlen, nullptr, 0, rgp);
+                 packed ? vlen : nullptr, packed ? nullptr : vlen, nullptr, 0, rgp, nullptr, tl);
+    }
     void* xn = act_alloc(M * C);
     const LNorm ln = lnorm("vo.out_ln");
     launch_layernorm(s_, dt_, x, M, C, ln.g, ln.b, a.ln_eps, xn);
@@ -1058,8 +1103,10 @@
         float* wp = f32_alloc(M * a.base_chunk_size);
         Epilogue e; e.mode = EPI_STORE; e.out_dtype = F32; e.out = wp; e.ldo = a.base_chunk_size;
         gemm("gemm_head", dt_, xn, C, linear("vo.head"), (int)M, e);
-        if (valid) launch_unpack_rows_quiet(s_, wp, valid, rg.off, B, T, a.base_chunk_size, vo_rf_, vo_quiet_, vo_edge_, wav);
+        if (prof_on_) prof_begin("unpack_rows", 0.0, ((double)M + (double)B * T) * a.base_chunk_size * 4.0);
+        if (valid) launch_unpack_rows_quiet(s_, wp, valid, rg.off, B, T, a.base_chunk_size, vo_rf_, vc.quiet, vc.edge, wav);
         else launch_unpack_rows(s_, wp, vlen, rg.off, B, T, a.base_chunk_size, wav);
+        if (prof_on_) prof_end();
     } else {
         Epilogue e; e.mode = EPI_STORE; e.out_dtype = F32; e.out = wav; e.ldo = a.base_chunk_size; e.len = vlen; e.L = T;
         gemm("gemm_head", dt_, xn, C, linear("vo.head"), (int)M, e);
diff --git a/supertonic_amd/csrc/engine.hpp b/supertonic_amd/csrc/engine.hpp
--- a/supertonic_amd/csrc/engine.hpp
+++ b/supertonic_amd/csrc/engine.hpp
@@ -153,7 +153,7 @@
                      bool z_ready = false ,
                      bool z_next = false );
     void vocoder_dev(int B, int L, const float* latent, float* wav, const int* vlen = nullptr, int vrows = 0,
-                     const int* valid = nullptr);
+                     const int* valid = nullptr, bool tails = false);
     int vocoder_receptive_field() const;
     void prepare_xattn_weights();
     std::unordered_map<const void*, const void*> frag_w_;
@@ -402,7 +402,8 @@
     void op_dwconv_ln(int dtype, int B, int L, int C, int k, int dil, const float* x, const float* w, const float* bias,
                       const float* g, const float* b, float* y, const int* seqlen = nullptr );
     std::string op_dwconv_ln_ex(int dtype, int B, int L, int C, int k, int dil, const float* x, int64_t x_rows, const float* w, const float* bias,
-                                const float* g, const float* b, const int* seqlen, int packed, int ln_only, float* y, int64_t y_rows);
+                                const float* g, const float* b, const int* seqlen, int packed, int ln_only, float* y, int64_t y_rows,
+                                const float* tail = nullptr, int T = 0, int rf = 0);
     void op_fold_ln(int dtype, int M, int C, int S, const float* part, const float* b2, const float* gamma, const float* rowvec, const int* row_b,
                     int nseq, const float* g, const float* b, float* x, float* y);
     void op_layout(int which, int dtype, const int* p, const float* a, int64_t a_n, const float* b, int64_t b_n, const float* c, int64_t c_n,
@@ -461,7 +462,8 @@
     struct FfnOp { FfnForm f; Linear w1, w2; FfnArgs a; };
     FfnOp op_ffn_setup(const char* op, int mode, int M, int C, int I, const float* W1, const float* W2, int split = 0);
     void convnext(const ConvNeXt& p, const FfnForm& f, float* x, int B, int L, int C, int hid, int k, int dil, const int* len,
-                  const int* conv_len = nullptr, const float* rowvec = nullptr, int rv_ld = 0, const Ragged* rg = nullptr, FoldState* fs = nullptr);
+                  const int* conv_len = nullptr, const float* rowvec = nullptr, int rv_ld = 0, const Ragged* rg = nullptr, FoldState* fs = nullptr,
+                  const DwconvTail& tl = DwconvTail() );
     void fold_layernorm(FoldState& fs, int64_t M, int C, const LNorm& ln, void* xn, const char* tag);
     void attn_block(const Attn& p, float* x, int B, int Lq, int C, int H, const void* ctx, int Lk, const int* qlen,
                     const int* klen, int rope_mode, bool self, const Ragged* qrg = nullptr);
@@ -512,11 +514,11 @@
     std::vector<int64_t> out_spans(int64_t Wo, int hz) const;
     void enqueue_after_duration(int total_step, const std::function<void()>& take_text_rows);
     struct GraphKey {
-        int B = 0, Lt = 0, L = 0, steps = 0; bool noise = false, ragged = false; int xattn = 0; int ffn = 0; int rows = 0, vrows = 0, trows = 0;
+        int B = 0, Lt = 0, L = 0, steps = 0; bool noise = false, ragged = false; int xattn = 0; int ffn = 0; int rows = 0, vrows = 0, trows = 0; int vform = 0;
         uint64_t gen = 0, wgen = 0; const void* p0 = nullptr; const void* p1 = nullptr; const void* pin = nullptr; hipStream_t s = nullptr;
         bool operator==(const GraphKey& o) const {
             return B == o.B && Lt == o.Lt && L == o.L && steps == o.steps && noise == o.noise && ragged == o.ragged && xattn == o.xattn && ffn == o.ffn &&
-                   rows == o.rows && vrows == o.vrows && trows == o.trows && gen == o.gen && wgen == o.wgen && p0 == o.p0 && p1 == o.p1 && pin == o.pin && s == o.s;
+                   rows == o.rows && vrows == o.vrows && vform == o.vform && trows == o.trows && gen == o.gen && wgen == o.wgen && p0 == o.p0 && p1 == o.p1 && pin == o.pin && s == o.s;
         }
     };
     struct GraphEntry { GraphKey key; hipGraph_t graph = nullptr, graph2 = nullptr; hipGraphExec_t exec = nullptr, exec2 = nullptr; uint64_t last_use = 0; };
@@ -542,10 +544,20 @@
     int gelu_act_ = ACT_GELU;
     int fused_xattn_ = 1;
     int64_t last_ve_rows_ = 0, last_vo_rows_ = 0;
-    float* vo_quiet_ = nullptr;
-    float* vo_edge_ = nullptr;
+    struct VoConsts {
+        float* quiet = nullptr;
+        float* edge = nullptr;
+        float* tail = nullptr;
+    };
+    VoConsts vo_c_[2];
     int vo_rf_ = 0;
+    int vo_force_ffn_ = -1;
+    float* vo_capture_ = nullptr;
+    void free_vocoder_constants();
+    enum VoForm : int { VO_DENSE = 0, VO_TRIM_2RF = 1, VO_TRIM_TAIL = 2 };
     int trimmed_rows(int B, int L, std::vector<int>* n_host) const;
+    int tail_rows(int B, int L) const;
+    int vocoder_rows(int B, int L, int* form) const;
     long graph_replays_ = 0;
     int* pin_llen_ = nullptr; size_t pin_llen_cap_ = 0;
     unsigned long long* pin_seed_ = nullptr;
diff --git a/supertonic_amd/csrc/engine_batch.cpp b/supertonic_amd/csrc/engine_batch.cpp
--- a/supertonic_amd/csrc/engine_batch.cpp
+++ b/supertonic_amd/csrc/engine_batch.cpp
@@ -190,7 +190,7 @@
     if (packed_rows_ok(B)) for (int v : b.h_llen) key.rows += v;
     if (shape_buckets_) key.rows = (int)bucket_up(key.rows, 64);
     last_ve_rows_ = key.rows ? key.rows : (int64_t)B * L;
-    key.vrows = trimmed_rows(B, L, nullptr);
+    key.vrows = vocoder_rows(B, L, &key.vform);
     if (shape_buckets_) key.vrows = (int)bucket_up(key.vrows, 64 * a.chunk_compress_factor);
     key.trows = tpk ? b.trows : 0;
     last_vo_rows_ = (int64_t)B * L * a.chunk_compress_factor;
@@ -359,17 +359,18 @@
     }
     int vrows = 0;
     const int* valid = nullptr;
+    bool tails = false;
     if (vo_ragged_ && packed_ve_) {
         for (int v : b.h_llen) vrows += v * a.chunk_compress_factor;
         if (shape_buckets_) vrows = (int)bucket_up(vrows, 64 * a.chunk_compress_factor);
-    } else if (int tr = trimmed_rows(B, L, nullptr)) {
+    } else if (int vform = VO_DENSE; int tr = vocoder_rows(B, L, &vform)) {
         if (shape_buckets_) tr = (int)bucket_up(tr, 64 * a.chunk_compress_factor);
         int* n_dev = static_cast<int*>(ar_.alloc(sizeof(int) * B));
         int* v_dev = static_cast<int*>(ar_.alloc(sizeof(int) * B));
-        launch_trim_len(s_, b.llen, B, a.chunk_compress_factor, L * a.chunk_compress_factor, vo_rf_, n_dev, v_dev);
-        vlen = n_dev; valid = v_dev; vrows = tr;
-    }
-    vocoder_dev(B, L, b.xt[cur], b.wav, vlen, vrows, valid);
+        launch_trim_len(s_, b.llen, B, a.chunk_compress_factor, L * a.chunk_compress_factor, vo_rf_, n_dev, v_dev, vform == VO_TRIM_TAIL);
+        vlen = n_dev; valid = v_dev; vrows = tr; tails = vform == VO_TRIM_TAIL;
+    }
+    vocoder_dev(B, L, b.xt[cur], b.wav, vlen, vrows, valid, tails);
     STN_HIP(hipGetLastError());
 }
 
diff --git a/supertonic_amd/csrc/engine_ops.cpp b/supertonic_amd/csrc/engine_ops.cpp
--- a/supertonic_amd/csrc/engine_ops.cpp
+++ b/supertonic_amd/csrc/engine_ops.cpp
@@ -527,7 +527,7 @@
 
 std::string Engine::op_dwconv_ln_ex(int dtype, int B, int L, int C, int k, int dil, const float* x, int64_t x_rows, const float* w,
                                     const float* bias, const float* g, const float* b, const int* seqlen, int packed, int ln_only, float* y,
-                                    int64_t y_rows) {
+                                    int64_t y_rows, const float* tail, int T, int rf) {
     STN_HIP(hipSetDevice(device_));
     ar_.reset();
     const int* dlen = seqlen ? up(ar_, s_, seqlen, (size_t)B) : nullptr;
@@ -548,8 +548,10 @@
             off = static_cast<int*>(ar_.alloc(sizeof(int) * (size_t)(B + 1)));
             launch_row_map(s_, dlen, B, off, nullptr);
         }
+        DwconvTail tl;
+        if (tail) { tl.tail = up(ar_, s_, tail, (size_t)(rf + 1) * C); tl.T = T; tl.rf = rf; }
         form = dwconv_ln_form(dtype, B, L, C, k, packed != 0).str();
-        launch_dwconv_ln(s_, dtype, dx, B, L, C, dw, db, k, dil, dg, dbt, 1e-6f, dy, dlen, off);
+        launch_dwconv_ln(s_, dtype, dx, B, L, C, dw, db, k, dil, dg, dbt, 1e-6f, dy, dlen, off, tl);
     }
     STN_HIP(hipGetLastError());
     down_as(ar_, s_, dtype, dy, y, (size_t)y_rows * C);
diff --git a/supertonic_amd/csrc/kernels.hpp b/supertonic_amd/csrc/kernels.hpp
--- a/supertonic_amd/csrc/kernels.hpp
+++ b/supertonic_amd/csrc/kernels.hpp
@@ -171,9 +171,13 @@
 void launch_repack_frag_acc(hipStream_t s, const void* W, int N, int K, void* Wf);
 void launch_ffn_pack(hipStream_t s, const void* W1, const void* W2, int C, int I, void* tmp, void* wseq, int S = 1);
 
+struct DwconvTail {
+    const float* tail = nullptr;
+    int T = 0, rf = 0;
+};
 void launch_dwconv_ln(hipStream_t s, int out_dtype, const float* x, int B, int L, int C, const float* w_t,
                       const float* bias, int k, int dil, const float* ln_g, const float* ln_b, float eps, void* y,
-                      const int* seqlen = nullptr, const int* row_off = nullptr);
+                      const int* seqlen = nullptr, const int* row_off = nullptr, const DwconvTail& tl = DwconvTail());
 enum DwconvLnKernel : int { DW_V3 = 0, DW_V2 = 1, DW_GENERIC = 2 };
 struct DwconvLnForm {
     int out_dtype = F32;
@@ -241,7 +245,7 @@
                            const int* seqlen = nullptr ,
                            const int* row_off = nullptr );
 void launch_unpack_rows(hipStream_t s, const float* src, const int* len, const int* row_off, int B, int T, int W, float* dst);
-void launch_trim_len(hipStream_t s, const int* len, int B, int ccf, int T, int rf, int* n_out, int* valid_out);
+void launch_trim_len(hipStream_t s, const int* len, int B, int ccf, int T, int rf, int* n_out, int* valid_out, bool tail_form = false);
 void launch_unpack_rows_quiet(hipStream_t s, const float* src, const int* valid, const int* row_off, int B, int T, int W, int rf,
                               const float* quiet, const float* edge, float* dst);
 void launch_masked_mean(hipStream_t s, int in_dtype, const void* x, int B, int L, int C, const int* len, float* pooled,
diff --git a/supertonic_amd/csrc/kernels_dwconv_ln.hip b/supertonic_amd/csrc/kernels_dwconv_ln.hip
--- a/supertonic_amd/csrc/kernels_dwconv_ln.hip
+++ b/supertonic_amd/csrc/kernels_dwconv_ln.hip
@@ -166,12 +166,13 @@
     }
 }
 
-template <typename OutT, int K, int R>
+template <typename OutT, int K, int R, bool TAIL = false>
 __device__ __forceinline__ void dwconv_ln_v3_body(const float* __restrict__ x, int nseq, int L, int C,
                                                            const float* __restrict__ w_t, const float* __restrict__ bias,
                                                            int dil, int wps , const float* __restrict__ g,
                                                            const float* __restrict__ bt, float eps, OutT* __restrict__ y,
-                                                           const int* __restrict__ seqlen, const int* __restrict__ row_off, int xcd_runs) {
+                                                           const int* __restrict__ seqlen, const int* __restrict__ row_off, int xcd_runs,
+                                                           const float* __restrict__ tail = nullptr, int T = 0, int rf = 0) {
     const int lane = threadIdx.x & 63;
     int bid = blockIdx.x;
     if (xcd_runs) {
@@ -215,8 +216,20 @@
             const int tt = t0 + (q - HALF) * dil;
             const int hi_ = row_off ? Lv : L;
             const int tc = tt < 0 ? 0 : (tt >= hi_ ? hi_ - 1 : tt);
-            const float4 v = x4[(int64_t)tc * C4 + cc];
-            win[q] = (tt >= 0 && tt < Lv) ? v : make_float4(0.f, 0.f, 0.f, 0.f);
+            if constexpr (TAIL) {
+                const float4* src = x4 + (int64_t)tc * C4;
+                bool keep = tt >= 0 && tt < Lv;
+                if (tt >= Lv && tt < T) {
+                    const int j = T - 1 - tt;
+                    src = reinterpret_cast<const float4*>(tail) + (int64_t)(j < rf ? j : rf) * C4;
+                    keep = true;
+                }
+                const float4 v = src[cc];
+                win[q] = keep ? v : make_float4(0.f, 0.f, 0.f, 0.f);
+            } else {
+                const float4 v = x4[(int64_t)tc * C4 + cc];
+                win[q] = (tt >= 0 && tt < Lv) ? v : make_float4(0.f, 0.f, 0.f, 0.f);
+            }
         }
         const float4 bv = b4[cc];
 #pragma unroll
@@ -286,11 +299,41 @@
 }
 
 template <typename OutT, int K, int R>
+__global__ __launch_bounds__(256) void dwconv_ln_v3_tail_kernel(const float* __restrict__ x, int nseq, int L, int C, const float* __restrict__ w_t,
+                                                                const float* __restrict__ bias, int dil, int wps, const float* __restrict__ g,
+                                                                const float* __restrict__ bt, float eps, OutT* __restrict__ y,
+                                                                const int* __restrict__ seqlen, const int* __restrict__ row_off, int xcd_runs,
+                                                                const float* __restrict__ tail, int T, int rf) {
+    dwconv_ln_v3_body<OutT, K, R, true>(x, nseq, L, C, w_t, bias, dil, wps, g, bt, eps, y, seqlen, row_off, xcd_runs, tail, T, rf);
+}
+template <typename OutT, int K, int R>
+__global__ __launch_bounds__(256) __attribute__((amdgpu_waves_per_eu(4, 4))) void dwconv_ln_v3_tail_occ4_kernel(
+    const float* __restrict__ x, int nseq, int L, int C, const float* __restrict__ w_t, const float* __restrict__ bias, int dil, int wps,
+    const float* __restrict__ g, const float* __restrict__ bt, float eps, OutT* __restrict__ y, const int* __restrict__ seqlen,
+    const int* __restrict__ row_off, int xcd_runs, const float* __restrict__ tail, int T, int rf) {
+    dwconv_ln_v3_body<OutT, K, R, true>(x, nseq, L, C, w_t, bias, dil, wps, g, bt, eps, y, seqlen, row_off, xcd_runs, tail, T, rf);
+}
+
+template <typename OutT, int K, int R>
 static void launch_dwconv_ln_v3_kr(hipStream_t s, bool occ4, const float* x, int nseq, int L, int C, const float* w_t, const float* bias,
-                                   int dil, const float* g, const float* b, float eps, OutT* y, const int* seqlen, const int* row_off) {
+                                   int dil, const float* g, const float* b, float eps, OutT* y, const int* seqlen, const int* row_off,
+                                   const DwconvTail& tl) {
     const int wps = ((L + R * dil - 1) / (R * dil)) * dil;
     const int64_t nw = (int64_t)nseq * wps;
     static const int xcd_runs = [] { const char* e = stn::dev_env("STN_DWCONV_XCD"); return e ? atoi(e) : 1; }();
+    if (tl.tail) {
+        if constexpr (K == 7 && R == 4 && !std::is_same<OutT, f16_t>::value) {
+            if (occ4) {
+                STN_KLAUNCH((dwconv_ln_v3_tail_occ4_kernel<OutT, K, R>), dim3((unsigned)((nw + 3) / 4)), dim3(256), 0, s, x, nseq, L, C, w_t, bias,
+                                   dil, wps, g, b, eps, y, seqlen, row_off, xcd_runs, tl.tail, tl.T, tl.rf);
+                return;
+            }
+        }
+        if (occ4) throw std::logic_error("dwconv_ln: no occ4 kernel for this form");
+        STN_KLAUNCH((dwconv_ln_v3_tail_kernel<OutT, K, R>), dim3((unsigned)((nw + 3) / 4)), dim3(256), 0, s, x, nseq, L, C, w_t, bias,
+                           dil, wps, g, b, eps, y, seqlen, row_off, xcd_runs, tl.tail, tl.T, tl.rf);
+        return;
+    }
     if constexpr (K == 7 && R == 4 && !std::is_same<OutT, f16_t>::value) {
         if (occ4) {
             STN_KLAUNCH((dwconv_ln_v3_occ4_kernel<OutT, K, R>), dim3((unsigned)((nw + 3) / 4)), dim3(256), 0, s, x, nseq, L, C, w_t, bias,
@@ -342,13 +385,14 @@
 
 template <typename OutT>
 static void launch_dwconv_ln_t(hipStream_t s, const DwconvLnForm& f, const float* x, int B, int L, int C, const float* w_t, const float* bias,
-                               int k, int dil, const float* g, const float* b, float eps, OutT* y, const int* seqlen, const int* row_off) {
+                               int k, int dil, const float* g, const float* b, float eps, OutT* y, const int* seqlen, const int* row_off,
+                               const DwconvTail& tl) {
     const int64_t M = (int64_t)B * L;
     if (f.kernel == DW_V3) {
-        if (f.K == 5 && f.R == 2) launch_dwconv_ln_v3_kr<OutT, 5, 2>(s, f.occ4, x, B, L, C, w_t, bias, dil, g, b, eps, y, seqlen, row_off);
-        else if (f.K == 5 && f.R == 4) launch_dwconv_ln_v3_kr<OutT, 5, 4>(s, f.occ4, x, B, L, C, w_t, bias, dil, g, b, eps, y, seqlen, row_off);
-        else if (f.K == 5 && f.R == 8) launch_dwconv_ln_v3_kr<OutT, 5, 8>(s, f.occ4, x, B, L, C, w_t, bias, dil, g, b, eps, y, seqlen, row_off);
-        else if (f.K == 7 && f.R == 4) launch_dwconv_ln_v3_kr<OutT, 7, 4>(s, f.occ4, x, B, L, C, w_t, bias, dil, g, b, eps, y, seqlen, row_off);
+        if (f.K == 5 && f.R == 2) launch_dwconv_ln_v3_kr<OutT, 5, 2>(s, f.occ4, x, B, L, C, w_t, bias, dil, g, b, eps, y, seqlen, row_off, tl);
+        else if (f.K == 5 && f.R == 4) launch_dwconv_ln_v3_kr<OutT, 5, 4>(s, f.occ4, x, B, L, C, w_t, bias, dil, g, b, eps, y, seqlen, row_off, tl);
+        else if (f.K == 5 && f.R == 8) launch_dwconv_ln_v3_kr<OutT, 5, 8>(s, f.occ4, x, B, L, C, w_t, bias, dil, g, b, eps, y, seqlen, row_off, tl);
+        else if (f.K == 7 && f.R == 4) launch_dwconv_ln_v3_kr<OutT, 7, 4>(s, f.occ4, x, B, L, C, w_t, bias, dil, g, b, eps, y, seqlen, row_off, tl);
         else throw std::logic_error("dwconv_ln: no v3 kernel for form " + f.str());
     } else if (f.kernel == DW_V2) {
         constexpr int R = 2;
@@ -364,14 +408,15 @@
 
 void launch_dwconv_ln(hipStream_t s, int out_dtype, const float* x, int B, int L, int C, const float* w_t,
                       const float* bias, int k, int dil, const float* ln_g, const float* ln_b, float eps, void* y,
-                      const int* seqlen, const int* row_off) {
+                      const int* seqlen, const int* row_off, const DwconvTail& tl) {
     check_ln_shape(C);
     if ((int64_t)B * L == 0) return;
     if (row_off && !seqlen) { throw std::invalid_argument("packed dwconv_ln needs lengths, C <= 512, k in {5,7}"); }
+    if (tl.tail && (!row_off || tl.T < L || tl.rf < 0)) { throw std::invalid_argument("dwconv_ln: a tail table needs packed rows, T >= L and rf >= 0"); }
     const DwconvLnForm f = dwconv_ln_form(out_dtype, B, L, C, k, row_off != nullptr);
     with_out_type(f.out_dtype, [&](auto* tag) {
         using T = std::remove_pointer_t<decltype(tag)>;
-        launch_dwconv_ln_t(s, f, x, B, L, C, w_t, bias, k, dil, ln_g, ln_b, eps, static_cast<T*>(y), seqlen, row_off);
+        launch_dwconv_ln_t(s, f, x, B, L, C, w_t, bias, k, dil, ln_g, ln_b, eps, static_cast<T*>(y), seqlen, row_off, tl);
     });
 }
 
diff --git a/supertonic_amd/csrc/kernels_layout.hip b/supertonic_amd/csrc/kernels_layout.hip
--- a/supertonic_amd/csrc/kernels_layout.hip
+++ b/supertonic_amd/csrc/kernels_layout.hip
@@ -440,42 +440,59 @@
     STN_KLAUNCH(scale_len_kernel, dim3((B + 255) / 256), dim3(256), 0, s, len, B, factor, out);
 }
 
-__global__ void trim_len_kernel(const int* __restrict__ len, int B, int ccf, int T, int rf, int* __restrict__ n_out,
+__global__ void trim_len_kernel(const int* __restrict__ len, int B, int ccf, int T, int rf, int tail_form, int* __restrict__ n_out,
                                 int* __restrict__ valid_out) {
     const int i = blockIdx.x * blockDim.x + threadIdx.x;
     if (i >= B) return;
     const int l6 = len[i] * ccf;
+    if (tail_form) {
+        n_out[i] = valid_out[i] = l6 + rf < T ? l6 + rf : T;
+        return;
+    }
     const bool trim = l6 + 2 * rf <= T;
     n_out[i] = trim ? l6 + 2 * rf : T;
     valid_out[i] = trim ? l6 + rf : T;
 }
-void launch_trim_len(hipStream_t s, const int* len, int B, int ccf, int T, int rf, int* n_out, int* valid_out) {
+void launch_trim_len(hipStream_t s, const int* len, int B, int ccf, int T, int rf, int* n_out, int* valid_out, bool tail_form) {
     if (B == 0) return;
-    STN_KLAUNCH(trim_len_kernel, dim3((B + 255) / 256), dim3(256), 0, s, len, B, ccf, T, rf, n_out, valid_out);
-}
-
-__global__ void unpack_rows_quiet_kernel(const float* __restrict__ src, const int* __restrict__ valid, const int* __restrict__ row_off,
-                                         int T, int W4, int rf, const float* __restrict__ quiet, const float* __restrict__ edge,
-                                         int64_t n4, float* __restrict__ dst) {
-    const int64_t i = (int64_t)blockIdx.x * blockDim.x + threadIdx.x;
-    if (i >= n4) return;
-    const int c = (int)(i % W4);
-    const int64_t r = i / W4;
-    const int t = (int)(r % T);
-    const int b = (int)(r / T);
-    float4 v;
-    if (t < valid[b]) v = reinterpret_cast<const float4*>(src)[((int64_t)row_off[b] + t) * W4 + c];
-    else if (t >= T - rf) v = reinterpret_cast<const float4*>(edge)[(int64_t)(t - (T - rf)) * W4 + c];
-    else v = reinterpret_cast<const float4*>(quiet)[c];
-    reinterpret_cast<float4*>(dst)[i] = v;
+    STN_KLAUNCH(trim_len_kernel, dim3((B + 255) / 256), dim3(256), 0, s, len, B, ccf, T, rf, tail_form ? 1 : 0, n_out, valid_out);
+}
+
+constexpr int UNPACK_RW = 4;
+__global__ __launch_bounds__(256) void unpack_rows_quiet_kernel(const float* __restrict__ src, const int* __restrict__ valid,
+                                                                const int* __restrict__ row_off, int T, int W4, int rf,
+                                                                const float* __restrict__ quiet, const float* __restrict__ edge, int64_t nrows,
+                                                                float* __restrict__ dst) {
+    const int lane = threadIdx.x & 63;
+    const int wave = __builtin_amdgcn_readfirstlane((int)(threadIdx.x >> 6));
+    const int64_t r0 = ((int64_t)blockIdx.x * 4 + wave) * UNPACK_RW;
+    if (r0 >= nrows) return;
+    const float4* sp[UNPACK_RW];
+#pragma unroll
+    for (int i = 0; i < UNPACK_RW; ++i) {
+        const int64_t r = r0 + i < nrows ? r0 + i : nrows - 1;
+        const int b = (int)(r / T), t = (int)(r - (int64_t)b * T);
+        if (t < valid[b]) sp[i] = reinterpret_cast<const float4*>(src) + ((int64_t)row_off[b] + t) * W4;
+        else if (t >= T - rf) sp[i] = reinterpret_cast<const float4*>(edge) + (int64_t)(t - (T - rf)) * W4;
+        else sp[i] = reinterpret_cast<const float4*>(quiet);
+    }
+    float4* d4 = reinterpret_cast<float4*>(dst) + r0 * W4;
+    for (int c = lane; c < W4; c += 64) {
+        float4 v[UNPACK_RW];
+#pragma unroll
+        for (int i = 0; i < UNPACK_RW; ++i) v[i] = sp[i][c];
+#pragma unroll
+        for (int i = 0; i < UNPACK_RW; ++i)
+            if (r0 + i < nrows) d4[(int64_t)i * W4 + c] = v[i];
+    }
 }
 void launch_unpack_rows_quiet(hipStream_t s, const float* src, const int* valid, const int* row_off, int B, int T, int W, int rf,
                               const float* quiet, const float* edge, float* dst) {
-    const int64_t n4 = (int64_t)B * T * (W / 4);
-    if (n4 == 0) return;
+    const int64_t nrows = (int64_t)B * T;
+    if (nrows == 0 || W == 0) return;
     if (W % 4) { throw std::invalid_argument("unpack_rows needs W % 4 == 0"); }
-    STN_KLAUNCH(unpack_rows_quiet_kernel, dim3((unsigned)((n4 + 255) / 256)), dim3(256), 0, s, src, valid, row_off, T, W / 4, rf, quiet, edge,
-                n4, dst);
+    STN_KLAUNCH(unpack_rows_quiet_kernel, dim3((unsigned)((nrows + 4 * UNPACK_RW - 1) / (4 * UNPACK_RW))), dim3(256), 0, s, src, valid, row_off, T,
+                W / 4, rf, quiet, edge, nrows, dst);
 }
 
 __global__ void mask_ncl_kernel(float* __restrict__ x, int D, int L, int64_t n, const int* __restrict__ len) {
```

Result: faster. 47810, median of 6 (+1.3%).
